# Illumina/manta

Hardware: AMD Instinct MI355X
Metric: candidate SV loci assembled+aligned per second (whole node) (higher is better)
Workload: dtype int32; 1 GPU; BASELINE config[1]: synthetic small-indel loci, 80 reads/locus x150bp, k=31..76 step 5, assemble + 10-mer trim + GlobalLargeIndelAligner(2,-8,-24,-1,-1;-100) on 1800 bp windows; loci_per_gpu=10000, reads_per_locus=80, block_loci=10000, workers_per_gpu=1, parallelism=loci sharded over 1 rank(s); per rank a cost-ordered block queue, queue=rank, dist_world=1, mix=False

## Files before the change

### include/manta_amd.h

```cpp
#ifndef MANTA_AMD_H
#define MANTA_AMD_H

#include <stdint.h>

#ifdef __cplusplus
extern "C" {
#endif

#define MANTA_OK 0
#define MANTA_E_INVALID_ARG (-1)
#define MANTA_E_NO_DEVICE (-2)
#define MANTA_E_HIP (-3)
#define MANTA_E_EMPTY_SEQ (-4)
#define MANTA_E_UNSUPPORTED (-5)
#define MANTA_E_CAPACITY (-6)
#define MANTA_E_DEVICE_FAULT (-7)
#define MANTA_E_SPLIT_QUERY_NOT_SHORTER (-8)
#define MANTA_E_SPLIT_EMPTY_SCAN (-9)
#define MANTA_E_NOT_TAKEN (-10)

typedef struct manta_ctx manta_ctx_t;

int         manta_ctx_create(int device_id, manta_ctx_t** ctx);
void        manta_ctx_destroy(manta_ctx_t* ctx);
const char* manta_last_error(const manta_ctx_t* ctx);
const char* manta_ctx_device_name(const manta_ctx_t* ctx);

enum { MANTA_ALIGNER_GLOBAL = 0, MANTA_ALIGNER_LARGE_INDEL = 1, MANTA_ALIGNER_JUMP = 2, MANTA_ALIGNER_JUMP_INTRON = 3 };

typedef struct {
  int32_t match, mismatch, open, extend, off_edge;
  int32_t is_allow_edge_insertion;
} manta_align_scores_t;

typedef struct {
  uint64_t query_off;
  uint64_t ref1_off;
  uint64_t ref2_off;
  uint32_t query_len;
  uint32_t ref1_len;
  uint32_t ref2_len;
  uint32_t reserved;
} manta_align_task_t;

enum { MANTA_INTRON_REF1_FW = 1, MANTA_INTRON_REF2_FW = 2, MANTA_INTRON_STRANDED = 4 };

typedef struct {
  int32_t  status;
  int32_t  score;
  int32_t  is_jumped;
  int32_t  begin_pos1;
  int32_t  begin_pos2;
  uint32_t jump_insert_size;
  uint32_t jump_range;
  uint32_t cigar1_len, cigar2_len;
  uint64_t cigar1_off, cigar2_off;
} manta_align_result_t;

int manta_align_batch(
    manta_ctx_t* ctx, int kind, const manta_align_scores_t* scores, int32_t extra_score, uint32_t n_tasks,
    const manta_align_task_t* tasks, const uint8_t* seq_arena, uint64_t seq_arena_bytes,
    manta_align_result_t* results, uint32_t* cigar_arena, uint64_t cigar_arena_cap, uint64_t* cigar_arena_used);

int manta_align_intron_batch(
    manta_ctx_t* ctx, const manta_align_scores_t* scores, int32_t jump_score, int32_t intron_open_score,
    int32_t intron_off_edge_score, uint32_t n_tasks, const manta_align_task_t* tasks, const uint8_t* seq_arena,
    uint64_t seq_arena_bytes, manta_align_result_t* results, uint32_t* cigar_arena, uint64_t cigar_arena_cap,
    uint64_t* cigar_arena_used);


typedef struct {
  uint32_t min_word_length, max_word_length, word_step_size, min_contig_length;
  uint32_t min_coverage, min_conservative_coverage, min_unused_reads, min_support_reads, max_assembly_count;
} manta_asm_options_t;

typedef struct {
  uint64_t seq_off;
  uint64_t support_off;
  uint64_t reject_off;
  uint32_t seq_len;
  uint32_t seed_read_count;
  int32_t  conservative_begin, conservative_end;
} manta_asm_contig_t;

typedef struct {
  int32_t  status;
  uint32_t n_contigs;
  uint32_t first_contig;
  uint32_t n_words;
  uint32_t n_pseudo;
  uint32_t final_word_length;
  uint32_t n_iterations;
  uint32_t cyclic_iterations;
  uint64_t pseudo_seq_off;
  uint64_t pseudo_len_off;
} manta_asm_locus_result_t;

int manta_assemble_batch(
    manta_ctx_t* ctx, const manta_asm_options_t* opt, uint32_t n_loci, const uint8_t* bases, const uint64_t* read_off,
    const uint32_t* locus_read_begin, manta_asm_locus_result_t* loci, manta_asm_contig_t* contigs, uint64_t contigs_cap,
    uint8_t* seq_arena, uint64_t seq_arena_cap, uint64_t* seq_arena_used, uint64_t* bits_arena, uint64_t bits_arena_cap,
    uint64_t* bits_arena_used);

int manta_debug_repeat_words(
    manta_ctx_t* ctx, const manta_asm_options_t* opt, uint32_t n_reads, const uint8_t* bases, const uint64_t* read_off, char* out,
    uint64_t out_cap, uint32_t* n_words);


typedef struct {
  uint32_t min_word_length, max_word_length, word_step_size, min_contig_length;
  uint32_t min_coverage, min_conservative_coverage, min_seed_reads, max_assembly_iterations;
} manta_small_asm_options_t;

int manta_small_assemble_batch(
    manta_ctx_t* ctx, const manta_small_asm_options_t* opt, uint32_t n_loci, const uint8_t* bases, const uint64_t* read_off,
    const uint32_t* locus_read_begin, manta_asm_locus_result_t* loci, manta_asm_contig_t* contigs, uint64_t contigs_cap,
    uint8_t* seq_arena, uint64_t seq_arena_cap, uint64_t* seq_arena_used, uint64_t* bits_arena, uint64_t bits_arena_cap,
    uint64_t* bits_arena_used);

typedef struct manta_smallsv manta_smallsv_t;

typedef struct {
  int32_t leading_cut, trailing_cut, max_leading_cut, max_trailing_cut;
} manta_ref_cuts_t;

typedef struct {
  int32_t              adjusted_leading_cut, adjusted_trailing_cut;
  manta_align_result_t align;
} manta_smallsv_alignment_t;

typedef struct {
  float    assemble_ms, schedule_ms, align_ms, total_ms;
  uint32_t n_align_launches;
  uint32_t n_alignments;
  uint64_t ptr_matrix_bytes;
  uint64_t dp_cells;
} manta_smallsv_stats_t;

int  manta_smallsv_create(manta_ctx_t* ctx, const manta_asm_options_t* opt, const manta_align_scores_t* scores,
                          int32_t large_indel_score, manta_smallsv_t** out);
void manta_smallsv_destroy(manta_smallsv_t* b);
int manta_smallsv_upload(manta_smallsv_t* b, uint32_t n_loci, const uint8_t* bases, const uint64_t* read_off,
                         const uint32_t* locus_read_begin, const uint8_t* refs, const uint64_t* ref_off,
                         const manta_ref_cuts_t* cuts);
int manta_smallsv_run(manta_smallsv_t* b);
int manta_smallsv_stats(const manta_smallsv_t* b, manta_smallsv_stats_t* stats);
int manta_smallsv_output_sizes(const manta_smallsv_t* b, uint64_t* contigs, uint64_t* seq_bytes, uint64_t* bits_words,
                               uint64_t* cigar_words);
int manta_smallsv_download(manta_smallsv_t* b, manta_asm_locus_result_t* loci, manta_asm_contig_t* contigs,
                           manta_smallsv_alignment_t* alignments, uint64_t contigs_cap, uint8_t* seq_arena,
                           uint64_t seq_arena_cap, uint64_t* seq_arena_used, uint64_t* bits_arena, uint64_t bits_arena_cap,
                           uint64_t* bits_arena_used, uint32_t* cigar_arena, uint64_t cigar_arena_cap,
                           uint64_t* cigar_arena_used);

typedef struct manta_spanning manta_spanning_t;

typedef struct {
  int32_t align1_leading_cut, align1_trailing_cut, align2_leading_cut, align2_trailing_cut;
} manta_jump_cuts_t;

typedef struct {
  int32_t              is_uncut;
  int32_t              reserved;
  manta_align_result_t align;
} manta_spanning_alignment_t;

int  manta_spanning_create(manta_ctx_t* ctx, const manta_asm_options_t* opt, const manta_align_scores_t* scores,
                           int32_t jump_score, manta_spanning_t** out);
void manta_spanning_destroy(manta_spanning_t* b);
int  manta_spanning_upload(manta_spanning_t* b, uint32_t n_loci, const uint8_t* bases, const uint64_t* read_off,
                           const uint32_t* locus_read_begin, const uint8_t* refs1, const uint64_t* ref1_off,
                           const uint8_t* refs2, const uint64_t* ref2_off, const manta_jump_cuts_t* cuts);
int  manta_spanning_run(manta_spanning_t* b);
int  manta_spanning_stats(const manta_spanning_t* b, manta_smallsv_stats_t* stats);
int  manta_spanning_output_sizes(const manta_spanning_t* b, uint64_t* contigs, uint64_t* seq_bytes, uint64_t* bits_words,
                                 uint64_t* cigar_words);
int  manta_spanning_download(manta_spanning_t* b, manta_asm_locus_result_t* loci, manta_asm_contig_t* contigs,
                             manta_spanning_alignment_t* alignments, uint64_t contigs_cap, uint8_t* seq_arena,
                             uint64_t seq_arena_cap, uint64_t* seq_arena_used, uint64_t* bits_arena, uint64_t bits_arena_cap,
                             uint64_t* bits_arena_used, uint32_t* cigar_arena, uint64_t cigar_arena_cap,
                             uint64_t* cigar_arena_used);

typedef struct {
  uint64_t query_off, qual_off, target_off;
  uint32_t query_len, target_len;
  int32_t  bp_begin, bp_end;
  uint32_t flank_score_size;
  uint32_t reserved;
} manta_split_task_t;

typedef struct {
  int32_t  status;
  uint32_t best_pos;
  float    best_ln_lhood;
  uint32_t left_size, hom_size, right_size;
  uint32_t left_mismatches, hom_mismatches, right_mismatches;
} manta_split_result_t;

int manta_split_read_batch(
    manta_ctx_t* ctx, const double* ln_comp_error_prob, const double* ln_error_prob, uint32_t n_qscores, float ln_one_third,
    float ln_random_base, uint32_t n_tasks, const manta_split_task_t* tasks, const uint8_t* arena, uint64_t arena_bytes,
    manta_split_result_t* results);

int manta_smallsv_set_word_lengths(manta_smallsv_t* b, uint32_t n_loci, const uint32_t* min_word_length,
                                   const uint32_t* max_word_length);
int manta_spanning_set_word_lengths(manta_spanning_t* b, uint32_t n_loci, const uint32_t* min_word_length,
                                    const uint32_t* max_word_length);

typedef struct {
  const uint32_t* codes;
  const uint32_t* nmask;
  const uint32_t* read_len;
  const uint64_t* read_code_off;
  const uint64_t* read_mask_off;
  const uint32_t* locus_read_begin;
} manta_packed_piles_t;

int manta_smallsv_upload_piles(manta_smallsv_t* b, uint32_t n_loci, const manta_packed_piles_t* piles, const uint8_t* refs,
                               const uint64_t* ref_off, const manta_ref_cuts_t* cuts);
int manta_spanning_upload_piles(manta_spanning_t* b, uint32_t n_loci, const manta_packed_piles_t* piles, const uint8_t* refs1,
                                const uint64_t* ref1_off, const uint8_t* refs2, const uint64_t* ref2_off,
                                const manta_jump_cuts_t* cuts);

int  manta_host_alloc(uint64_t bytes, void** out);
void manta_host_free(void* p);

#define MANTA_BATCH_SERIAL_KERNELS 1u
#define MANTA_BATCH_NO_STREAMED_UPLOAD 2u
typedef struct {
  uint32_t block_loci;
  uint32_t n_workers;
  uint32_t flags;
  uint32_t reserved;
  uint32_t* shared_queue;
} manta_batch_plan_t;

#define MANTA_ABI_VERSION 6
uint32_t manta_abi_version(void);
uint64_t manta_batch_stats_size(void);

typedef struct {
  double   wall_ms;
  double   h2d_ms, kernel_ms, d2h_ms;
  float    assemble_ms, schedule_ms, align_ms;
  uint32_t n_blocks, n_workers;
  uint64_t n_alignments, n_align_launches, dp_cells, ptr_matrix_bytes;
  uint64_t h2d_bytes, d2h_bytes;
  uint64_t n_loci_lds_small, n_loci_lds_big, n_loci_handed_back, n_loci_general;
} manta_batch_stats_t;

int manta_smallsv_batch(
    manta_ctx_t* ctx, const manta_asm_options_t* opt, const manta_align_scores_t* scores, int32_t large_indel_score,
    uint32_t n_loci, const uint8_t* bases, const uint64_t* read_off, const uint32_t* locus_read_begin, const uint8_t* refs,
    const uint64_t* ref_off, const manta_ref_cuts_t* cuts, const uint32_t* locus_min_word_length ,
    const uint32_t* locus_max_word_length , manta_asm_locus_result_t* loci, manta_asm_contig_t* contigs,
    manta_smallsv_alignment_t* alignments, uint64_t contigs_cap, uint8_t* seq_arena, uint64_t seq_arena_cap,
    uint64_t* seq_arena_used, uint64_t* bits_arena, uint64_t bits_arena_cap, uint64_t* bits_arena_used, uint32_t* cigar_arena,
    uint64_t cigar_arena_cap, uint64_t* cigar_arena_used, const manta_batch_plan_t* plan ,
    manta_batch_stats_t* stats );

int manta_smallsv_batch_piles(
    manta_ctx_t* ctx, const manta_asm_options_t* opt, const manta_align_scores_t* scores, int32_t large_indel_score,
    uint32_t n_loci, const manta_packed_piles_t* piles, const uint8_t* refs, const uint64_t* ref_off, const manta_ref_cuts_t* cuts,
    const uint32_t* locus_min_word_length , const uint32_t* locus_max_word_length ,
    manta_asm_locus_result_t* loci, manta_asm_contig_t* contigs, manta_smallsv_alignment_t* alignments, uint64_t contigs_cap,
    uint8_t* seq_arena, uint64_t seq_arena_cap, uint64_t* seq_arena_used, uint64_t* bits_arena, uint64_t bits_arena_cap,
    uint64_t* bits_arena_used, uint32_t* cigar_arena, uint64_t cigar_arena_cap, uint64_t* cigar_arena_used,
    const manta_batch_plan_t* plan , manta_batch_stats_t* stats );

int manta_spanning_batch(
    manta_ctx_t* ctx, const manta_asm_options_t* opt, const manta_align_scores_t* scores, int32_t jump_score, uint32_t n_loci,
    const uint8_t* bases, const uint64_t* read_off, const uint32_t* locus_read_begin, const uint8_t* refs1,
    const uint64_t* ref1_off, const uint8_t* refs2, const uint64_t* ref2_off, const manta_jump_cuts_t* cuts,
    const uint32_t* locus_min_word_length , const uint32_t* locus_max_word_length ,
    manta_asm_locus_result_t* loci, manta_asm_contig_t* contigs, manta_spanning_alignment_t* alignments, uint64_t contigs_cap,
    uint8_t* seq_arena, uint64_t seq_arena_cap, uint64_t* seq_arena_used, uint64_t* bits_arena, uint64_t bits_arena_cap,
    uint64_t* bits_arena_used, uint32_t* cigar_arena, uint64_t cigar_arena_cap, uint64_t* cigar_arena_used,
    const manta_batch_plan_t* plan , manta_batch_stats_t* stats );

int manta_spanning_batch_piles(
    manta_ctx_t* ctx, const manta_asm_options_t* opt, const manta_align_scores_t* scores, int32_t jump_score, uint32_t n_loci,
    const manta_packed_piles_t* piles, const uint8_t* refs1, const uint64_t* ref1_off, const uint8_t* refs2, const uint64_t* ref2_off,
    const manta_jump_cuts_t* cuts, const uint32_t* locus_min_word_length , const uint32_t* locus_max_word_length ,
    manta_asm_locus_result_t* loci, manta_asm_contig_t* contigs, manta_spanning_alignment_t* alignments, uint64_t contigs_cap,
    uint8_t* seq_arena, uint64_t seq_arena_cap, uint64_t* seq_arena_used, uint64_t* bits_arena, uint64_t bits_arena_cap,
    uint64_t* bits_arena_used, uint32_t* cigar_arena, uint64_t cigar_arena_cap, uint64_t* cigar_arena_used,
    const manta_batch_plan_t* plan , manta_batch_stats_t* stats );

typedef struct manta_node manta_node_t;
int         manta_node_create(const int32_t* device_ids, uint32_t n_devices, manta_node_t** out);
void        manta_node_destroy(manta_node_t* node);
uint32_t    manta_node_device_count(const manta_node_t* node);
const char* manta_node_last_error(const manta_node_t* node);

int manta_node_smallsv_batch(
    manta_node_t* node, const manta_asm_options_t* opt, const manta_align_scores_t* scores, int32_t large_indel_score,
    uint32_t n_loci, const uint8_t* bases, const uint64_t* read_off, const uint32_t* locus_read_begin, const uint8_t* refs,
    const uint64_t* ref_off, const manta_ref_cuts_t* cuts, const uint32_t* locus_min_word_length ,
    const uint32_t* locus_max_word_length , manta_asm_locus_result_t* loci, manta_asm_contig_t* contigs,
// ... 97 lines not shown
```

### manta_amd/csrc/api.cpp

```cpp
#include "api_internal.hpp"

extern "C" {

uint32_t manta_abi_version(void) { return MANTA_ABI_VERSION; }
uint64_t manta_batch_stats_size(void) { return sizeof(manta_batch_stats_t); }

int manta_ctx_create(int device_id, manta_ctx_t** out)
{
  if (!out) {
    g_createError = "manta_ctx_create: null output pointer";
    return MANTA_E_INVALID_ARG;
  }
  *out = nullptr;
  try {
    rt::init(device_id);
    if (!stringHashMatchesLibstdcxx()) {
      g_createError = "this libstdc++'s std::hash<std::string> is not the Murmur variant the exact repeat search restates";
      return MANTA_E_UNSUPPORTED;
    }
    manta_ctx_t* ctx = new manta_ctx();
    ctx->deviceName  = rt::deviceName();
    ctx->cuCount     = rt::cuCount();
    ctx->deviceId    = rt::currentDevice();
    *out             = ctx;
// ... 267 lines not shown
    AsmLocusOut lo;
    rt::d2h(&lo, st.dLoci, sizeof(lo));
    if (lo.status != ASM_OK) return fail(ctx, asmStatusToAbi(lo.status), "manta_debug_repeat_words: the locus did not assemble");
    const uint32_t nNodes = lo.reserved & 0x3ffffffu, slab = lo.reserved >> 26, k = lo.final_word_length;
    const AsmWsLayout L = asmWorkspaceLayout(st.capSlots, st.capNodes, st.capWords, st.capReads, st.maxContigLen, st.wMax, o.max_assembly_count);
    const uint8_t*    ws = st.dWs + st.stride * uint64_t(slab);
    std::vector<uint32_t> flag(nNodes), key(nNodes), codes(st.capWords + 2);
    rt::d2h(flag.data(), ws + L.node_flag, sizeof(uint32_t) * nNodes);
    rt::d2h(key.data(), ws + L.node_key, sizeof(uint32_t) * nNodes);
    rt::d2h(codes.data(), ws + L.codes, sizeof(uint32_t) * codes.size());
    std::vector<std::string> words;
    for (uint32_t nd = 0; nd < nNodes; ++nd) {
      if (!(flag[nd] & NF_REPEAT)) continue;
      std::string w(k, '?');
      for (uint32_t i = 0; i < k; ++i) {
        const uint32_t pb = key[nd] + i;
        w[i]              = "ACGT"[(codes[pb >> 4] >> (30 - 2 * (pb & 15))) & 3];
      }
      words.push_back(w);
    }
    std::sort(words.begin(), words.end());
    uint64_t used = 0;
    for (const std::string& w : words) {
      if (used + w.size() + 1 > out_cap) return fail(ctx, MANTA_E_CAPACITY, "manta_debug_repeat_words: output buffer too small");
      std::memcpy(out + used, w.data(), w.size());
      used += w.size();
      out[used++] = '\n';
    }
    if (used < out_cap) out[used] = 0;
    *n_words = uint32_t(words.size());
    return MANTA_OK;
  } catch (const std::exception& e) {
    return fail(ctx, MANTA_E_HIP, e.what());
  }
}

int manta_small_assemble_batch(
    manta_ctx_t* ctx, const manta_small_asm_options_t* opt, uint32_t n_loci, const uint8_t* bases, const uint64_t* read_off,
    const uint32_t* locus_read_begin, manta_asm_locus_result_t* loci, manta_asm_contig_t* contigs, uint64_t contigs_cap,
    uint8_t* seq_arena, uint64_t seq_arena_cap, uint64_t* seq_arena_used, uint64_t* bits_arena, uint64_t bits_arena_cap,
    uint64_t* bits_arena_used)
{
  if (!ctx) return MANTA_E_INVALID_ARG;
  if (!opt || (n_loci && (!bases || !read_off || !locus_read_begin || !loci || !contigs || !seq_arena || !bits_arena)))
    return fail(ctx, MANTA_E_INVALID_ARG, "manta_small_assemble_batch: null argument");
  if (opt->word_step_size == 0 || opt->min_word_length < 2 || opt->max_assembly_iterations > 31)
    return fail(ctx, MANTA_E_INVALID_ARG, "manta_small_assemble_batch: wordStepSize 0, minWordLength < 2 or more than 31 iterations");
  if (seq_arena_used) *seq_arena_used = 0;
  if (bits_arena_used) *bits_arena_used = 0;
  if (n_loci == 0) return MANTA_OK;
  try {
    rt::setDevice(ctx->deviceId);
    rt::ScopedStream onStream(ctx->stream);
    AsmStage st(ctx);
    manta_asm_options_t o{};
    o.min_word_length           = opt->min_word_length;
    o.max_word_length           = opt->max_word_length;
    o.word_step_size            = opt->word_step_size;
    o.min_contig_length         = opt->min_contig_length;
    o.min_coverage              = opt->min_coverage;
    o.min_conservative_coverage = opt->min_conservative_coverage;
    o.min_unused_reads          = 0;
    o.min_support_reads         = 0;
    o.max_assembly_count        = opt->max_assembly_iterations + 1;
    st.smallMode                = true;
    st.smallMinSeedReads        = opt->min_seed_reads;
    st.smallMaxIterations       = opt->max_assembly_iterations;
    int rc = st.plan(o, n_loci, read_off, locus_read_begin);
    if (rc != MANTA_OK) {
      for (uint32_t l = 0; l < n_loci; ++l) {
        std::memset(&loci[l], 0, sizeof(loci[l]));
        loci[l].status = rc;
      }
      return rc;
    }
    st.upload(bases, read_off, locus_read_begin);
    st.launch();
    rt::sync();
    return st.fetch(loci, contigs, contigs_cap, seq_arena, seq_arena_cap, seq_arena_used, bits_arena, bits_arena_cap, bits_arena_used);
  } catch (const std::exception& e) {
    return fail(ctx, MANTA_E_HIP, e.what());
  }
}

int manta_smallsv_create(
    manta_ctx_t* ctx, const manta_asm_options_t* opt, const manta_align_scores_t* scores, int32_t large_indel_score,
    manta_smallsv_t** out)
{
  if (!ctx) return MANTA_E_INVALID_ARG;
  if (!opt || !scores || !out) return fail(ctx, MANTA_E_INVALID_ARG, "manta_smallsv_create: null argument");
  try {
    rt::setDevice(ctx->deviceId);
    manta_smallsv* b = new manta_smallsv(ctx);
    b->opt           = *opt;
    b->scores        = *scores;
    b->largeIndel    = large_indel_score;
    *out             = b;
  } catch (const std::exception& e) {
    return fail(ctx, MANTA_E_HIP, e.what());
  }
  return MANTA_OK;
}

void manta_smallsv_destroy(manta_smallsv_t* b)
{
  delete b;
}

int manta_smallsv_upload(
    manta_smallsv_t* b, uint32_t n_loci, const uint8_t* bases, const uint64_t* read_off, const uint32_t* locus_read_begin,
    const uint8_t* refs, const uint64_t* ref_off, const manta_ref_cuts_t* cuts)
{
  if (!b) return MANTA_E_INVALID_ARG;
  manta_ctx_t* ctx = b->ctx;
  if (n_loci == 0 || !bases || !read_off || !locus_read_begin || !refs || !ref_off || !cuts)
    return fail(ctx, MANTA_E_INVALID_ARG, "manta_smallsv_upload: null argument or empty batch");
  try {
    rt::setDevice(ctx->deviceId);
    rt::ScopedStream onStream(b->main);
    b->uploaded = false;
    const double tP0 = nowMs();
    const bool streamed = b->streamUploads && !std::getenv("MANTA_AMD_NO_STREAM_UPLOAD");
    const bool noEarlyStream = std::getenv("MANTA_AMD_NO_EARLY_STREAM") != nullptr;
    const bool        chunksInFlight = streamed && !noEarlyStream && b->asmStage.startStream(n_loci, bases, read_off, locus_read_begin, b->copy);
    struct DrainOnFailure {
      manta_smallsv_t* b;
      bool             armed;
      ~DrainOnFailure() { if (armed) drainCopyStream(b); }
    } drain{b, chunksInFlight};
    int rc      = b->asmStage.plan(b->opt, n_loci, read_off, locus_read_begin);
    if (rc != MANTA_OK) return rc;
    const double tP1 = nowMs();
    b->nLoci    = n_loci;
    b->refBytes = ref_off[n_loci];
    b->maxRef   = 0;
    for (uint32_t l = 0; l < n_loci; ++l) {
      if (ref_off[l + 1] < ref_off[l]) return fail(ctx, MANTA_E_INVALID_ARG, "manta_smallsv_upload: ref_off not monotone");
      b->maxRef = std::max<uint64_t>(b->maxRef, ref_off[l + 1] - ref_off[l]);
      if (cuts[l].leading_cut < 0 || cuts[l].trailing_cut < 0 || cuts[l].max_leading_cut < 0 || cuts[l].max_trailing_cut < 0)
        return fail(ctx, MANTA_E_INVALID_ARG, "manta_smallsv_upload: negative reference cut");
    }
    uint8_t*  dRefs   = b->dRefs.as<uint8_t>(b->refBytes + 16);
    uint64_t* dRefOff = b->dRefOff.as<uint64_t>(n_loci + 1);
    auto*     dCuts   = b->dCuts.as<SmallSvCuts>(n_loci);
    static_assert(sizeof(SmallSvCuts) == sizeof(manta_ref_cuts_t), "cuts layout");
    b->refsOnCopy       = streamed;
    if (streamed) {
      b->asmStage.uploadStreamed(bases, read_off, locus_read_begin, b->copy);
      rt::ScopedStream onCopy(b->copy);
      rt::h2d(dRefs, refs, b->refBytes);
      rt::h2d(dRefOff, ref_off, sizeof(uint64_t) * (n_loci + 1));
      rt::h2d(dCuts, cuts, sizeof(SmallSvCuts) * n_loci);
      b->refsReady.record();
    } else {
      rt::h2d(dRefs, refs, b->refBytes);
      rt::h2d(dRefOff, ref_off, sizeof(uint64_t) * (n_loci + 1));
      rt::h2d(dCuts, cuts, sizeof(SmallSvCuts) * n_loci);
      b->asmStage.upload(bases, read_off, locus_read_begin);
      rt::sync();
    }
    if (std::getenv("MANTA_AMD_DEBUG_TIMING"))
      std::fprintf(stderr, "manta_amd: smallsv_upload plan %.2f ms, upload (%s) %.2f ms\n", tP1 - tP0, b->asmStage.streaming ? "streamed" : "blocking", nowMs() - tP1);
    drain.armed = false;
    b->uploaded = true;
    return MANTA_OK;
  } catch (const std::exception& e) {
    return fail(ctx, MANTA_E_HIP, e.what());
  }
}


int manta_smallsv_upload_piles(
    manta_smallsv_t* b, uint32_t n_loci, const manta_packed_piles_t* piles, const uint8_t* refs, const uint64_t* ref_off,
    const manta_ref_cuts_t* cuts)
{
  if (!b) return MANTA_E_INVALID_ARG;
  manta_ctx_t* ctx = b->ctx;
  if (n_loci == 0 || !refs || !ref_off || !cuts) return fail(ctx, MANTA_E_INVALID_ARG, "manta_smallsv_upload_piles: null argument or empty batch");
  int rc = checkPiles(ctx, piles, "manta_smallsv_upload_piles");
  if (rc != MANTA_OK) return rc;
  try {
    rt::setDevice(ctx->deviceId);
    rt::ScopedStream onStream(b->main);
    b->uploaded = false;
    b->refsOnCopy = false;
    rc          = b->asmStage.plan(b->opt, n_loci, nullptr, piles->locus_read_begin, piles->read_len);
    if (rc != MANTA_OK) return rc;
    b->nLoci    = n_loci;
    b->refBytes = ref_off[n_loci];
    b->maxRef   = 0;
    for (uint32_t l = 0; l < n_loci; ++l) {
      if (ref_off[l + 1] < ref_off[l]) return fail(ctx, MANTA_E_INVALID_ARG, "manta_smallsv_upload_piles: ref_off not monotone");
      b->maxRef = std::max<uint64_t>(b->maxRef, ref_off[l + 1] - ref_off[l]);
      if (cuts[l].leading_cut < 0 || cuts[l].trailing_cut < 0 || cuts[l].max_leading_cut < 0 || cuts[l].max_trailing_cut < 0)
        return fail(ctx, MANTA_E_INVALID_ARG, "manta_smallsv_upload_piles: negative reference cut");
    }
    uint8_t*  dRefs   = b->dRefs.as<uint8_t>(b->refBytes + 16);
    uint64_t* dRefOff = b->dRefOff.as<uint64_t>(n_loci + 1);
    auto*     dCuts   = b->dCuts.as<SmallSvCuts>(n_loci);
    b->refsOnCopy     = b->streamUploads && !std::getenv("MANTA_AMD_NO_STREAM_UPLOAD");
    if (b->refsOnCopy) {
      b->asmStage.uploadPilesStreamed(*piles, b->copy);
      rt::ScopedStream onCopy(b->copy);
      rt::h2d(dRefs, refs, b->refBytes);
      rt::h2d(dRefOff, ref_off, sizeof(uint64_t) * (n_loci + 1));
      rt::h2d(dCuts, cuts, sizeof(SmallSvCuts) * n_loci);
      b->refsReady.record();
    } else {
      b->asmStage.uploadPiles(*piles);
      rt::h2d(dRefs, refs, b->refBytes);
      rt::h2d(dRefOff, ref_off, sizeof(uint64_t) * (n_loci + 1));
      rt::h2d(dCuts, cuts, sizeof(SmallSvCuts) * n_loci);
      rt::sync();
    }
    b->uploaded = true;
    return MANTA_OK;
  } catch (const std::exception& e) {
    return fail(ctx, MANTA_E_HIP, e.what());
  }
}

}

int smallsvRunImpl(manta_smallsv_t* b, StageGates* gates)
{
  if (!b) return MANTA_E_INVALID_ARG;
  manta_ctx_t* ctx = b->ctx;
  if (!b->uploaded) return fail(ctx, MANTA_E_INVALID_ARG, "manta_smallsv_run: nothing uploaded");
  try {
    rt::setDevice(ctx->deviceId);
    rt::ScopedStream onStream(b->main);
    const uint32_t nLoci   = b->nLoci;
    const uint32_t maxAsm  = b->opt.max_assembly_count;
    const uint64_t nSlots  = uint64_t(nLoci) * maxAsm;
    AsmStage&      as(b->asmStage);
    AlignTaskDev*    dTasks   = b->dTasks.as<AlignTaskDev>(nSlots);
    SmallSvTaskInfo* dInfo    = b->dInfo.as<SmallSvTaskInfo>(nSlots);
    AlignResultDev*  dResults = b->dResults.as<AlignResultDev>(nSlots);
    uint32_t*        dBuckets = b->dBucketIds.as<uint32_t>(nSlots * kNumESet);
    uint32_t*        dSmall   = b->dSmall.as<uint32_t>(64);
    const uint32_t   tableCap = nextPow2(2ull * as.maxContigLen);
    const int        schedWaves = std::getenv("MANTA_AMD_SCHED_WAVES_PER_CU") ? std::max(1, std::atoi(std::getenv("MANTA_AMD_SCHED_WAVES_PER_CU"))) : 12;
    const uint32_t   schedChunk = std::getenv("MANTA_AMD_SCHED_CHUNK") ? uint32_t(std::max(1, std::atoi(std::getenv("MANTA_AMD_SCHED_CHUNK")))) : 2u;
    const int        schedGrid = rt::roundGrid(int(std::min<uint64_t>((nLoci + schedChunk - 1) / schedChunk, uint64_t(std::max(1, ctx->cuCount * schedWaves)))));
    uint32_t*        dTable   = b->dTable.as<uint32_t>(uint64_t(tableCap) * schedGrid);
    rt::dzero(dSmall, sizeof(uint32_t) * 64);
    rt::dzero(dResults, sizeof(AlignResultDev) * nSlots);

    const bool dbg = std::getenv("MANTA_AMD_DEBUG") != nullptr;
    auto       stage = [&](const char* what) {
      if (!dbg) return;
      rt::sync();
      std::fprintf(stderr, "manta_amd: smallsv_run %s\n", what);
      std::fflush(stderr);
    };
    stage("start");
    uint64_t asmCnt[4];
    {
      GateLock only(gates, &StageGates::asmMu);
      std::unique_lock<std::mutex> streamedOnly(streamedAsmMu(ctx), std::defer_lock);
      if (as.streaming) streamedOnly.lock();
      as.stageQueued = false;
      as.earlyStaged = false;
      b->evStart.record();
      as.launch();
      b->evAsm.record();
      rt::d2h(asmCnt, as.dCnt, sizeof(asmCnt));
      if (asmCnt[3]) {
        as.rerunCapacityFailures(asmCnt[3]);
        rt::d2h(asmCnt, as.dCnt, sizeof(asmCnt));
      }
    }
    stage("assembled");
    const bool noEarlyStage = std::getenv("MANTA_AMD_NO_EARLY_STAGE") != nullptr;
    const bool        earlyStage   = b->stageBehindRun && b->whileAligning && !noEarlyStage;
    if (earlyStage) as.stageEarly(b->copy, asmCnt, b->evEarlyStaged);
    const uint64_t cigarCap = 8ull * std::min<uint64_t>(asmCnt[1], as.devSeqCap) + 64;
    if (cigarCap + 16 > 0xffffffffull)
      return fail(ctx, MANTA_E_UNSUPPORTED, "manta_smallsv_run: alignment scratch of this block exceeds 2^32 words; use smaller blocks "
                                         "(manta_smallsv_batch splits a batch into blocks, manta_batch_plan_t::block_loci)");
    uint32_t* dCigar = b->dCigar.as<uint32_t>(cigarCap + 16);
    GateLock alignOnly(gates, &StageGates::alignMu);
    if (b->refsOnCopy) rt::curStreamWaits(b->refsReady);

    ScheduleParams S;
    S.loci               = as.dLoci;
    S.contigs            = as.dCont;
    S.seq_arena          = as.dSeq;
    S.n_loci             = nLoci;
    S.max_assembly_count = maxAsm;
    S.refs               = static_cast<const uint8_t*>(b->dRefs.p);
    S.ref_off            = static_cast<const uint64_t*>(b->dRefOff.p);
    S.cuts               = static_cast<const SmallSvCuts*>(b->dCuts.p);
    S.tasks              = dTasks;
    S.info               = dInfo;
    S.bucket_ids         = dBuckets;
    S.bucket_count       = dSmall;
    S.bucket_maxref      = dSmall + 16;
    S.cigar_used         = reinterpret_cast<unsigned long long*>(dSmall + 34);
    S.cigar_cap          = cigarCap;
    S.counter            = dSmall + 32;
    S.table_ws           = dTable;
    S.table_cap          = tableCap;
    S.n_e                = kNumESet;
    S.chunk              = schedChunk;
    for (int i = 0; i < kNumESet; ++i) S.e_set[i] = uint32_t(kESet[i]);
    rt::launch(smallsv_schedule_kernel, schedGrid, SCHED_LDS_BYTES, S);
    uint32_t  pairMask       = 0;
    uint32_t* dBucketsSorted = nullptr;
    for (int k = 0; k < kNumESet; ++k)
      if (alignUsesPairs(MANTA_ALIGNER_LARGE_INDEL, k, b->scores.match, b->scores.mismatch, b->scores.open, b->scores.extend, b->scores.off_edge,
                         b->largeIndel, b->scores.is_allow_edge_insertion ? 1 : 0, b->maxRef))
        pairMask |= 1u << k;
    if (pairMask) {
      dBucketsSorted = b->dBucketIds2.as<uint32_t>(nSlots * kNumESet);
      BucketSortParams BS;
      BS.tasks        = dTasks;
      BS.loci         = as.dLoci;
      BS.info         = dInfo;
      BS.ids_out      = dBucketsSorted;
      BS.n_loci       = nLoci;
      BS.max_assembly_count = maxAsm;
      BS.total        = uint32_t(nSlots);
      BS.mask         = pairMask;
      rt::launchWG(bucket_sort_kernel, kNumESet, int(BS_WAVES), BS_LDS_BYTES, BS);
    }
    b->evSched.record();
    stage("scheduled");

    uint32_t hSmall[40];
    const int    maxWaves = std::max(1, ctx->cuCount * alignWavesPerCu());
    const size_t wsBudget = workspaceBudget(size_t(48) << 30);
    bool         fromHistory = b->bucketHistory && b->stageBehindRun && !std::getenv("MANTA_AMD_SYNC_BUCKETS");
    struct Launch {
      int      k, grid;
      uint64_t stride, slabOff;
      bool     pair;
    };
    std::vector<Launch> launches;
    uint64_t            slabBytes = 0;
    auto pairOf = [&](int k) {
      return alignUsesPairs(MANTA_ALIGNER_LARGE_INDEL, k, b->scores.match, b->scores.mismatch, b->scores.open, b->scores.extend, b->scores.off_edge,
                            b->largeIndel, b->scores.is_allow_edge_insertion ? 1 : 0, b->maxRef);
    };
    const bool batchCall = b->stageBehindRun && !std::getenv("MANTA_AMD_SYNC_BUCKETS");
    bool       haveCounts = false;
    if (batchCall && !fromHistory) {
      rt::d2h(hSmall, dSmall, sizeof(hSmall));
      std::memcpy(b->lastSmall, hSmall, sizeof(b->lastSmall));
      haveCounts  = true;
      fromHistory = true;
    }
    if (fromHistory) {
      for (int k = kNumESet - 1; k >= 0; --k) {
        const bool     pair   = pairOf(k);
        const uint64_t tasks  = b->lastSmall[k] ? uint64_t(b->lastSmall[k]) + b->lastSmall[k] / 4 + 64 : 4;
        const uint64_t hint   = pair ? (tasks + 1) / 2 : tasks;
        const uint64_t qBound = (kESet[k] == 32) ? std::max<uint64_t>(as.maxContigLen, 64ull * 32) : 64ull * uint64_t(kESet[k]);
        const uint64_t refLen = alignSlabRefLen(MANTA_ALIGNER_LARGE_INDEL, kESet[k], qBound, b->maxRef);
        const uint64_t stride = ((pair ? 2 : 1) * alignPtrSlabBytes(MANTA_ALIGNER_LARGE_INDEL, kESet[k], refLen) + 255) & ~uint64_t(255);
        const int      grid   = rt::roundGrid(int(std::min<uint64_t>(hint, uint64_t(maxWaves))));
        launches.push_back(Launch{k, grid, stride, slabBytes, pair});
        slabBytes += stride * uint64_t(grid);
      }
      if (slabBytes > wsBudget / 3) {
        fromHistory = false;
        launches.clear();
        slabBytes = 0;
      }
    }
    if (!fromHistory) {
      if (!haveCounts) rt::d2h(hSmall, dSmall, sizeof(hSmall));
      for (int k = kNumESet - 1; k >= 0; --k) {
        const uint32_t cnt = hSmall[k];
        if (cnt == 0) continue;
        const bool     pair   = pairOf(k);
        const uint64_t stride = ((pair ? 2 : 1) * alignPtrSlabBytes(MANTA_ALIGNER_LARGE_INDEL, kESet[k], hSmall[16 + k]) + 255) & ~uint64_t(255);
        int            grid   = int(std::min<size_t>(pair ? (cnt + 1) / 2 : cnt, size_t(maxWaves)));
        grid                  = int(std::max<size_t>(1, std::min<size_t>(size_t(grid), (wsBudget / 3) / stride)));
        grid                  = rt::roundGrid(grid);
        launches.push_back(Launch{k, grid, stride, slabBytes, pair});
        slabBytes += stride * uint64_t(grid);
      }
    }
    b->stats.n_align_launches = 0;
    b->stats.n_alignments     = 0;
    b->stats.ptr_matrix_bytes = 0;
    {
      static const bool   noMerge = std::getenv("MANTA_AMD_NO_ALIGN_MERGE") != nullptr;
      std::vector<Launch> merged;
      if (!noMerge) {
        std::vector<Launch> rest;
        for (const Launch& l : launches) (l.pair ? merged : rest).push_back(l);
        if (merged.size() < 2 || merged.size() > 6) {
          merged.clear();
        } else {
          launches.swap(rest);
          slabBytes = 0;
          for (Launch& l : launches) {
            l.slabOff = slabBytes;
            slabBytes += l.stride * uint64_t(l.grid);
          }
        }
      }
      uint64_t mergedStride = 0, mergedWaves = 0, mergedOff = slabBytes;
      const uint32_t* counts = fromHistory ? b->lastSmall : hSmall;
      if (!merged.empty()) {
        std::stable_sort(merged.begin(), merged.end(), [&](const Launch& x, const Launch& y) { return counts[x.k] < counts[y.k]; });
        for (const Launch& l : merged) {
          mergedStride = std::max(mergedStride, l.stride);
          mergedWaves += uint64_t(l.grid);
        }
        mergedWaves = std::min<uint64_t>(std::min<uint64_t>(mergedWaves, uint64_t(maxWaves)), (wsBudget / 3) / mergedStride);
        mergedWaves = std::max<uint64_t>(WV_WAVES_PER_WG, (mergedWaves / WV_WAVES_PER_WG) * WV_WAVES_PER_WG);
        slabBytes += mergedStride * mergedWaves;
      }
      uint8_t* dWsAll = b->dPtrWs.as<uint8_t>(slabBytes + 256);
      for (int i = 0; i < 3; ++i) rt::streamWaits(b->side[i], b->evSched);
      auto baseParams = [&]() {
        AlignParams P;
        P.tasks          = dTasks;
        P.results        = dResults;
        P.cigar          = dCigar;
        P.task_ids       = nullptr;
        P.n_tasks        = 0;
        P.n_tasks_dev    = nullptr;
        P.counter        = nullptr;
        P.ptr_ws         = nullptr;
        P.ptr_ws_stride  = 0;
        P.match          = b->scores.match;
        P.mismatch       = b->scores.mismatch;
        P.open           = b->scores.open;
        P.extend         = b->scores.extend;
        P.off_edge       = b->scores.off_edge;
        P.allow_edge_ins = b->scores.is_allow_edge_insertion ? 1 : 0;
        P.extra          = b->largeIndel;
        return P;
      };
      for (size_t i = 0; i < launches.size(); ++i) {
        const Launch& l(launches[i]);
        AlignParams   P  = baseParams();
        P.task_ids       = (l.pair ? dBucketsSorted : dBuckets) + uint64_t(l.k) * nSlots;
        P.n_tasks        = fromHistory ? uint32_t(nSlots) : hSmall[l.k];
        P.n_tasks_dev    = fromHistory ? dSmall + l.k : nullptr;
        P.counter        = dSmall + 40 + l.k;
        P.ptr_ws         = dWsAll + l.slabOff;
        P.ptr_ws_stride  = l.stride;
        {
          rt::ScopedStream onSide(b->side[i % 3]);
          launchAlignKind(MANTA_ALIGNER_LARGE_INDEL, l.k, l.grid, P, l.pair);
        }
        if (!fromHistory) {
          b->stats.n_align_launches++;
          b->stats.n_alignments += hSmall[l.k];
        }
      }
      if (!merged.empty()) {
        PairMultiParams M;
        M.A               = baseParams();
        M.A.counter       = dSmall + 40 + merged[0].k;
        M.A.ptr_ws        = dWsAll + mergedOff;
        M.A.ptr_ws_stride = mergedStride;
        M.bucket_ids      = dBucketsSorted;
        M.counts          = dSmall;
        M.n_slots         = uint32_t(nSlots);
        M.n_order         = uint32_t(merged.size());
        M.prio_work[0] = 2560u;
        M.prio_work[1] = 0u;
        M.prio_work[2] = 4096u;
        if (const char* e = std::getenv("MANTA_AMD_ALIGN_PRIO")) {
          unsigned v[3] = {0, 0, 0};
          std::sscanf(e, "%u,%u,%u", &v[0], &v[1], &v[2]);
          for (int i = 0; i < 3; ++i) M.prio_work[i] = v[i];
        }
        for (size_t i = 0; i < 8; ++i) {
          M.order[i] = uint8_t(i < merged.size() ? merged[i].k : 0);
          M.e_of[i]  = uint8_t(i < merged.size() ? kESet[merged[i].k] : 0);
        }
        if (std::getenv("MANTA_AMD_DEBUG"))
          std::fprintf(stderr, "manta_amd: align_pair_multi_kernel: %llu waves over %zu packed buckets, slab stride %llu\n",
                       (unsigned long long)mergedWaves, merged.size(), (unsigned long long)mergedStride);
        rt::launch(align_pair_multi_kernel, int(mergedWaves), 0, M);
        if (!fromHistory) {
          b->stats.n_align_launches++;
          for (const Launch& l : merged) b->stats.n_alignments += hSmall[l.k];
        }
      }
      for (size_t i = 0; i < std::min<size_t>(launches.size(), 3); ++i) {
        b->sideDone[i].recordOn(b->side[i]);
        rt::curStreamWaits(b->sideDone[i]);
      }
    }
    launchPack(b, dTasks, nullptr, dResults, nullptr, dInfo, nullptr, dCigar, cigarCap);
    b->evAlign.record();
    uint32_t* hSmallPin = b->pSmall.as<uint32_t>(40);
    rt::d2hAsync(hSmallPin, dSmall, sizeof(uint32_t) * 40);
    if (b->stageBehindRun) pipeStageEnqueue(b);
    if (earlyStage) {
      b->evEarlyStaged.sync();
      as.finishEarly();
      b->whileAligning();
    }
    rt::sync();
    std::memcpy(b->lastSmall, hSmallPin, sizeof(b->lastSmall));
    b->bucketHistory = true;
    if (fromHistory)
      for (int k = 0; k < kNumESet; ++k)
        if (b->lastSmall[k]) {
          b->stats.n_align_launches++;
          b->stats.n_alignments += b->lastSmall[k];
        }
    alignOnly.release();
    if (as.streaming) {
      rt::ScopedStream onCopy(b->copy);
      rt::sync();
    }
    stage("aligned");
    b->stats.assemble_ms = rt::elapsedMs(b->evStart, b->evAsm);
    b->stats.schedule_ms = rt::elapsedMs(b->evAsm, b->evSched);
    b->stats.align_ms    = rt::elapsedMs(b->evSched, b->evAlign);
    b->stats.total_ms    = rt::elapsedMs(b->evStart, b->evAlign);
    b->ran               = true;
    return MANTA_OK;
  } catch (const std::exception& e) {
    drainCopyStream(b);
    return fail(ctx, MANTA_E_HIP, e.what());
  }
}

extern "C" {

int manta_smallsv_run(manta_smallsv_t* b) { return smallsvRunImpl(b, nullptr); }

int manta_smallsv_stats(const manta_smallsv_t* b, manta_smallsv_stats_t* stats)
{
  if (!b || !stats) return MANTA_E_INVALID_ARG;
  *stats = b->stats;
  return MANTA_OK;
}

int manta_smallsv_output_sizes(const manta_smallsv_t* b, uint64_t* contigs, uint64_t* seq_bytes, uint64_t* bits_words, uint64_t* cigar_words)
{
  if (!b || !contigs || !seq_bytes || !bits_words || !cigar_words) return MANTA_E_INVALID_ARG;
  if (!b->ran) return fail(b->ctx, MANTA_E_INVALID_ARG, "manta_smallsv_output_sizes: run first");
  try {
    rt::setDevice(b->ctx->deviceId);
    rt::ScopedStream onStream(const_cast<manta_smallsv_t*>(b)->main);
    b->asmStage.outputSizes(*contigs, *seq_bytes, *bits_words);
    uint32_t hSmall[40];
    rt::d2h(hSmall, b->dSmall.p, sizeof(hSmall));
    uint64_t cig = 0;
    std::memcpy(&cig, hSmall + 34, sizeof(uint64_t));
    *cigar_words = cig + 64;
    return MANTA_OK;
  } catch (const std::exception& e) {
    return fail(b->ctx, MANTA_E_HIP, e.what());
  }
}

}


extern "C" {

int manta_smallsv_download(
    manta_smallsv_t* b, manta_asm_locus_result_t* loci, manta_asm_contig_t* contigs, manta_smallsv_alignment_t* alignments,
    uint64_t contigs_cap, uint8_t* seq_arena, uint64_t seq_arena_cap, uint64_t* seq_arena_used, uint64_t* bits_arena,
    uint64_t bits_arena_cap, uint64_t* bits_arena_used, uint32_t* cigar_arena, uint64_t cigar_arena_cap,
    uint64_t* cigar_arena_used)
{
  if (!b) return MANTA_E_INVALID_ARG;
  manta_ctx_t* ctx = b->ctx;
  if (!b->ran) return fail(ctx, MANTA_E_INVALID_ARG, "manta_smallsv_download: run first");
  if (!loci || !contigs || !alignments || !seq_arena || !bits_arena || !cigar_arena)
    return fail(ctx, MANTA_E_INVALID_ARG, "manta_smallsv_download: null argument");
  try {
    rt::setDevice(ctx->deviceId);
    rt::ScopedStream onStream(b->main);
    pipeStage(b);
    return smallsvCompact(b, loci, contigs, alignments, 0, contigs_cap, seq_arena, seq_arena_cap, 0, seq_arena_used, bits_arena,
                          bits_arena_cap, 0, bits_arena_used, cigar_arena, cigar_arena_cap, 0, cigar_arena_used);
  } catch (const std::exception& e) {
    return fail(ctx, MANTA_E_HIP, e.what());
  }
}

int manta_spanning_create(
    manta_ctx_t* ctx, const manta_asm_options_t* opt, const manta_align_scores_t* scores, int32_t jump_score, manta_spanning_t** out)
{
  if (!ctx) return MANTA_E_INVALID_ARG;
  if (!opt || !scores || !out) return fail(ctx, MANTA_E_INVALID_ARG, "manta_spanning_create: null argument");
  if (scores->is_allow_edge_insertion)
    return fail(ctx, MANTA_E_INVALID_ARG, "GlobalJumpAligner does not support isAllowEdgeInsertion");
  try {
    rt::setDevice(ctx->deviceId);
    manta_spanning* b = new manta_spanning(ctx);
    b->opt            = *opt;
    b->scores         = *scores;
    b->jumpScore      = jump_score;
    *out              = b;
  } catch (const std::exception& e) {
    return fail(ctx, MANTA_E_HIP, e.what());
  }
  return MANTA_OK;
}

void manta_spanning_destroy(manta_spanning_t* b)
{
  delete b;
}

int manta_spanning_upload(
    manta_spanning_t* b, uint32_t n_loci, const uint8_t* bases, const uint64_t* read_off, const uint32_t* locus_read_begin,
    const uint8_t* refs1, const uint64_t* ref1_off, const uint8_t* refs2, const uint64_t* ref2_off, const manta_jump_cuts_t* cuts)
{
  if (!b) return MANTA_E_INVALID_ARG;
  manta_ctx_t* ctx = b->ctx;
  if (n_loci == 0 || !bases || !read_off || !locus_read_begin || !refs1 || !ref1_off || !refs2 || !ref2_off || !cuts)
    return fail(ctx, MANTA_E_INVALID_ARG, "manta_spanning_upload: null argument or empty batch");
  try {
    rt::setDevice(ctx->deviceId);
    rt::ScopedStream onStream(b->main);
    b->uploaded = false;
    int rc      = b->asmStage.plan(b->opt, n_loci, read_off, locus_read_begin);
    if (rc != MANTA_OK) return rc;
    b->nLoci     = n_loci;
    b->ref1Bytes = ref1_off[n_loci];
    b->ref2Bytes = ref2_off[n_loci];
    for (uint32_t l = 0; l < n_loci; ++l) {
      if (ref1_off[l + 1] < ref1_off[l] || ref2_off[l + 1] < ref2_off[l])
        return fail(ctx, MANTA_E_INVALID_ARG, "manta_spanning_upload: reference offsets not monotone");
      const manta_jump_cuts_t& c(cuts[l]);
      if (c.align1_leading_cut < 0 || c.align1_trailing_cut < 0 || c.align2_leading_cut < 0 || c.align2_trailing_cut < 0)
        return fail(ctx, MANTA_E_INVALID_ARG, "manta_spanning_upload: negative reference cut");
    }
    static_assert(sizeof(JumpCuts) == sizeof(manta_jump_cuts_t), "cuts layout");
    uint8_t*  dRefs1   = b->dRefs1.as<uint8_t>(b->ref1Bytes + 16);
    uint64_t* dRef1Off = b->dRef1Off.as<uint64_t>(n_loci + 1);
    uint8_t*  dRefs2   = b->dRefs2.as<uint8_t>(b->ref2Bytes + 16);
    uint64_t* dRef2Off = b->dRef2Off.as<uint64_t>(n_loci + 1);
    JumpCuts* dCuts    = b->dCuts.as<JumpCuts>(n_loci);
    auto      copyRefs = [&] {
      rt::h2d(dRefs1, refs1, b->ref1Bytes);
      rt::h2d(dRef1Off, ref1_off, sizeof(uint64_t) * (n_loci + 1));
      rt::h2d(dRefs2, refs2, b->ref2Bytes);
      rt::h2d(dRef2Off, ref2_off, sizeof(uint64_t) * (n_loci + 1));
      rt::h2d(dCuts, cuts, sizeof(JumpCuts) * n_loci);
    };
    b->hostCuts.assign(reinterpret_cast<const JumpCuts*>(cuts), reinterpret_cast<const JumpCuts*>(cuts) + n_loci);
    b->refsOnCopy = b->streamUploads && !std::getenv("MANTA_AMD_NO_STREAM_UPLOAD");
    if (b->refsOnCopy) {
      b->asmStage.uploadStreamed(bases, read_off, locus_read_begin, b->copy);
      rt::ScopedStream onCopy(b->copy);
      copyRefs();
      b->refsReady.record();
    } else {
      b->asmStage.upload(bases, read_off, locus_read_begin);
      copyRefs();
      rt::sync();
    }
    b->uploaded = true;
    return MANTA_OK;
  } catch (const std::exception& e) {
    return fail(ctx, MANTA_E_HIP, e.what());
  }
}

int manta_spanning_upload_piles(
    manta_spanning_t* b, uint32_t n_loci, const manta_packed_piles_t* piles, const uint8_t* refs1, const uint64_t* ref1_off,
    const uint8_t* refs2, const uint64_t* ref2_off, const manta_jump_cuts_t* cuts)
{
  if (!b) return MANTA_E_INVALID_ARG;
  manta_ctx_t* ctx = b->ctx;
  if (n_loci == 0 || !refs1 || !ref1_off || !refs2 || !ref2_off || !cuts)
    return fail(ctx, MANTA_E_INVALID_ARG, "manta_spanning_upload_piles: null argument or empty batch");
  int rc = checkPiles(ctx, piles, "manta_spanning_upload_piles");
  if (rc != MANTA_OK) return rc;
  try {
    rt::setDevice(ctx->deviceId);
    rt::ScopedStream onStream(b->main);
    b->uploaded = false;
    b->refsOnCopy = false;
    rc          = b->asmStage.plan(b->opt, n_loci, nullptr, piles->locus_read_begin, piles->read_len);
    if (rc != MANTA_OK) return rc;
    b->asmStage.uploadPiles(*piles);
    b->nLoci     = n_loci;
    b->ref1Bytes = ref1_off[n_loci];
    b->ref2Bytes = ref2_off[n_loci];
    for (uint32_t l = 0; l < n_loci; ++l) {
      if (ref1_off[l + 1] < ref1_off[l] || ref2_off[l + 1] < ref2_off[l])
        return fail(ctx, MANTA_E_INVALID_ARG, "manta_spanning_upload_piles: reference offsets not monotone");
// ... 349 lines not shown
```

### manta_amd/csrc/api_internal.hpp

```cpp
#pragma once
#include "../../include/manta_amd.h"

#include <algorithm>
#include <atomic>
#include <unistd.h>
#include <functional>
#include <condition_variable>
#include <chrono>
#include <cstdio>
#include <cstdlib>
#include <cstring>
#include <memory>
#include <mutex>
#include <string>
#include <thread>
#include <vector>

#include "align_kernels.hpp"
#include "align_jump_pair.hpp"
#include "assemble_kernels.hpp"
#include "asm_lds.hpp"
#include "small_asm.hpp"
#include "pipeline_kernels.hpp"
#include "split_kernels.hpp"
// ... 310 lines not shown
class HostPool {
 public:
  static HostPool& get()
  {
    static HostPool pool;
    return pool;
  }
  template <typename F>
  void run(const uint64_t n, const unsigned parts, F fn)
  {
    auto begin = [&](unsigned t) { return n * t / parts; };
    if (parts <= 1 || getpid() != owner) {
      fn(0u, uint64_t(0), n);
      return;
    }
    std::lock_guard<std::mutex> only(runMu);
    std::function<void(unsigned)> job = [&](unsigned t) { fn(t, begin(t), begin(t + 1)); };
    {
      std::lock_guard<std::mutex> g(mu);
      current = &job;
      wanted  = parts - 1;
      pending = parts - 1;
      ++generation;
    }
    cv.notify_all();
    struct WaitForHelpers {
      HostPool& p;
      ~WaitForHelpers()
      {
        std::unique_lock<std::mutex> g(p.mu);
        p.done.wait(g, [&] { return p.pending == 0; });
        p.current = nullptr;
      }
    } waitForHelpers{*this};
    fn(0u, begin(0), begin(1));
  }

 private:
  HostPool() : owner(getpid())
  {
    for (unsigned i = 0; i + 1 < kHostPartsMax; ++i) threads.emplace_back([this, i] { loop(i + 1); });
  }
  ~HostPool()
  {
    if (getpid() != owner) {
      for (std::thread& t : threads) t.detach();
      return;
    }
    {
      std::lock_guard<std::mutex> g(mu);
      stop = true;
    }
    cv.notify_all();
    for (std::thread& t : threads) t.join();
  }
  void loop(const unsigned id)
  {
    uint64_t seen = 0;
    while (true) {
      std::function<void(unsigned)>* job = nullptr;
      {
        std::unique_lock<std::mutex> g(mu);
        cv.wait(g, [&] { return stop || generation != seen; });
        if (stop) return;
        seen = generation;
        if (id <= wanted) job = current;
      }
      if (job) {
        (*job)(id);
        std::lock_guard<std::mutex> g(mu);
        if (--pending == 0) done.notify_one();
      }
    }
  }
  const pid_t                    owner;
  std::mutex                     mu, runMu;
  std::condition_variable        cv, done;
  std::vector<std::thread>       threads;
  std::function<void(unsigned)>* current = nullptr;
  unsigned                       wanted = 0, pending = 0;
  uint64_t                       generation = 0;
  bool                           stop = false;
};
template <typename F>
void hostParallel(const uint64_t n, const unsigned parts, F fn)
{
  HostPool::get().run(n, parts, fn);
}

inline uint32_t nextPow2(uint64_t v)
{
  uint64_t p = 1;
  while (p < v) p <<= 1;
  return uint32_t(p);
}

inline int asmStatusToAbi(int st)
{
  switch (st) {
  case ASM_OK: return MANTA_OK;
  case ASM_E_ALPHABET:
  case ASM_E_WORD_TOO_LONG:
  case ASM_E_TOO_MANY_READS: return MANTA_E_UNSUPPORTED;
  default: return MANTA_E_DEVICE_FAULT;
  }
}


struct AsmStage {
  manta_ctx_t* ctx;
  explicit AsmStage(manta_ctx_t* c) : ctx(c)
  {
    g_liveWorkspaces++;
    g_livePerDevice[std::min(kMaxDevices - 1, std::max(0, c->deviceId))]++;
  }
  ~AsmStage()
  {
    g_liveWorkspaces--;
    g_livePerDevice[std::min(kMaxDevices - 1, std::max(0, ctx->deviceId))]--;
    if (dChunksDone) rt::dfree(dChunksDone);
  }
  AsmStage(const AsmStage&) = delete;
  AsmStage& operator=(const AsmStage&) = delete;
  PinnedBuf     pLoci, pCont, pSeq, pBits, pCnt;
  AsmLocusOut*  hLoci = nullptr;
  AsmContigOut* hCont = nullptr;
  uint8_t*      hSeq  = nullptr;
  uint64_t*     hBits = nullptr;
  uint64_t*     hCnt  = nullptr;
  uint64_t      seqUsedDev = 0, bitsUsedDev = 0, nContigsOut = 0, pseudoBytesOut = 0, pseudoCountOut = 0;
  bool          staged = false;
  uint32_t      ldsFallbacks = 0;

  manta_asm_options_t opt{};
  uint32_t            nLoci = 0, nReadsTotal = 0, maxContigLen = 0, wMax = 0, capWords = 0, capReads = 0, capNodes = 0, capSlots = 0;
  uint64_t            nBases = 0, stride = 0, devSeqCap = 0, devBitsCap = 0;
  int                 grid = 1;
  DevBuf              bBases, bReadOff, bLocusBegin, bLoci, bContigs, bSeqArena, bBitsArena, bCounters, bWs, bGrowth, bWl, bOrder;
  std::vector<uint32_t> locusMinWl, locusMaxWl;
  std::vector<uint32_t> order;
  uint32_t              maxWordLen = 0;
  uint32_t              capWords2 = 0, capNodes2 = 0, capSlots2 = 0;
  uint64_t              stride2 = 0;
  DevBuf                bWs2, bFailIds;
  uint32_t              nRerun = 0;
  AsmParams             lastParams{};
  bool                  smallMode = false;
  uint32_t              smallMinSeedReads = 0, smallMaxIterations = 0;
  int                   wavesPerCuCap = 0;
  bool                  useFast = false;
  int                   gridFast = 1;
  int                   gridContig[manta_dev::LG_CLASSES] = {0, 0, 0, 0};
  bool                  contigPool = false;
  uint32_t              classBytes[manta_dev::LG_CLASSES] = {0, 0, 0, 0};
  uint64_t              lgArenaCap = 0, cwsStride = 0;
  std::vector<uint32_t> fastIds, genIds;
  std::vector<uint32_t> bigIds;
  int                   gridBig = 1;
  int                   gridContigBig[manta_dev::LGL_CLASSES] = {0, 0};
  uint32_t              classBytesBig[manta_dev::LGL_CLASSES] = {0, 0};
  uint64_t              cwsStrideBig = 0;
  DevBuf                bLgClassIdsBig, bCwsBig;
  uint32_t              bigRounds = 0;
  std::function<void()> afterFirstRound;
  bool                  firstRoundHookRan = false;
  int                   gridRepeat = 0;
  uint64_t              pseudoArenaDw = 0, rwsStride = 0;
  DevBuf                bLgIter, bLgPseudo, bLgNext, bLgCyc, bLgRounds, bRws, bGws;
  DevBuf                bPunt, bLgArena, bLgOff, bLgClassIds, bLgCnt, bCws, bLgBins;
  uint32_t*             dPunt = nullptr;
  DevBuf                bPlCodes, bPlMask, bPlLen, bPlCodeOff, bPlMaskOff;
  uint32_t *            dPlCodes = nullptr, *dPlMask = nullptr, *dPlLen = nullptr;
  uint64_t *            dPlCodeOff = nullptr, *dPlMaskOff = nullptr;
  uint32_t*             dMinWl = nullptr;
  uint32_t*             dMaxWl = nullptr;
  uint32_t*             dOrder = nullptr;
  uint8_t*            dBases = nullptr;
  uint64_t*           dOff   = nullptr;
  uint32_t*           dBegin = nullptr;
  AsmLocusOut*        dLoci  = nullptr;
  AsmContigOut*       dCont  = nullptr;
  uint8_t*            dSeq   = nullptr;
  uint64_t*           dBits  = nullptr;
  uint64_t*           dCnt   = nullptr;
  uint8_t*            dWs    = nullptr;
  uint32_t*           dGrowth = nullptr;

  int plan(const manta_asm_options_t& o, uint32_t n_loci, const uint64_t* read_off, const uint32_t* locus_read_begin,
           const uint32_t* read_len = nullptr)
  {
    if (o.min_word_length == 0 || o.word_step_size == 0 || o.min_coverage == 0 || o.max_assembly_count == 0)
      return fail(ctx, MANTA_E_INVALID_ARG, "assembler options: word length, step, minCoverage and maxAssemblyCount must be >= 1");
    if (o.max_word_length > 16u * ASM_MAX_KW) return fail(ctx, MANTA_E_UNSUPPORTED, "word lengths above 128 are not supported");
    if (2 * o.max_assembly_count > ASM_MAX_CAND) return fail(ctx, MANTA_E_UNSUPPORTED, "maxAssemblyCount above 32 is not supported");
    opt         = o;
    nLoci       = n_loci;
    for (uint32_t l = 0; l < n_loci; ++l)
      if (locus_read_begin[l + 1] < locus_read_begin[l]) return fail(ctx, MANTA_E_INVALID_ARG, "locus_read_begin not monotone");
    nReadsTotal = locus_read_begin[n_loci];
    maxWordLen  = o.max_word_length;
    if (!locusMinWl.empty()) {
      if (locusMinWl.size() != n_loci || locusMaxWl.size() != n_loci)
        return fail(ctx, MANTA_E_INVALID_ARG, "per-locus word lengths were set for a different number of loci");
      for (uint32_t l = 0; l < n_loci; ++l) {
        if (locusMinWl[l] == 0 || locusMaxWl[l] > 16u * ASM_MAX_KW) return fail(ctx, MANTA_E_UNSUPPORTED, "per-locus word length outside 1..128");
        maxWordLen = std::max(maxWordLen, locusMaxWl[l]);
      }
    }
    nBases      = read_off ? read_off[nReadsTotal] : 0;
    const double tPlan0 = nowMs();
    uint64_t maxLocusBases = 0, maxLocusWords = 0, bitsBound = 0;
    uint32_t maxLocusReads = 0, maxReadLen = 0;
    std::vector<uint64_t> cost(n_loci);
    uint32_t              ldsFit = 0, ldsFitBig = 0;
    {
      struct Part {
        uint64_t maxLocusBases = 0, maxLocusWords = 0, bitsBound = 0;
        uint32_t maxLocusReads = 0, maxReadLen = 0, ldsFit = 0, ldsFitBig = 0;
        int      bad = 0;
      };
      const unsigned    parts = hostParts(nReadsTotal);
      std::vector<Part> part(parts);
      const uint32_t    maxAsm = opt.max_assembly_count;
      const bool        avx2   = hostHasAvx2();
      hostParallel(n_loci, parts, [&](unsigned t, uint64_t l0, uint64_t l1) {
        Part p;
        struct StoreAtExit {
          Part& to;
          Part& from;
          ~StoreAtExit() { to = from; }
        } storeAtExit{part[t], p};
        for (uint64_t l = l0; l < l1; ++l) {
          const uint32_t rb = locus_read_begin[l], re = locus_read_begin[l + 1];
          if (re < rb || re > nReadsTotal) {
            p.bad = 1;
            return;
          }
          uint64_t b = 0, w = 0, longest = 0;
          if (read_off) {
            const uint64_t* o = read_off + rb;
            (avx2 ? scanOffsetsAvx2 : scanOffsetsBase)(o, re - rb, w, longest);
            b = o[re - rb] - o[0];
          } else {
            const uint32_t* o = read_len + rb;
            for (uint32_t i = 0; i < re - rb; ++i) {
              const uint64_t len = o[i];
              b += len;
              w += (len + 15) >> 4;
              longest = std::max(longest, len);
            }
          }
          w += re - rb;
          if (longest > 0xffffffffull) {
            p.bad = 2;
            return;
          }
          p.maxReadLen = std::max<uint32_t>(p.maxReadLen, uint32_t(longest));
          cost[l] = b * uint64_t(re - rb);
          if ((re - rb) + 2 * maxAsm <= manta_dev::LG_MAX_READS && w + 2 <= manta_dev::LG_MAX_PILE) {
            p.ldsFit++;
            cost[l] |= uint64_t(1) << 63;
          } else if ((re - rb) + 2 * maxAsm <= manta_dev::LGL_MAX_READS && w + 2 <= manta_dev::LGL_MAX_PILE + 2 &&
                     (!read_off || b + 64 <= manta_dev::LGL_STAGE_BYTES)) {
            p.ldsFitBig++;
            cost[l] |= uint64_t(1) << 62;
          }
          p.maxLocusBases = std::max(p.maxLocusBases, b);
          p.maxLocusWords = std::max(p.maxLocusWords, w);
          p.maxLocusReads = std::max(p.maxLocusReads, re - rb);
          const uint64_t W = ((re - rb) + 2 * maxAsm + 63) / 64;
          p.bitsBound += uint64_t(maxAsm) * 2 * W + 2 * maxAsm;
        }
      });
      for (const Part& p : part) {
        if (p.bad == 1) return fail(ctx, MANTA_E_INVALID_ARG, "locus_read_begin not monotone");
        if (p.bad == 2) return fail(ctx, MANTA_E_INVALID_ARG, "read_off not monotone");
        maxLocusBases = std::max(maxLocusBases, p.maxLocusBases);
        maxLocusWords = std::max(maxLocusWords, p.maxLocusWords);
        maxLocusReads = std::max(maxLocusReads, p.maxLocusReads);
        maxReadLen    = std::max(maxReadLen, p.maxReadLen);
        ldsFit += p.ldsFit;
        ldsFitBig += p.ldsFitBig;
        bitsBound += p.bitsBound;
      }
    }
    const double tPlan1 = nowMs();
    {
      order.resize(n_loci);
      bool uniform = true;
      for (uint32_t l = 1; l < n_loci && uniform; ++l) uniform = cost[l] == cost[0];
      if (uniform) {
        for (uint32_t l = 0; l < n_loci; ++l) order[l] = l;
      } else {
        std::vector<std::pair<uint64_t, uint32_t>> keyed(n_loci);
        for (uint32_t l = 0; l < n_loci; ++l) keyed[l] = std::make_pair(~(cost[l] & ~(uint64_t(3) << 62)), l);
        std::sort(keyed.begin(), keyed.end());
        for (uint32_t l = 0; l < n_loci; ++l) order[l] = keyed[l].second;
      }
    }
    {
      const char*       pathEnv = std::getenv("MANTA_AMD_ASM_PATH");
      const std::string path    = pathEnv ? pathEnv : "";
      const bool        useBig  = !(std::getenv("MANTA_AMD_LG_BIG") && std::atoi(std::getenv("MANTA_AMD_LG_BIG")) == 0);
      useFast                   = !smallMode && (ldsFit > 0 || (useBig && ldsFitBig > 0)) && path != "general";
      fastIds.clear();
      bigIds.clear();
// ... 76 lines not shown
      if (std::getenv("MANTA_AMD_DEBUG"))
        for (unsigned c = 0; c < LG_CLASSES; ++c) {
          if (!classBytes[c]) continue;
          if (c == 0 && contigPool)
            std::fprintf(stderr, "manta_amd: contig_pool_kernel class 0: up to %u bytes per locus from pools of %u bytes, %d waves in workgroups of %u (%d per CU by the runtime's count)\n",
                         classBytes[c], CK_POOL_BYTES, gridContig[c], CK_POOL_WAVES, rt::blocksPerCu(contig_pool_kernel, 64 * int(CK_POOL_WAVES), CK_POOL_BYTES, -1));
          else
            std::fprintf(stderr, "manta_amd: contig_kernel class %u: %u bytes of LDS, %d workgroups (%d per CU by the runtime's count)\n", c, classBytes[c], gridContig[c], rt::blocksPerCu(contig_kernel, 64, classBytes[c], -1));
        }
      cwsStride  = ckWorkspaceLayout().total;
      gridBig = int(std::max<uint64_t>(1, std::min<uint64_t>(bigIds.size(), uint64_t(ctx->cuCount))));
      static const uint32_t kClassBig[LGL_CLASSES] = {81920, 163840};
      for (unsigned c = 0; c < LGL_CLASSES; ++c) {
        classBytesBig[c] = kClassBig[c];
        gridContigBig[c] = int(std::max<uint64_t>(1, std::min<uint64_t>(bigIds.size(), uint64_t(ctx->cuCount) * (163840 / kClassBig[c]))));
      }
      cwsStrideBig = ckWorkspaceLayout(LgL::SETW).total;
      bigRounds    = 0;
      const char*    re       = std::getenv("MANTA_AMD_BIG_ROUNDS");
      const uint64_t roundMax = std::getenv("MANTA_AMD_BIG_ROUNDS_MAX") ? std::strtoull(std::getenv("MANTA_AMD_BIG_ROUNDS_MAX"), nullptr, 10) : uint64_t(65536);
      const bool     roundsOn = re ? (std::atoi(re) != 0) : (bigIds.size() <= roundMax);
      if (roundsOn && !bigIds.empty() && opt.max_assembly_count <= 20) {
        for (const uint32_t l : bigIds) {
          const uint32_t lo = locusMinWl.empty() ? opt.min_word_length : locusMinWl[l], hi = locusMaxWl.empty() ? opt.max_word_length : locusMaxWl[l];
          if (hi >= lo) bigRounds = std::max<uint32_t>(bigRounds, (hi - lo) / opt.word_step_size + 1);
        }
        bigRounds     = std::min<uint32_t>(bigRounds, LGL_MAX_ROUNDS);
        gridRepeat    = rt::roundGrid(int(std::min<uint64_t>(uint64_t(ctx->cuCount) * 4 * MANTA_RPB_OCC, std::max<uint64_t>(64, bigIds.size() / 4))));
        rwsStride     = rpbWorkspaceLayout().total;
        pseudoArenaDw = std::max<uint64_t>(uint64_t(4) << 20, uint64_t(bigIds.size()) * 512);
      }
      lgArenaCap   = std::min<uint64_t>(uint64_t(fastIds.size()) * lgSlabBytes(LG_MAX_NODES, LG_MAX_NODES, LG_MAX_PILE + 2) +
                                          uint64_t(bigIds.size() + (bigRounds ? 3 * std::min<size_t>(bigIds.size(), 512) : 0)) * lgSlabL(LGL_MAX_NODES, LGL_POOL_CAP + LGL_POOL_OVF, LGL_MAX_PILE_ALL + 4).total + 4096,
                                      wsBudget / 2);
      if (std::getenv("MANTA_AMD_DEBUG"))
        std::fprintf(stderr, "manta_amd: slab arena of the LDS pipeline: %.1f MB for %zu + %zu loci (cap %.1f MB)\n", double(lgArenaCap) / 1e6, fastIds.size(), bigIds.size(),
                     double(wsBudget / 2) / 1e6);
      (void)maxGrid;
    }
    const uint64_t worstLocusSeq = uint64_t(opt.max_assembly_count) * maxContigLen + uint64_t(nCandMax) * pseudoLen;
    devSeqCap  = uint64_t(n_loci) * std::min<uint64_t>(worstLocusSeq, 65536) + worstLocusSeq + 4096;
    devBitsCap = bitsBound + 64;
    if (std::getenv("MANTA_AMD_DEBUG_TIMING"))
      std::fprintf(stderr, "manta_amd: plan: scan %.2f ms, order %.2f, sizing %.2f\n", tPlan1 - tPlan0, tPlan2 - tPlan1, nowMs() - tPlan2);
    std::call_once(ctx->growthOnce, [&] { recordGrowthSchedule(ctx->growthSize, ctx->growthBuckets, 4u << 20); });
    return MANTA_OK;
  }

  void uploadPiles(const manta_packed_piles_t& pl)
  {
    const uint64_t c0 = pl.read_code_off[0], c1 = pl.read_code_off[nReadsTotal], m0 = pl.read_mask_off[0], m1 = pl.read_mask_off[nReadsTotal];
    dPlCodes   = bPlCodes.as<uint32_t>(c1 - c0 + 4);
    dPlMask    = bPlMask.as<uint32_t>(m1 - m0 + 4);
    dPlLen     = bPlLen.as<uint32_t>(nReadsTotal + 1);
    dPlCodeOff = bPlCodeOff.as<uint64_t>(nReadsTotal + 1);
    dPlMaskOff = bPlMaskOff.as<uint64_t>(nReadsTotal + 1);
    rt::h2d(dPlCodes, pl.codes + c0, sizeof(uint32_t) * (c1 - c0));
    rt::h2d(dPlMask, pl.nmask + m0, sizeof(uint32_t) * (m1 - m0));
    rt::h2d(dPlLen, pl.read_len, sizeof(uint32_t) * nReadsTotal);
    if (c0 == 0 && m0 == 0) {
      rt::h2d(dPlCodeOff, pl.read_code_off, sizeof(uint64_t) * (nReadsTotal + 1));
      rt::h2d(dPlMaskOff, pl.read_mask_off, sizeof(uint64_t) * (nReadsTotal + 1));
    } else {
      plRebased.resize(2 * (size_t(nReadsTotal) + 1));
      for (uint32_t r = 0; r <= nReadsTotal; ++r) {
        plRebased[r]                   = pl.read_code_off[r] - c0;
        plRebased[nReadsTotal + 1 + r] = pl.read_mask_off[r] - m0;
      }
      rt::h2d(dPlCodeOff, plRebased.data(), sizeof(uint64_t) * (nReadsTotal + 1));
      rt::h2d(dPlMaskOff, plRebased.data() + nReadsTotal + 1, sizeof(uint64_t) * (nReadsTotal + 1));
    }
    plBytes = 4 * (c1 - c0) + 4 * (m1 - m0) + 20ull * nReadsTotal;
    upload(nullptr, nullptr, pl.locus_read_begin);
  }
  std::vector<uint64_t> plRebased;
  uint64_t              plBytes = 0;

  static const uint32_t kStreamChunks = 32;
  static int streamFreeSlots(const int cuCount)
  {
    static const int forced = std::getenv("MANTA_AMD_STREAM_FREE_WGS") ? std::max(1, std::atoi(std::getenv("MANTA_AMD_STREAM_FREE_WGS"))) : 0;
    const int        want   = forced ? forced : 16;
    return std::max(1, std::min(((want + 7) / 8) * 8, cuCount / 4));
  }
  static uint32_t streamChunks()
  {
    static const uint32_t n = std::getenv("MANTA_AMD_STREAM_CHUNKS") ? uint32_t(std::max(1, std::min(int(kStreamChunks), std::atoi(std::getenv("MANTA_AMD_STREAM_CHUNKS"))))) : 16u;
    return n;
  }
  DevBuf                bPlShift;
  uint64_t*             dPlShift = nullptr;
  bool                  streamingPiles = false;
  DevBuf                bStream;
  uint32_t*             dStream = nullptr;
  uint32_t*             dChunksDone = nullptr;
  PinnedBuf             pChunkIds;
  uint32_t              chunkLoci = 0;
  bool                  streaming = false;

  void uploadStreamed(const uint8_t* bases, const uint64_t* read_off, const uint32_t* locus_read_begin, rt::Stream& copyStream)
  {
    const bool chunksQueued = preStreamed && preLoci == nLoci;
    if (preStreamed && !chunksQueued) {
      rt::ScopedStream onCopy(copyStream);
      rt::sync();
    }
    preStreamed = false;
    StreamLayout L;
    if (chunksQueued)
      L = preLayout;
    else
      L = streamLayout(nLoci, read_off, locus_read_begin);
    chunkLoci                 = L.chunkLoci;
    const uint64_t savedBases = nBases;
    nBases                    = L.cursor + 64;
    upload(nullptr, nullptr, chunksQueued ? nullptr : locus_read_begin);
    nBases  = savedBases;
    dPlCodes = nullptr;
    if (!chunksQueued) rt::h2d(dOff, read_off, sizeof(uint64_t) * (nReadsTotal + 1));
    dStream = bStream.as<uint32_t>(1 + kStreamChunks);
    rt::h2d(dStream, L.shift, sizeof(uint32_t) * (1 + kStreamChunks));
    if (!chunksQueued) resetChunkCounter(copyStream);
    if (chunksQueued) rt::curStreamWaits(evPreSmall);
    rt::sync();
    if (!chunksQueued) queueChunks(L, bases, copyStream);
    streaming = true;
  }

  struct StreamLayout {
    uint32_t chunkLoci = 0, nChunks = 0;
    uint64_t cursor = 0;
    uint64_t hostBegin[kStreamChunks + 1] = {0}, devBegin[kStreamChunks + 1] = {0};
    uint32_t shift[1 + kStreamChunks] = {0};
    bool     monotone = true;
  };
  static StreamLayout streamLayout(const uint32_t n, const uint64_t* read_off, const uint32_t* locus_read_begin)
  {
    StreamLayout L;
    L.chunkLoci = std::max<uint32_t>(1, (n + streamChunks() - 1) / streamChunks());
    L.nChunks   = (n + L.chunkLoci - 1) / L.chunkLoci;
    for (uint32_t c = 0; c < L.nChunks; ++c) {
      const uint32_t l0 = c * L.chunkLoci, l1 = std::min(n, l0 + L.chunkLoci);
      L.hostBegin[c]    = read_off[locus_read_begin[l0]];
      const uint64_t end = read_off[locus_read_begin[l1]];
      if (end < L.hostBegin[c]) L.monotone = false;
      const uint64_t len = end - L.hostBegin[c];
      L.devBegin[c]      = L.cursor;
      L.shift[1 + c]     = uint32_t(L.devBegin[c] - L.hostBegin[c]);
      L.cursor           = (L.cursor + len + 64 + 255) & ~uint64_t(255);
    }
    L.hostBegin[L.nChunks] = read_off[locus_read_begin[n]];
    return L;
  }
  void resetChunkCounter(rt::Stream& copyStream)
  {
    if (!dChunksDone) dChunksDone = static_cast<uint32_t*>(rt::dmallocFine(64));
    uint32_t* ids = pChunkIds.as<uint32_t>(kStreamChunks + 1);
    for (uint32_t c = 0; c <= kStreamChunks; ++c) ids[c] = c;
    {
      rt::ScopedStream onCopy(copyStream);
      rt::sync();
    }
    rt::h2d(dChunksDone, ids, sizeof(uint32_t));
  }
  void queueChunks(const StreamLayout& L, const uint8_t* bases, rt::Stream& copyStream)
  {
    const uint32_t*   ids = pChunkIds.as<uint32_t>(kStreamChunks + 1);
    rt::ScopedStream onCopy(copyStream);
    for (uint32_t c = 0; c < L.nChunks; ++c) {
      rt::h2d(dBases + L.devBegin[c], bases + L.hostBegin[c], L.hostBegin[c + 1] - L.hostBegin[c]);
      if (!rt::streamWrite32(dChunksDone, c + 1)) rt::h2d(dChunksDone, ids + c + 1, sizeof(uint32_t));
    }
  }
  bool                  preStreamed = false;
  rt::Event             evPreSmall;
  uint32_t              preLoci     = 0;
  StreamLayout          preLayout;
  bool startStream(const uint32_t n_loci, const uint8_t* bases, const uint64_t* read_off, const uint32_t* locus_read_begin, rt::Stream& copyStream)
  {
    preStreamed = false;
    for (uint32_t l = 0; l < n_loci; ++l)
      if (locus_read_begin[l + 1] < locus_read_begin[l]) return false;
    preLayout = streamLayout(n_loci, read_off, locus_read_begin);
    if (!preLayout.monotone) return false;
    dBases = bBases.as<uint8_t>(preLayout.cursor + 64 + 64);
    const uint32_t nReads = locus_read_begin[n_loci];
    dOff   = bReadOff.as<uint64_t>(size_t(nReads) + 1);
    dBegin = bLocusBegin.as<uint32_t>(size_t(n_loci) + 1);
    resetChunkCounter(copyStream);
    rt::sync();
    {
      rt::ScopedStream onCopy(copyStream);
      rt::h2d(dOff, read_off, sizeof(uint64_t) * (size_t(nReads) + 1));
      rt::h2d(dBegin, locus_read_begin, sizeof(uint32_t) * (size_t(n_loci) + 1));
      evPreSmall.record();
    }
    queueChunks(preLayout, bases, copyStream);
    preStreamed = true;
    preLoci     = n_loci;
    return true;
  }

  void uploadPilesStreamed(const manta_packed_piles_t& pl, rt::Stream& copyStream)
  {
    chunkLoci = std::max<uint32_t>(1, (nLoci + streamChunks() - 1) / streamChunks());
    const uint32_t nChunks = (nLoci + chunkLoci - 1) / chunkLoci;
    struct Piece {
      uint32_t r0, r1;
      uint64_t c0, c1, m0, m1, dr, dc, dm;
    };
    std::vector<Piece>    pc(nChunks);
    std::vector<uint64_t> shifts(3 * kStreamChunks, 0);
    uint64_t              curR = 0, curC = 0, curM = 0;
    auto                  lineUp = [](uint64_t v) { return (v + 63) & ~uint64_t(63); };
    for (uint32_t c = 0; c < nChunks; ++c) {
      const uint32_t l0 = c * chunkLoci, l1 = std::min(nLoci, l0 + chunkLoci);
      Piece&         q(pc[c]);
      q.r0 = pl.locus_read_begin[l0], q.r1 = pl.locus_read_begin[l1];
      q.c0 = pl.read_code_off[q.r0], q.c1 = pl.read_code_off[q.r1];
      q.m0 = pl.read_mask_off[q.r0], q.m1 = pl.read_mask_off[q.r1];
      q.dr = curR, q.dc = curC, q.dm = curM;
      shifts[3 * c + 0] = q.dr - q.r0;
      shifts[3 * c + 1] = q.dc - q.c0;
      shifts[3 * c + 2] = q.dm - q.m0;
      curR = lineUp(curR + (q.r1 - q.r0) + 1);
      curC = lineUp(curC + (q.c1 - q.c0) + 4);
      curM = lineUp(curM + (q.m1 - q.m0) + 4);
    }
    dPlCodes   = bPlCodes.as<uint32_t>(curC + 64);
    dPlMask    = bPlMask.as<uint32_t>(curM + 64);
    dPlLen     = bPlLen.as<uint32_t>(curR + 64);
    dPlCodeOff = bPlCodeOff.as<uint64_t>(curR + 64);
    dPlMaskOff = bPlMaskOff.as<uint64_t>(curR + 64);
    plBytes    = 0;
    upload(nullptr, nullptr, pl.locus_read_begin);
    dPlShift = bPlShift.as<uint64_t>(3 * kStreamChunks);
    rt::h2d(dPlShift, shifts.data(), sizeof(uint64_t) * 3 * kStreamChunks);
    if (!dChunksDone) dChunksDone = static_cast<uint32_t*>(rt::dmallocFine(64));
    uint32_t* ids = pChunkIds.as<uint32_t>(kStreamChunks + 1);
    for (uint32_t c = 0; c <= kStreamChunks; ++c) ids[c] = c;
    {
      rt::ScopedStream onCopy(copyStream);
      rt::sync();
    }
    rt::h2d(dChunksDone, ids, sizeof(uint32_t));
    rt::sync();
    {
      rt::ScopedStream onCopy(copyStream);
      for (uint32_t c = 0; c < nChunks; ++c) {
        const Piece&   q(pc[c]);
        const uint64_t nR = q.r1 - q.r0;
        rt::h2d(dPlLen + q.dr, pl.read_len + q.r0, sizeof(uint32_t) * nR);
        rt::h2d(dPlCodeOff + q.dr, pl.read_code_off + q.r0, sizeof(uint64_t) * (nR + 1));
        rt::h2d(dPlMaskOff + q.dr, pl.read_mask_off + q.r0, sizeof(uint64_t) * (nR + 1));
        rt::h2d(dPlCodes + q.dc, pl.codes + q.c0, sizeof(uint32_t) * (q.c1 - q.c0));
        rt::h2d(dPlMask + q.dm, pl.nmask + q.m0, sizeof(uint32_t) * (q.m1 - q.m0));
        if (!rt::streamWrite32(dChunksDone, c + 1)) rt::h2d(dChunksDone, ids + c + 1, sizeof(uint32_t));
        plBytes += 4 * (q.c1 - q.c0) + 4 * (q.m1 - q.m0) + 20ull * nR;
      }
    }
    streaming       = true;
    streamingPiles  = true;
  }

  void upload(const uint8_t* bases, const uint64_t* read_off, const uint32_t* locus_read_begin)
  {
    if (bases) dPlCodes = nullptr;
    streaming = streamingPiles = false;
    dBases  = bBases.as<uint8_t>(nBases + 64);
    dOff    = bReadOff.as<uint64_t>(nReadsTotal + 1);
    dBegin  = bLocusBegin.as<uint32_t>(nLoci + 1);
    dLoci   = bLoci.as<AsmLocusOut>(nLoci);
    dCont   = bContigs.as<AsmContigOut>(uint64_t(nLoci) * opt.max_assembly_count);
    dSeq    = bSeqArena.as<uint8_t>(devSeqCap);
    dBits   = bBitsArena.as<uint64_t>(devBitsCap);
    dCnt    = bCounters.as<uint64_t>(16);
    dWs     = bWs.as<uint8_t>(stride * grid);
    dGrowth = bGrowth.as<uint32_t>(2 * ctx->growthSize.size() + 2);
    dOrder  = bOrder.as<uint32_t>(nLoci);
    if (useFast) {
      dPunt = bPunt.as<uint32_t>(nLoci);
      if (!fastIds.empty()) rt::h2d(dOrder, fastIds.data(), sizeof(uint32_t) * fastIds.size());
      if (!bigIds.empty()) rt::h2d(dOrder + fastIds.size(), bigIds.data(), sizeof(uint32_t) * bigIds.size());
      if (!genIds.empty()) rt::h2d(dPunt, genIds.data(), sizeof(uint32_t) * genIds.size());
      int maxGrid = 1, maxGridBig = 1;
      for (unsigned c = 0; c < manta_dev::LG_CLASSES; ++c) maxGrid = std::max(maxGrid, gridContig[c]);
      for (unsigned c = 0; c < manta_dev::LGL_CLASSES; ++c) maxGridBig = std::max(maxGridBig, gridContigBig[c]);
      (void)bLgArena.as<uint8_t>(lgArenaCap + 64);
      (void)bLgOff.as<uint64_t>(nLoci);
      (void)bLgClassIds.as<uint32_t>(uint64_t(manta_dev::LG_CLASSES) * std::max<size_t>(1, fastIds.size()));
      if (contigPool) (void)bLgBins.as<uint32_t>(manta_dev::CK_BIN_IDS + uint64_t(manta_dev::CK_BINS) * fastIds.size());
      (void)bLgCnt.as<uint64_t>(16);
      (void)bCws.as<uint8_t>(cwsStride * uint64_t(maxGrid));
      if (!bigIds.empty()) {
        (void)bLgClassIdsBig.as<uint32_t>(uint64_t(manta_dev::LGL_CLASSES) * bigIds.size());
        (void)bCwsBig.as<uint8_t>(cwsStrideBig * uint64_t(maxGridBig));
        if (bigRounds) {
          (void)bLgIter.as<manta_dev::LgIter>(nLoci);
          (void)bLgPseudo.as<uint32_t>(pseudoArenaDw + 64);
          (void)bLgNext.as<uint32_t>(2 * bigIds.size());
          (void)bLgCyc.as<uint32_t>(bigIds.size());
          (void)bLgRounds.as<uint32_t>(8 * (manta_dev::LGL_MAX_ROUNDS + 1) + 32);
          (void)bRws.as<uint8_t>(rwsStride * uint64_t(gridRepeat));
          (void)bGws.as<uint8_t>(uint64_t(manta_dev::LGL_GWS_BYTES) * uint64_t(gridBig));
        }
      }
    } else {
      rt::h2d(dOrder, order.data(), sizeof(uint32_t) * nLoci);
    }
    dMinWl = dMaxWl = nullptr;
    if (!locusMinWl.empty()) {
      dMinWl = bWl.as<uint32_t>(2ull * nLoci);
      dMaxWl = dMinWl + nLoci;
      rt::h2d(dMinWl, locusMinWl.data(), sizeof(uint32_t) * nLoci);
      rt::h2d(dMaxWl, locusMaxWl.data(), sizeof(uint32_t) * nLoci);
    }
    if (bases) {
      rt::h2d(dBases, bases, nBases);
      rt::h2d(dOff, read_off, sizeof(uint64_t) * (nReadsTotal + 1));
    }
    if (locus_read_begin) rt::h2d(dBegin, locus_read_begin, sizeof(uint32_t) * (nLoci + 1));
    rt::h2d(dGrowth, ctx->growthSize.data(), sizeof(uint32_t) * ctx->growthSize.size());
    rt::h2d(dGrowth + ctx->growthSize.size(), ctx->growthBuckets.data(), sizeof(uint32_t) * ctx->growthBuckets.size());
  }

  void launch()
  {
    rt::dzero(dCnt, sizeof(uint64_t) * 16);
    rt::dfill(dLoci, 0xff, sizeof(AsmLocusOut) * nLoci);
    AsmParams P;
    P.bases            = dBases;
    P.read_off         = dOff;
    P.locus_read_begin = dBegin;
    P.n_loci           = nLoci;
    P.opt = AsmOptsDev{opt.min_word_length, opt.max_word_length, opt.word_step_size, opt.min_coverage,
                       opt.min_conservative_coverage, opt.min_unused_reads, opt.min_support_reads, opt.max_assembly_count};
    P.counter        = reinterpret_cast<uint32_t*>(dCnt);
    P.ws             = dWs;
    P.ws_stride      = stride;
    P.cap_slots      = capSlots;
    P.cap_nodes      = capNodes;
    P.cap_words      = capWords;
    P.cap_reads      = capReads;
    P.max_contig_len = maxContigLen;
    P.w_max          = wMax;
    P.loci           = dLoci;
    P.contigs        = dCont;
    P.seq_arena      = dSeq;
    P.seq_cap        = devSeqCap;
    P.seq_used       = reinterpret_cast<unsigned long long*>(dCnt + 1);
    P.bits_arena     = dBits;
    P.bits_cap       = devBitsCap;
    P.bits_used      = reinterpret_cast<unsigned long long*>(dCnt + 2);
    P.phase_cycles   = reinterpret_cast<unsigned long long*>(dCnt + 4);
    P.growth_size    = dGrowth;
    P.growth_buckets = dGrowth + ctx->growthSize.size();
    P.n_growth       = uint32_t(ctx->growthSize.size());
    P.flags          = std::getenv("MANTA_AMD_SERIAL_WALK") ? ASM_FLAG_SERIAL_WALK : 0u;
    P.locus_min_wl   = dMinWl;
    P.locus_max_wl   = dMaxWl;
    P.locus_ids      = dOrder;
    P.pl_codes       = dPlCodes;
    P.pl_nmask       = dPlMask;
    P.pl_read_len    = dPlLen;
    P.pl_code_off    = dPlCodeOff;
    P.pl_mask_off    = dPlMaskOff;
    P.upload_chunks_done = streaming ? dChunksDone : nullptr;
    P.chunk_shift        = (streaming && !streamingPiles) ? dStream + 1 : nullptr;
    P.pl_chunk_shift     = streamingPiles ? dPlShift : nullptr;
    P.chunk_loci         = streaming ? chunkLoci : 0;
    P.reserved2          = 0;
    P.small_min_seed_reads = smallMinSeedReads;
    P.small_max_iterations = smallMaxIterations;
    P.punt_ids             = nullptr;
    P.punt_count           = nullptr;
    P.n_loci_dev           = nullptr;
    P.lds_bytes            = ASM_LDS_BYTES;
    P.stop_before          = 0;
    lastParams             = P;
    nRerun                 = 0;
    if (smallMode) {
      rt::launch(small_assemble_kernel, grid, 0, P);
      return;
    }
    int g = grid;
    if (streaming && g >= ctx->cuCount * 16) g = rt::roundGrid(g - ctx->cuCount);
    P.lds_bytes = ASM_LDS_BYTES;
    if (useFast) {
      using namespace manta_dev;
      const uint32_t nGen = uint32_t(genIds.size());
      rt::h2d(reinterpret_cast<uint32_t*>(dCnt + 14), &nGen, sizeof(uint32_t));
      uint64_t* dLg = bLgCnt.as<uint64_t>(16);
      rt::dzero(dLg, sizeof(uint64_t) * 16);
      LgArgs A;
      A.P            = P;
      A.P.n_loci     = uint32_t(fastIds.size());
      A.P.punt_ids   = dPunt;
      A.P.punt_count = reinterpret_cast<uint32_t*>(dCnt + 14);
      A.G.arena        = bLgArena.as<uint8_t>(lgArenaCap + 64);
      A.G.arena_cap    = lgArenaCap;
      A.G.arena_used   = reinterpret_cast<unsigned long long*>(dLg);
      A.G.slab_off     = bLgOff.as<uint64_t>(nLoci);
      A.G.class_ids    = bLgClassIds.as<uint32_t>(uint64_t(LG_CLASSES) * std::max<size_t>(1, fastIds.size()));
      A.G.class_count  = reinterpret_cast<uint32_t*>(dLg + 1);
      A.G.class_stride = uint32_t(fastIds.size());
      for (unsigned c = 0; c < LG_CLASSES; ++c) A.G.class_bytes[c] = classBytes[c];
      A.G.cls        = 0;
      A.G.flags      = (std::getenv("MANTA_AMD_LG_NO_PROOF") ? LG_FLAG_NO_PROOF : 0u) | (std::getenv("MANTA_AMD_LG_NO_RESCUE") ? LG_FLAG_NO_RESCUE : 0u);
      A.G.stats      = reinterpret_cast<uint32_t*>(dLg + 8);
      int maxGrid = 1;
      for (unsigned c = 0; c < LG_CLASSES; ++c) maxGrid = std::max(maxGrid, gridContig[c]);
      A.G.cws        = bCws.as<uint8_t>(cwsStride * uint64_t(maxGrid));
      A.G.cws_stride = cwsStride;
      A.G.cost_bins = nullptr;
      if (contigPool && !fastIds.empty()) {
        A.G.cost_bins = bLgBins.as<uint32_t>(CK_BIN_IDS + uint64_t(CK_BINS) * fastIds.size());
        rt::dzero(A.G.cost_bins, sizeof(uint32_t) * CK_BIN_IDS);
      }
      A.G.round = A.G.last_round = 0;
      A.G.iter        = nullptr;
      A.G.parena      = nullptr;
      A.G.parena_cap  = 0;
      A.G.parena_used = nullptr;
      A.G.next_ids = A.G.next_count = A.G.cyc_ids = A.G.cyc_count = nullptr;
      A.G.rws        = nullptr;
      A.G.rws_stride = 0;
      A.G.gws        = nullptr;
      A.G.rprof      = nullptr;
      int gf = gridFast;
      if (streaming && gf >= ctx->cuCount * 2) gf -= streamFreeSlots(ctx->cuCount);
      if (!fastIds.empty()) {
        uint32_t firstWl = opt.min_word_length;
        if (!locusMinWl.empty()) {
          firstWl = 0;
          for (const uint32_t l : fastIds) firstWl = std::max(firstWl, locusMinWl[l]);
        }
        if (firstWl <= 32)
          rt::launchWG(graph_kernel<2>, gf, int(LG_WAVES), LG_BUDGET, A);
        else if (firstWl <= 64)
          rt::launchWG(graph_kernel<4>, gf, int(LG_WAVES), LG_BUDGET, A);
        else
          rt::launchWG(graph_kernel<8>, gf, int(LG_WAVES), LG_BUDGET, A);
      }
      bool smallContigsLaunched = false;
      auto launchSmallContigs   = [&] {
        if (smallContigsLaunched) return;
        smallContigsLaunched = true;
        for (unsigned c = 0; c < LG_CLASSES && !fastIds.empty(); ++c) {
          if (!classBytes[c]) continue;
          A.G.cls       = c;
          A.P.counter   = reinterpret_cast<uint32_t*>(dLg + 3) + c;
          A.P.lds_bytes = classBytes[c];
          if (c == 0 && contigPool)
            rt::launchWG(contig_pool_kernel, gridContig[c] / int(CK_POOL_WAVES), int(CK_POOL_WAVES), CK_POOL_BYTES, A);
          else
            rt::launchSingle(contig_kernel, gridContig[c], classBytes[c], A);
        }
      };
      firstRoundHookRan = false;
      if (!bigIds.empty()) {
        LgArgs B         = A;
        B.G.cost_bins    = nullptr;
        B.P.n_loci       = uint32_t(bigIds.size());
        B.P.locus_ids    = dOrder + fastIds.size();
        B.P.counter      = reinterpret_cast<uint32_t*>(dLg + 7);
        B.G.class_ids    = bLgClassIdsBig.as<uint32_t>(uint64_t(LGL_CLASSES) * bigIds.size());
        B.G.class_count  = reinterpret_cast<uint32_t*>(dLg + 5);
        B.G.class_stride = uint32_t(bigIds.size());
        for (unsigned c = 0; c < LG_CLASSES; ++c) B.G.class_bytes[c] = (c < LGL_CLASSES) ? classBytesBig[c] : 0u;
        B.G.stats        = reinterpret_cast<uint32_t*>(dLg + 11);
        int maxGridBig = 1;
        for (unsigned c = 0; c < LGL_CLASSES; ++c) maxGridBig = std::max(maxGridBig, gridContigBig[c]);
        B.G.cws        = bCwsBig.as<uint8_t>(cwsStrideBig * uint64_t(maxGridBig));
        B.G.cws_stride = cwsStrideBig;
        int gb = gridBig;
        if (streaming && gb >= ctx->cuCount) gb -= streamFreeSlots(ctx->cuCount);
        uint32_t firstWl = bigRounds ? opt.max_word_length : opt.min_word_length;
        if (!locusMinWl.empty()) {
          firstWl = 0;
          for (const uint32_t l : bigIds) firstWl = std::max(firstWl, bigRounds ? locusMaxWl[l] : locusMinWl[l]);
        }
        if (!bigRounds) {
          if (firstWl <= 80)
            rt::launchWG(graph_big_kernel<5>, gb, int(LGL_WAVES), LGL_BUDGET, B);
          else
            rt::launchWG(graph_big_kernel<8>, gb, int(LGL_WAVES), LGL_BUDGET, B);
          for (unsigned c = 0; c < LGL_CLASSES; ++c) {
            B.G.cls       = c;
            B.P.counter   = reinterpret_cast<uint32_t*>(dLg + 9) + c;
            B.P.lds_bytes = classBytesBig[c];
            rt::launchSingle(contig_big_kernel, gridContigBig[c], classBytesBig[c], B);
          }
        } else {
          uint32_t* rc = bLgRounds.as<uint32_t>(8 * (LGL_MAX_ROUNDS + 1) + 32);
          rt::dzero(rc, sizeof(uint32_t) * (8 * (LGL_MAX_ROUNDS + 1) + 32));
          uint32_t* nextBuf = bLgNext.as<uint32_t>(2 * bigIds.size());
          B.G.iter        = bLgIter.as<LgIter>(nLoci);
          B.G.parena      = bLgPseudo.as<uint32_t>(pseudoArenaDw + 64);
          B.G.parena_cap  = pseudoArenaDw;
          B.G.parena_used = reinterpret_cast<unsigned long long*>(rc + 8 * LGL_MAX_ROUNDS);
          B.G.cyc_ids     = bLgCyc.as<uint32_t>(bigIds.size());
          B.G.rws         = bRws.as<uint8_t>(rwsStride * uint64_t(gridRepeat));
          B.G.rws_stride  = rwsStride;
          B.G.gws         = bGws.as<uint8_t>(uint64_t(LGL_GWS_BYTES) * uint64_t(gridBig));
          B.G.rprof       = std::getenv("MANTA_AMD_DEBUG") ? reinterpret_cast<unsigned long long*>(rc + 8 * (LGL_MAX_ROUNDS + 1)) : nullptr;
          B.G.last_round  = bigRounds - 1;
          const int later = int(std::max<size_t>(32, bigIds.size() / 4));
          const bool oneClassLater = !(std::getenv("MANTA_AMD_BIG_ONE_CLASS") && std::atoi(std::getenv("MANTA_AMD_BIG_ONE_CLASS")) == 0);
          for (uint32_t r = 0; r < bigRounds; ++r) {
            uint32_t* cr     = rc + 8 * r;
            LgArgs    R      = B;
            R.G.round        = r;
            R.G.class_count  = cr + 1;
            R.G.cyc_count    = cr + 5;
            R.G.next_ids     = nextBuf + size_t(r & 1u) * bigIds.size();
            R.G.next_count   = cr + 7;
            R.P.counter      = cr;
            if (r > 0) {
              R.P.locus_ids  = nextBuf + size_t((r - 1) & 1u) * bigIds.size();
              R.P.n_loci     = 0;
              R.P.n_loci_dev = rc + 8 * (r - 1) + 7;
            }
            if (oneClassLater && r > 0)
              for (unsigned c = 0; c + 1 < LGL_CLASSES; ++c) R.G.class_bytes[c] = 0;
            const int gg = (r == 0) ? gb : std::min(gb, later);
            if (firstWl <= 80)
              rt::launchWG(graph_big_kernel<5>, gg, int(LGL_WAVES), LGL_BUDGET, R);
            else
              rt::launchWG(graph_big_kernel<8>, gg, int(LGL_WAVES), LGL_BUDGET, R);
            R.P.n_loci_dev = nullptr;
            R.P.counter    = cr + 6;
            R.P.lds_bytes  = RPB_LDS_BYTES;
            rt::launch(repeat_big_kernel, (r == 0) ? gridRepeat : std::min(gridRepeat, rt::roundGrid(2 * later)), RPB_LDS_BYTES, R);
            for (unsigned c = 0; c < LGL_CLASSES; ++c) {
              if (oneClassLater && r > 0 && c + 1 < LGL_CLASSES) continue;
              R.G.cls       = c;
              R.P.counter   = cr + 3 + c;
              R.P.lds_bytes = classBytesBig[c];
              rt::launchSingle(contig_big_kernel, (r == 0) ? gridContigBig[c] : std::min(gridContigBig[c], later), classBytesBig[c], R);
            }
            if (r == 0 && bigRounds > 1) {
              launchSmallContigs();
              if (afterFirstRound) {
                afterFirstRound();
                firstRoundHookRan = true;
              }
            }
          }
        }
      }
      launchSmallContigs();
      P.locus_ids  = dPunt;
      P.n_loci     = nLoci;
      P.n_loci_dev = reinterpret_cast<uint32_t*>(dCnt + 14);
      P.counter    = reinterpret_cast<uint32_t*>(dCnt + 15);
      if (nGen == 0) g = std::min(g, rt::roundGrid(std::max<int>(ctx->cuCount * 4, int(std::min<uint64_t>(bigIds.size() / 8 + 1, uint64_t(g))))));
      rt::launch(assemble_kernel, g, ASM_LDS_BYTES, P);
    } else {
      rt::launch(assemble_kernel, g, ASM_LDS_BYTES, P);
    }
    CountStatusParams C;
    C.loci    = dLoci;
    C.n_loci  = nLoci;
    C.code    = ASM_E_TABLE_FULL;
    C.counter = reinterpret_cast<unsigned long long*>(dCnt + 3);
    rt::launch(count_status_kernel, rt::roundGrid(int(std::min<uint64_t>((nLoci + 63) / 64, 64))), 0, C);
// ... 210 lines not shown
      const char* const* names = useFast ? namesLds : namesGeneral;
      uint64_t           tot = 0;
      for (int i = 0; i < 8; ++i) tot += hCnt[4 + i];
      std::fprintf(stderr, "manta_amd %s phase share (shader clocks summed over %u loci; graph_kernel: clocks of one wave of the workgroup):", useFast ? "graph_kernel + contig_kernel" : "assemble_kernel", nLoci);
      for (int i = 0; i < 8; ++i) std::fprintf(stderr, " %s=%.1f%%", names[i], tot ? 100.0 * double(hCnt[4 + i]) / double(tot) : 0.0);
      std::fprintf(stderr, " | avg clocks/locus=%.0f\n", double(tot) / nLoci);
    }
  }
  void stageOut()
  {
    stageEnqueue([] {});
    rt::sync();
    stageFinish([](bool&) {});
  }

  struct SparseContigs {
    const AsmStage* st;
    const AsmContigOut& operator()(uint32_t l, uint32_t c) const { return st->hCont[uint64_t(l) * st->opt.max_assembly_count + c]; }
  };
  void exactSizes(uint64_t& nContigs, uint64_t& seqBytes, uint64_t& bitsWords) const { exactSizes(SparseContigs{this}, nContigs, seqBytes, bitsWords); }
  template <typename ContigAt>
  void exactSizes(ContigAt contigAt, uint64_t& nContigs, uint64_t& seqBytes, uint64_t& bitsWords) const
  {
    nContigs = nContigsOut;
    seqBytes = pseudoBytesOut;
    bitsWords = pseudoCountOut;
    for (uint32_t l = 0; l < nLoci; ++l) {
      const AsmLocusOut& h(hLoci[l]);
      if (h.status != ASM_OK) continue;
      for (uint32_t c = 0; c < h.n_contigs; ++c) seqBytes += contigAt(l, c).seq_len;
      bitsWords += 2ull * h.n_words * h.n_contigs;
    }
  }

  template <typename ContigAt>
  void rangeSizes(ContigAt contigAt, uint32_t lBegin, uint32_t lEnd, uint64_t& nContigs, uint64_t& seqBytes, uint64_t& bitsWords) const
  {
    nContigs = seqBytes = bitsWords = 0;
    for (uint32_t l = lBegin; l < lEnd; ++l) {
      const AsmLocusOut& h(hLoci[l]);
      if (h.status != ASM_OK) continue;
      nContigs += h.n_contigs;
      for (uint32_t c = 0; c < h.n_contigs; ++c) seqBytes += contigAt(l, c).seq_len;
      for (uint32_t q = 0; q < h.n_pseudo; ++q) seqBytes += hBits[h.pseudo_len_off + q];
      bitsWords += 2ull * h.n_words * h.n_contigs + h.n_pseudo;
    }
  }

  void outputSizes(uint64_t& nContigs, uint64_t& seqBytes, uint64_t& bitsWords) const
  {
    uint64_t c[3];
    rt::d2h(c, dCnt, sizeof(c));
    nContigs  = uint64_t(nLoci) * opt.max_assembly_count + 1;
    seqBytes  = std::min<uint64_t>(c[1], devSeqCap) + 64;
    bitsWords = std::min<uint64_t>(c[2], devBitsCap) + 64;
  }

  int compact(
      manta_asm_locus_result_t* loci, manta_asm_contig_t* contigs, uint64_t contigs_cap, uint8_t* seq_arena,
      uint64_t seq_arena_cap, uint64_t* seq_arena_used, uint64_t* bits_arena, uint64_t bits_arena_cap, uint64_t* bits_arena_used,
      uint64_t contigBase = 0, uint64_t seqBase = 0, uint64_t bitsBase = 0)
  {
    return compact(SparseContigs{this}, loci, contigs, contigs_cap, seq_arena, seq_arena_cap, seq_arena_used, bits_arena, bits_arena_cap,
                   bits_arena_used, contigBase, seqBase, bitsBase);
  }
  template <typename ContigAt>
  int compact(
      ContigAt contigAt, manta_asm_locus_result_t* loci, manta_asm_contig_t* contigs, uint64_t contigs_cap, uint8_t* seq_arena,
      uint64_t seq_arena_cap, uint64_t* seq_arena_used, uint64_t* bits_arena, uint64_t bits_arena_cap, uint64_t* bits_arena_used,
      uint64_t contigBase, uint64_t seqBase, uint64_t bitsBase, uint32_t lBegin = 0, uint32_t lEnd = ~0u)
  {
    uint64_t seqUsed = 0, bitsUsed = 0, nContigs = 0;
    int      worst = MANTA_OK;
    lEnd           = std::min(lEnd, nLoci);
    for (uint32_t l = lBegin; l < lEnd; ++l) {
      const AsmLocusOut&        h(hLoci[l]);
      manta_asm_locus_result_t& o(loci[l]);
      std::memset(&o, 0, sizeof(o));
      o.status       = asmStatusToAbi(h.status);
      o.first_contig = uint32_t(contigBase + nContigs);
      if (o.status != MANTA_OK) {
        worst = o.status;
        if (std::getenv("MANTA_AMD_DEBUG") || std::getenv("MANTA_AMD_DEBUG_STATUS"))
          std::fprintf(stderr, "manta_amd: locus %u device status %d (k=%u iter=%u)\n", l, h.status, h.final_word_length, h.n_iterations);
        continue;
      }
      o.n_contigs         = h.n_contigs;
      o.n_words           = h.n_words;
      o.n_pseudo          = h.n_pseudo;
      o.final_word_length = h.final_word_length;
      o.n_iterations      = h.n_iterations;
      o.cyclic_iterations = h.cyclic_iterations;
      if (nContigs + h.n_contigs > contigs_cap) return fail(ctx, MANTA_E_CAPACITY, "contig array too small");
      for (uint32_t c = 0; c < h.n_contigs; ++c) {
        const AsmContigOut& hc(contigAt(l, c));
        manta_asm_contig_t& oc(contigs[nContigs++]);
        if (seqUsed + hc.seq_len > seq_arena_cap || bitsUsed + 2ull * h.n_words > bits_arena_cap)
          return fail(ctx, MANTA_E_CAPACITY, "output arena too small");
        std::memcpy(seq_arena + seqUsed, hSeq + hc.seq_off, hc.seq_len);
        std::memcpy(bits_arena + bitsUsed, hBits + hc.bits_off, sizeof(uint64_t) * 2 * h.n_words);
        oc.seq_off            = seqBase + seqUsed;
        oc.seq_len            = hc.seq_len;
        oc.support_off        = bitsBase + bitsUsed;
        oc.reject_off         = bitsBase + bitsUsed + h.n_words;
        oc.seed_read_count    = smallMode ? hc.reserved : 0u;
        oc.conservative_begin = hc.cons_begin;
        oc.conservative_end   = hc.cons_end;
        seqUsed += hc.seq_len;
        bitsUsed += 2ull * h.n_words;
      }
      uint64_t pBytes = 0;
      for (uint32_t q = 0; q < h.n_pseudo; ++q) pBytes += hBits[h.pseudo_len_off + q];
      if (seqUsed + pBytes > seq_arena_cap || bitsUsed + h.n_pseudo > bits_arena_cap)
        return fail(ctx, MANTA_E_CAPACITY, "output arena too small");
      std::memcpy(seq_arena + seqUsed, hSeq + h.pseudo_off, pBytes);
      std::memcpy(bits_arena + bitsUsed, hBits + h.pseudo_len_off, sizeof(uint64_t) * h.n_pseudo);
      o.pseudo_seq_off = seqBase + seqUsed;
      o.pseudo_len_off = bitsBase + bitsUsed;
      seqUsed += pBytes;
      bitsUsed += h.n_pseudo;
    }
    if (seq_arena_used) *seq_arena_used = seqUsed;
    if (bits_arena_used) *bits_arena_used = bitsUsed;
    if (worst != MANTA_OK) return fail(ctx, worst, "one or more loci failed; see per-locus status");
    return MANTA_OK;
  }

  int fetch(
      manta_asm_locus_result_t* loci, manta_asm_contig_t* contigs, uint64_t contigs_cap, uint8_t* seq_arena,
      uint64_t seq_arena_cap, uint64_t* seq_arena_used, uint64_t* bits_arena, uint64_t bits_arena_cap, uint64_t* bits_arena_used)
  {
    stageOut();
    return compact(loci, contigs, contigs_cap, seq_arena, seq_arena_cap, seq_arena_used, bits_arena, bits_arena_cap, bits_arena_used);
  }
};

}
using namespace manta_host;

struct manta_smallsv {
  manta_ctx_t*          ctx;
  AsmStage              asmStage;
  manta_asm_options_t   opt{};
  manta_align_scores_t  scores{};
  int32_t               largeIndel = 0;
  uint32_t              nLoci      = 0;
  uint64_t              refBytes = 0, maxRef = 0;
  bool                  uploaded = false, ran = false;
  DevBuf                dRefs, dRefOff, dCuts, dTasks, dInfo, dResults, dBucketIds, dBucketIds2, dSmall, dCigar, dTable, dPtrWs;
  rt::Event             evStart, evAsm, evSched, evAlign, refsReady;
  rt::Stream            main;
  rt::Stream            copy;
  bool                  streamUploads = false, refsOnCopy = false;
  rt::Stream            side[3];
  rt::Event             sideDone[3];
  manta_smallsv_stats_t stats{};
  DevBuf                dFirst, dPacked, dCigPacked, dPackCnt;
  PinnedBuf             pFirst, pPacked, pCig, pPackCnt;
  uint32_t*             hFirst  = nullptr;
  PackedContigOut*      hPacked = nullptr;
  uint32_t*             hCig    = nullptr;
  uint32_t*             hPackCnt = nullptr;
  uint64_t              packLast[2] = {0, 0}, packedCopied = 0, cigCopied = 0;
  PinnedBuf             pSmall;
  uint32_t              lastSmall[40] = {0};
  bool                  bucketHistory = false;
  bool                  stageBehindRun = false;
  bool                  staged = false;
  std::function<void()> whileAligning;
  rt::Event             evEarlyStaged;
  PinnedBuf             hostOff[3], hostBegin;
  explicit manta_smallsv(manta_ctx_t* c) : ctx(c), asmStage(c) {}
};


struct manta_spanning {
  manta_ctx_t*          ctx;
  AsmStage              asmStage;
  manta_asm_options_t   opt{};
  manta_align_scores_t  scores{};
  int32_t               jumpScore = 0;
  uint32_t              nLoci     = 0;
  uint64_t              ref1Bytes = 0, ref2Bytes = 0;
  bool                  uploaded = false, ran = false;
  DevBuf                dRefs1, dRef1Off, dRefs2, dRef2Off, dCuts, dTasks, dTasks2, dInfo, dResults, dResults2, dBucketIds, dBucketIds2, dSmall,
      dCigar, dPtrWs;
  rt::Event             evStart, evAsm, evSched, evAlign, refsReady;
  rt::Stream            main;
  rt::Stream            copy;
  bool                  streamUploads = false, refsOnCopy = false;
  rt::Stream            side[3];
  rt::Event             sideDone[3];
  manta_smallsv_stats_t stats{};
  DevBuf                dFirst, dPacked, dCigPacked, dPackCnt;
  PinnedBuf             pFirst, pPacked, pCig, pPackCnt;
  std::unique_ptr<rt::Stream> early;
  std::unique_ptr<rt::Stream> sideEarly[3];
  int                   sideEarlyReserved = -1;
  rt::Event             evRound0;
  DevBuf                dPassMask;
  uint32_t              earlyLoci = 0;
  std::vector<JumpCuts> hostCuts;
  uint32_t*             hFirst  = nullptr;
  PackedContigOut*      hPacked = nullptr;
  uint32_t*             hCig    = nullptr;
  uint32_t*             hPackCnt = nullptr;
  uint64_t              packLast[2] = {0, 0}, packedCopied = 0, cigCopied = 0;
  bool                  stageBehindRun = false;
  bool                  staged = false;
  std::function<void()> whileAligning;
  rt::Event             evEarlyStaged;
  PinnedBuf             hostOff[3], hostBegin;
  explicit manta_spanning(manta_ctx_t* c) : ctx(c), asmStage(c) {}
};

namespace manta_host {

template <typename Pipe>
void launchPack(Pipe* b, const AlignTaskDev* tasks, const AlignTaskDev* tasks2, const AlignResultDev* res, const AlignResultDev* res2,
                const SmallSvTaskInfo* infoSmall, const SpanTaskInfo* infoSpan, const uint32_t* cigar, uint64_t cigarCap)
{
  const uint32_t nLoci  = b->nLoci;
  const uint64_t nSlots = uint64_t(nLoci) * b->opt.max_assembly_count;
  PackParams     K;
  K.loci               = b->asmStage.dLoci;
  K.contigs            = b->asmStage.dCont;
  K.n_loci             = nLoci;
  K.max_assembly_count = b->opt.max_assembly_count;
  K.tasks              = tasks;
  K.tasks2             = tasks2;
  K.results            = res;
  K.results2           = res2;
  K.info_small         = infoSmall;
  K.info_span          = infoSpan;
  K.cigar              = cigar;
  K.first              = b->dFirst.template as<uint32_t>(nLoci);
  K.packed             = b->dPacked.template as<PackedContigOut>(nSlots);
  K.cigar_packed       = b->dCigPacked.template as<uint32_t>(cigarCap + 16);
  K.counters           = b->dPackCnt.template as<uint32_t>(4);
  rt::dzero(K.counters, 16);
  rt::launch(pack_results_kernel, rt::roundGrid(int(std::min<uint64_t>((nLoci + 63) / 64, uint64_t(std::max(1, b->ctx->cuCount * 8))))), 0, K);
}

}
using namespace manta_host;

namespace manta_host {
inline int checkPiles(manta_ctx_t* ctx, const manta_packed_piles_t* pl, const char* who)
{
  if (!pl || !pl->codes || !pl->nmask || !pl->read_len || !pl->read_code_off || !pl->read_mask_off || !pl->locus_read_begin)
    return fail(ctx, MANTA_E_INVALID_ARG, std::string(who) + ": null pointer in the packed piles");
  return MANTA_OK;
}
}
using namespace manta_host;

static const int kPipelinedAsmWavesPerCu = std::getenv("MANTA_AMD_PIPELINED_ASM_WAVES") ? std::atoi(std::getenv("MANTA_AMD_PIPELINED_ASM_WAVES")) : 12;
struct StageGates {
  std::mutex asmMu, alignMu;
};
inline std::mutex g_streamedAsmMuOfDevice[16];
inline std::mutex& streamedAsmMu(const manta_ctx_t* ctx) { return g_streamedAsmMuOfDevice[unsigned(ctx->deviceId) % 16u]; }
struct GateLock {
  std::unique_lock<std::mutex> l;
  GateLock(StageGates* g, std::mutex StageGates::*m) { if (g) l = std::unique_lock<std::mutex>(g->*m); }
  void release() { if (l.owns_lock()) l.unlock(); }
};

template <typename Pipe>
void drainCopyStream(Pipe* b) noexcept
{
  try {
    rt::ScopedStream onCopy(b->copy);
    rt::sync();
  } catch (...) {
  }
}

int smallsvRunImpl(manta_smallsv_t* b, StageGates* gates);
int spanningRunImpl(manta_spanning_t* b, StageGates* gates);

namespace manta_host {

template <typename Pipe>
void pipeStageEnqueue(Pipe* b)
{
  const uint32_t nLoci = b->nLoci;
  b->hPackCnt          = b->pPackCnt.template as<uint32_t>(4);
  b->hFirst            = b->pFirst.template as<uint32_t>(nLoci);
  auto packCopies = [&] {
        rt::d2hAsync(b->hPackCnt, b->dPackCnt.p, 16);
        rt::d2hAsync(b->hFirst, b->dFirst.p, sizeof(uint32_t) * nLoci);
        b->packedCopied = b->packLast[0] + b->packLast[0] / 4 + (b->packLast[0] ? 64 : 0);
        b->cigCopied    = b->packLast[1] + b->packLast[1] / 4 + (b->packLast[1] ? 1024 : 0);
        b->packedCopied = std::min<uint64_t>(b->packedCopied, b->dPacked.cap / sizeof(PackedContigOut));
        b->cigCopied    = std::min<uint64_t>(b->cigCopied, b->dCigPacked.cap / sizeof(uint32_t));
        b->hPacked      = b->pPacked.template as<PackedContigOut>(b->packedCopied + 1);
        b->hCig         = b->pCig.template as<uint32_t>(b->cigCopied + 1);
        rt::d2hAsync(b->hPacked, b->dPacked.p, sizeof(PackedContigOut) * b->packedCopied);
        rt::d2hAsync(b->hCig, b->dCigPacked.p, sizeof(uint32_t) * b->cigCopied);
      };
  if (b->asmStage.earlyStaged)
    b->asmStage.stageEnqueueRest(packCopies);
  else
    b->asmStage.stageEnqueue(packCopies, false);
}
// ... 212 lines not shown
```

### manta_amd/csrc/asm_contig.hpp

```cpp
#pragma once
#ifdef MANTA_WAVE_EMU
#include <map>
#include <set>
#endif
#include "asm_lds.hpp"

namespace manta_dev {

#ifndef MANTA_CK_FAST_CAP
#define MANTA_CK_FAST_CAP 3
#endif
static const unsigned CK_FAST_CAP = MANTA_CK_FAST_CAP;
static const unsigned CK_MAX_EXT = 1020;

struct CkWsLayout {
  uint64_t lane_seq, lane_bits, lane_meta, lane_log, total;
};
static const unsigned CK_SEQ_WORDS = CK_MAX_EXT / 16 + 2;
static const unsigned CK_LOG_QW    = (CK_MAX_EXT + 4) / 4;
WV_HD CkWsLayout ckWorkspaceLayout(const unsigned setw = 2)
{
  CkWsLayout L;
  uint64_t   o = 0;
  L.lane_seq  = asmPut(o, 64ull * 2 * 4 * CK_SEQ_WORDS);
// ... 1077 lines not shown
    auto chosenAt = [&](const unsigned f) { return unsigned(((f < 10) ? (chosen >> (6 * f)) : (chosenHi >> (6 * (f - 10)))) & 63u); };

    AsmLocusOut out;
    out.status            = ASM_OK;
    out.n_contigs         = finalCount;
    out.n_words           = W;
    const unsigned nP     = st ? wv::first(st->nPseudo) : 0u;
    out.n_pseudo          = nP;
    out.final_word_length = k;
    out.n_iterations      = nIter;
    out.cyclic_iterations = cycIters;
    out.reserved          = 0;
    uint64_t seqBytes = 0;
    for (unsigned f = 0; f < finalCount; ++f) seqBytes += wv::readlane(myLen, int(chosenAt(f)));
    const unsigned pLen = (lane < nP) ? unsigned(st->len[lane]) : 0u;
    {
      unsigned t = pLen;
      for (int off = 1; off < 64; off <<= 1) t += wv::shfl(t, wv::lane() ^ off);
      seqBytes += t;
    }
    const uint64_t     bitsWords = uint64_t(finalCount) * 2 * W + nP;
    unsigned long long seqBase = 0, bitsBase = 0;
    if (lane == 0) {
      seqBase  = wv::atomic_add(P.seq_used, (unsigned long long)seqBytes);
      bitsBase = wv::atomic_add(P.bits_used, (unsigned long long)bitsWords);
    }
    seqBase  = wv::readlane(uint64_t(seqBase), 0);
    bitsBase = wv::readlane(uint64_t(bitsBase), 0);
    if (seqBase + seqBytes > P.seq_cap || bitsBase + bitsWords > P.bits_cap) {
      out.status         = ASM_E_OUT_CAPACITY;
      out.n_contigs      = 0;
      out.pseudo_off     = 0;
      out.pseudo_len_off = 0;
      if (lane == 0) P.loci[locus] = out;
      return;
    }
    uint64_t        so = seqBase, bo = bitsBase;
    const uint16_t* gp = gPb();
    for (unsigned f = 0; f < finalCount; ++f) {
      const int      c   = int(chosenAt(f));
      const unsigned sl  = wv::readlane(candSlotV, c);
      const unsigned nL  = wv::readlane(nLeft, c), nR = wv::readlane(nRight, c), len = nL + k + nR;
      const unsigned seedPb = gp[slotNode[sl]];
      for (unsigned i = lane; i < len; i += 64) P.seq_arena[so + i] = uint8_t("ACGT"[contigCode(sl, nL, seedPb, i)]);
      {
        const unsigned half = lane / W, w = lane % W;
        uint64_t       mine = 0;
        for (unsigned q = 0; q < SW; ++q) {
          const uint64_t sq = wv::readlane(sup.w[q], c), rq = wv::readlane(rej.w[q], c);
          if (w == q) mine = half ? rq : sq;
        }
        if (lane < 2 * W) P.bits_arena[bo + lane] = mine;
      }
      const int cb = wv::readlane(consB, c), ce = wv::readlane(consE, c);
      if (lane == 0) {
        AsmContigOut o;
        o.seq_off    = so;
        o.bits_off   = bo;
        o.seq_len    = len;
        o.cons_begin = cb;
        o.cons_end   = int(len) - ce;
        o.reserved   = 0;
        P.contigs[size_t(locus) * P.opt.maxAssemblyCount + f] = o;
      }
      so += len;
      bo += 2 * W;
    }
    out.pseudo_off     = so;
    out.pseudo_len_off = bo;
    if (nP) {
      const uint32_t* pc = G.parena + st->off;
      unsigned        cw = 0;
      for (unsigned p = 0; p < nP; ++p) {
        const unsigned len = wv::readlane(pLen, int(p));
        for (unsigned i = lane; i < len; i += 64) P.seq_arena[so + i] = uint8_t("ACGT"[(pc[cw + (i >> 4)] >> (30 - 2 * (i & 15))) & 3u]);
        if (lane == 0) P.bits_arena[bo + p] = len;
        so += len;
        cw += (len + 15) / 16 + 1;
      }
    }
    if (lane == 0) P.loci[locus] = out;
  }

  WV_DEV int run(const unsigned locus)
  {
    tMark = wv::clock();
#ifdef MANTA_WAVE_EMU
#define CK_TRACE(why) do { if (std::getenv("MANTA_EMU_PUNT_TRACE") && lane == 0) std::fprintf(stderr, "  contig_kernel punts locus %u: %s (%u words, %u with a set, k %u)\n", locus, why, nNodes, nFat, k); } while (0)
#else
#define CK_TRACE(why) do { } while (0)
#endif
    if (!load(locus)) {
      CK_TRACE("does not fit this launch's LDS");
      if (C::BIG && lane == 0 && G.stats) wv::atomic_add(&G.stats[7], 1u);
      return CK_PUNT;
    }
    tick(4);
    if (!acyclic && !cyclic && graphHasCycle()) {
      CK_TRACE("cyclic graph");
      return CK_PUNT;
    }
    tick(3);
    loadPool();
    tick(4);
    anyRep = false;
    if ((C::BIG ? contigRoundsStretch() : contigRounds()) != 0) {
      CK_TRACE("contig too long");
      if (C::BIG && lane == 0 && G.stats) wv::atomic_add(&G.stats[7], 1u);
      return CK_PUNT;
    }
    const bool rounds = C::BIG && G.iter != nullptr;
    if (anyRep && !rounds) {
      CK_TRACE("repeat hit");
      return CK_PUNT;
    }
    const unsigned round    = rounds ? G.round : 0u;
    const unsigned nIter    = round + 1;
    const unsigned cycIters = ((round > 0) ? wv::first(G.iter[locus].cyclicIters) : 0u) + (cyclic ? 1u : 0u);
    const LgIter*  st       = (round > 0) ? &G.iter[locus] : nullptr;
    if (anyRep) {
      if (!writePseudo(locus)) {
        CK_TRACE("pseudo arena full");
        if (lane == 0 && G.stats) wv::atomic_add(&G.stats[8], 1u);
        return CK_PUNT;
      }
      st                   = &G.iter[locus];
      const unsigned maxWL = P.locus_max_wl ? P.locus_max_wl[locus] : P.opt.maxWordLength;
      if (k + P.opt.wordStepSize <= maxWL) {
        if (round >= G.last_round) {
          CK_TRACE("more word lengths than rounds");
          if (lane == 0 && G.stats) wv::atomic_add(&G.stats[9], 1u);
          return CK_PUNT;
        }
        if (lane == 0) {
          LgIter* w      = &G.iter[locus];
          w->k           = k + P.opt.wordStepSize;
          w->nIter       = nIter;
          w->cyclicIters = cycIters;
          G.next_ids[wv::atomic_add(G.next_count, 1u)] = locus;
        }
        LG_STAT(7, 1);
        return CK_NEXT;
      }
    }
    selectAndEmit(locus, st, nIter, cycIters);
    tick(7);
    LG_STAT(0, 1);
    LG_STAT(3, nCand);
    LG_STAT(6, acyclic ? 1u : 0u);
    return CK_DONE;
  }
};

template <class C>
WV_DEV void contigKernelBody(const LgArgs& A)
{
  const AsmParams& P = A.P;
  const LgParams&  G = A.G;
  uint8_t*        ws    = G.cws + uint64_t(wv::block_single()) * G.cws_stride;
  char*           lds   = wv::lds_single();
  const unsigned  nLoci = wv::first(wv::atomic_load(&G.class_count[G.cls]));
  const uint32_t* ids   = G.class_ids + size_t(G.cls) * G.class_stride;
  while (true) {
    unsigned slot = 0;
    if (wv::lane() == 0) slot = wv::atomic_add(P.counter, 1u);
    slot = wv::first(slot);
    if (slot >= nLoci) break;
    const unsigned locus = ids[slot];
    LdsContig<C>   c(P, G, lds, ws);
    const int      rc = c.run(locus);
    wv::sync();
    if (rc == CK_PUNT && wv::lane() == 0) P.punt_ids[wv::atomic_add(P.punt_count, 1u)] = locus;
    wv::sync();
  }
}
#if !MANTA_TU_DEFINES(MANTA_TU_CONTIG)
WV_KERNEL_SINGLE WV_WAVES_PER_SIMD(2) void contig_kernel(const LgArgs A);
#else
WV_KERNEL_SINGLE WV_WAVES_PER_SIMD(2) void contig_kernel(const LgArgs A)
{
  contigKernelBody<LgS>(A);
}
#endif

static const unsigned CK_POOL_WAVES = 12;
static const unsigned CK_POOL_BYTES = 163840;
static const unsigned CK_POOL_HDR   = 64;
static_assert(4 * (1 + CK_POOL_WAVES) <= CK_POOL_HDR && (CK_POOL_BYTES - CK_POOL_HDR) / 16 < 65536, "pool header");

WV_DEV unsigned ckPoolTake(char* pool, const unsigned w, const unsigned units, uint32_t* stat)
{
  uint32_t*      lock  = reinterpret_cast<uint32_t*>(pool);
  uint32_t*      share = lock + 1;
  const unsigned lane  = unsigned(wv::lane());
  const unsigned capU  = (CK_POOL_BYTES - CK_POOL_HDR) / 16;
  unsigned       polls = 0;
  while (true) {
    ++polls;
    unsigned got = 0;
    if (lane == 0) got = (wv::atomic_cas(lock, 0u, 1u) == 0u) ? 1u : 0u;
    if (wv::first(got)) {
      wv::fence_wg();
      unsigned s = 0;
      if (lane >= 1 && lane <= CK_POOL_WAVES) s = wv::atomic_load(&share[lane - 1]) >> 16;
      bool ok = lane <= CK_POOL_WAVES && s + units <= capU;
      for (unsigned v = 0; v < CK_POOL_WAVES; ++v) {
        const unsigned e = wv::atomic_load(&share[v]), a = e & 0xffffu, b = e >> 16;
        if (a < b && s < b && a < s + units) ok = false;
      }
      const uint64_t m  = wv::ballot(ok);
      const unsigned at = m ? wv::readlane(s, wv::ctz(m)) : 0u;
      if (m && lane == 0) wv::atomic_store(&share[w], at | ((at + units) << 16));
      const unsigned e        = (lane < CK_POOL_WAVES) ? wv::atomic_load(&share[lane]) : 0u;
      const bool     held     = (e & 0xffffu) < (e >> 16);
      const unsigned resident = unsigned(wv::popc(wv::ballot(held)));
      wv::fence_wg();
      if (lane == 0) wv::atomic_exch(lock, 0u);
      if (m) {
        if (stat && lane == 0) {
          wv::atomic_add(&stat[0], 1u);
          wv::atomic_add(&stat[1], resident);
          if (polls > 1) wv::atomic_add(&stat[2], 1u);
          wv::atomic_add(&stat[3], polls);
        }
        return CK_POOL_HDR + 16 * at;
      }
    }
    wv::sleep();
  }
}

template <class C>
WV_DEV void contigPoolBody(const LgArgs& A)
{
  const AsmParams& P    = A.P;
  const LgParams&  G    = A.G;
  const unsigned   w    = unsigned(wv::wave_in_wg());
  uint8_t*         ws   = G.cws + (uint64_t(wv::block_single()) * unsigned(wv::wg_waves()) + w) * G.cws_stride;
  char*            pool = wv::lds_single();
  if (w == 0 && wv::lane() <= int(CK_POOL_WAVES)) reinterpret_cast<uint32_t*>(pool)[wv::lane()] = 0u;
  wv::wg_barrier();
  const unsigned  nLoci = wv::first(wv::atomic_load(&G.class_count[G.cls]));
  const uint32_t* ids   = G.class_ids + size_t(G.cls) * G.class_stride;
  const unsigned  capU  = (P.lds_bytes + 15) / 16;
  const unsigned lane   = unsigned(wv::lane());
  unsigned       binLen = 0, binAt = 0;
  if (G.cost_bins) {
    binLen = (lane < CK_BINS) ? wv::atomic_load(&G.cost_bins[lane]) : 0u;
    binAt  = binLen;
    for (int off = 1; off < 64; off <<= 1) {
      const unsigned o = wv::shfl(binAt, int(lane) - off);
      if (int(lane) >= off) binAt += o;
    }
    binAt -= binLen;
  }
  while (true) {
    unsigned slot = 0;
    if (lane == 0) slot = wv::atomic_add(P.counter, 1u);
    slot = wv::first(slot);
    if (slot >= nLoci) break;
    unsigned locus;
    if (G.cost_bins) {
      const uint64_t inBin = wv::ballot(lane < CK_BINS && slot >= binAt && slot < binAt + binLen);
      const unsigned b     = unsigned(wv::ctz(inBin));
      locus                = G.cost_bins[CK_BIN_IDS + size_t(b) * G.class_stride + (slot - wv::readlane(binAt, int(b)))];
    } else {
      locus = ids[slot];
    }
    const LgHdr*   gh    = reinterpret_cast<const LgHdr*>(G.arena + G.slab_off[locus]);
    const unsigned needU = (wv::first(gh->need) + 15) / 16;
    const unsigned units = (needU < capU) ? needU : capU;
    char*          lds   = pool + ckPoolTake(pool, w, units, G.cost_bins ? G.cost_bins + CK_BIN_STAT : nullptr);
    LdsContig<C>   c(P, G, lds, ws);
    const int      rc = c.run(locus);
    wv::sync();
    if (wv::lane() == 0) wv::atomic_store(reinterpret_cast<uint32_t*>(pool) + 1 + w, 0u);
    if (rc == CK_PUNT && wv::lane() == 0) P.punt_ids[wv::atomic_add(P.punt_count, 1u)] = locus;
    wv::sync();
  }
}
#if !MANTA_TU_DEFINES(MANTA_TU_CONTIG)
WV_KERNEL_WG(CK_POOL_WAVES) WV_WAVES_PER_SIMD(3) void contig_pool_kernel(const LgArgs A);
#else
WV_KERNEL_WG(CK_POOL_WAVES) WV_WAVES_PER_SIMD(3) void contig_pool_kernel(const LgArgs A)
{
  contigPoolBody<LgS>(A);
}
#endif
#if !MANTA_TU_DEFINES(MANTA_TU_CONTIG)
WV_KERNEL_SINGLE WV_WAVES_PER_SIMD(1) void contig_big_kernel(const LgArgs A);
#else
WV_KERNEL_SINGLE WV_WAVES_PER_SIMD(1) void contig_big_kernel(const LgArgs A)
{
  contigKernelBody<LgL>(A);
}
#endif

}

#include "asm_lds_big.hpp"
#include "asm_repeat_big.hpp"
```

### manta_amd/csrc/asm_lds.hpp

```cpp
#pragma once
#include "assemble_kernels.hpp"

namespace manta_dev {

static const unsigned LG_SLOTS     = 2048;
static const unsigned LG_BUCKETS   = LG_SLOTS / 4;
static const unsigned LG_MAX_NODES = 1843;
static const unsigned LG_MAX_READS = 128;
static const unsigned LG_MAX_PILE  = 2046;
static const unsigned LG_EMPTY     = 0xffffffffu;
static const unsigned LG_FAT       = 0x800u;
static const unsigned LG_NO_SLOT   = 0xffffu;
static const unsigned LG_WAVES     = 8;
static const unsigned LG_BUDGET    = 81920;
static const unsigned LG_SIB_CAP   = 32;
static const unsigned LG_OVF_CAP   = 32;
static const unsigned LG_CLASSES   = 4;
static const unsigned CK_BINS     = 8;
static const unsigned CK_BIN_STAT = CK_BINS;
static const unsigned CK_BIN_IDS  = 16;

static const unsigned LG_OFF_HDR   = 0;
static const unsigned LG_OFF_RD    = 512;
static const unsigned LG_OFF_RDM   = LG_OFF_RD + 512;
static const unsigned LG_OFF_DBASE = LG_OFF_RDM + 256;
static const unsigned LG_OFF_WHIST = LG_OFF_DBASE + 1024;
static const unsigned LG_OFF_SLOTS = LG_OFF_WHIST + 1024 * LG_WAVES;
static const unsigned LG_OFF_SETS  = LG_OFF_SLOTS + 4 * LG_SLOTS;
static const unsigned LG_OFF_SORTA = LG_OFF_SETS + 16 * LG_SLOTS;
static const unsigned LG_OFF_SORTB = LG_OFF_SORTA + 2 * LG_SLOTS;
static const unsigned LG_OFF_KEYS  = LG_OFF_SORTB + 2 * LG_SLOTS;
static const unsigned LG_OFF_CNT   = LG_OFF_KEYS + 4 * LG_SLOTS;
static const unsigned LG_OFF_DYN   = LG_OFF_CNT + LG_SLOTS;
static_assert(LG_OFF_DYN + 12000 <= LG_BUDGET, "graph_kernel LDS map");
static_assert(8 * (LG_SIB_CAP + 2 * LG_OVF_CAP) + 528 <= 1024 * LG_WAVES, "side tables inside the histogram region");
static const unsigned LG_OFF_SIB   = LG_OFF_WHIST;
static const unsigned LG_OFF_SOVF  = LG_OFF_SIB + 8 * LG_SIB_CAP;
static const unsigned LG_OFF_POVF  = LG_OFF_SOVF + 8 * LG_OVF_CAP;
static const unsigned LG_OFF_CHAIN = LG_OFF_POVF + 8 * LG_OVF_CAP;
static const unsigned LG_FILTER_BITS = 16384;
static const unsigned LG_OFF_FILTER = LG_OFF_WHIST + 4096;
static const unsigned LG_OFF_PHI   = LG_OFF_SORTB;
static const unsigned LG_OFF_ANCH  = LG_OFF_DBASE;
static const unsigned LG_NO_ANCHOR = 0xffffffffu;

enum {
  LG_H_SLOT = 0,
  LG_H_FLAG = 1,
  LG_H_N    = 2,
  LG_H_NSIB = 3,
  LG_H_NSOVF = 16, LG_H_NPOVF = 17,
  LG_H_CYC  = 18,
  LG_H_PAR  = 32,
  LG_H_OFF_LO = 4,
  LG_H_OFF_HI = 5,
  LG_H_PUNT = 6,
  LG_H_TOT  = 8
};

typedef uint64_t FRec8;
struct alignas(16) FSet {
  uint64_t w[2];
};
struct alignas(16) FBucket {
  uint32_t s[4];
};

struct alignas(16) LgHdr {
  uint32_t nNodes, nFat, k, nNormal;
  uint32_t nEligible;
  uint32_t nSpec;
  uint32_t nSib, codeWords;
  uint32_t W, need;
  uint32_t nSovf, nPovf;
  uint32_t acyclic;
  uint32_t nPseudo;
  uint32_t cyclic;
  uint32_t nCore;
};
struct LgSlab {
  uint32_t recs, pool, spec, sib, sovf, povf, pb, codes, total, rd1, lex, flags;
};
WV_HD LgSlab lgSlab(const unsigned nNodes, const unsigned nFat, const unsigned codeWords)
{
  LgSlab   L;
  uint32_t o = uint32_t(sizeof(LgHdr));
  L.rd1   = 0;
  L.lex   = 0;
  L.flags = 0;
  L.recs  = o;
  o += (8u * nNodes + 15u) & ~15u;
  L.pool  = o;
  o += 16u * nFat;
  L.spec  = o;
  o += 128u;
  L.sib   = o;
  o += 8u * LG_SIB_CAP;
  L.sovf  = o;
  o += 8u * LG_OVF_CAP;
  L.povf  = o;
  o += 8u * LG_OVF_CAP;
  L.pb    = o;
  o += (2u * nNodes + 15u) & ~15u;
  L.codes = o;
  o += (4u * codeWords + 15u) & ~15u;
  L.total = o;
  return L;
}
WV_HD uint64_t lgSlabBytes(const unsigned nNodes, const unsigned nFat, const unsigned codeWords)
{
  return lgSlab(nNodes, nFat, codeWords).total;
}

static const unsigned CK_OFF_HDR    = 0;
static const unsigned CK_OFF_UNUSED = 64;
static const unsigned CK_OFF_TENT   = 320;
static const unsigned CK_OFF_SLOTND = 576;
static const unsigned CK_OFF_TBL    = 704;
static const unsigned CK_OFF_SIB    = 768;
static const unsigned CK_OFF_SOVF   = CK_OFF_SIB + 8 * LG_SIB_CAP;
static const unsigned CK_OFF_POVF   = CK_OFF_SOVF + 8 * LG_OVF_CAP;
static const unsigned CK_OFF_RECS   = CK_OFF_POVF + 8 * LG_OVF_CAP;
WV_HD unsigned ckNeed(const unsigned nNodes, const unsigned nFat, const bool acyclic)
{
  const unsigned kahn = acyclic ? 0u : ((4 * ((nNodes + 3) / 4) + 2 * nNodes + 32 + 15) & ~15u);
  const unsigned pool = 16 * (nFat ? nFat : 1u);
  return CK_OFF_RECS + ((8 * nNodes + 15) & ~15u) + ((pool > kahn) ? pool : kahn);
}

static const unsigned LGL_SLOTS     = 8192;
static const unsigned LGL_BUCKETS   = LGL_SLOTS / 4;
static const unsigned LGL_MAX_NODES = 7168;
static const unsigned LGL_MAX_READS = 256;
static const unsigned LGL_MAX_PILE  = 3598;
static const unsigned LGL_MAX_PILE_ALL = 4090;
static const unsigned LGL_POOL_CAP  = 1280;
static const unsigned LGL_POOL_OVF  = 704;
static const unsigned LGL_GWS_SETS  = 32 * LGL_POOL_OVF;
static const unsigned LGL_GWS_BYTES = LGL_GWS_SETS + 2 * 8192 + 2 * 8192;
static const unsigned LGL_WAVES     = 16;
static const unsigned LGL_BUDGET    = 163840;
static const unsigned LGL_OVF_CAP   = 128;
static const unsigned LGL_CLASSES   = 2;

struct LgS {
  static const bool     BIG       = false;
  static const unsigned ID_BITS   = 11;
  static const unsigned SETW      = 2;
  static const unsigned MAX_NODES = LG_MAX_NODES;
  static const unsigned OVF_CAP   = LG_OVF_CAP;
  static const unsigned UNUSED_DW = 64;
  static const unsigned CNT_SH = 44, FIRST_SH = 55, LAST_SH = 57, SELF_SH = 59, SOVF_SH = 60, POVF_SH = 61;
};
struct LgL {
// ... 18 lines not shown
  WV_DEV static unsigned cnt(const FRec8 w) { return unsigned(w >> C::CNT_SH) & 15u; }
  WV_DEV static unsigned firstBase(const FRec8 w) { return unsigned(w >> C::FIRST_SH) & 3u; }
  WV_DEV static unsigned lastBase(const FRec8 w) { return unsigned(w >> C::LAST_SH) & 3u; }
  WV_DEV static bool     selfLoop(const FRec8 w) { return (w >> C::SELF_SH) & 1u; }
  WV_DEV static bool     sOvf(const FRec8 w) { return (w >> C::SOVF_SH) & 1u; }
  WV_DEV static bool     pOvf(const FRec8 w) { return (w >> C::POVF_SH) & 1u; }
  WV_DEV static uint64_t links(const FRec8 w, const unsigned nd, const bool succ, const uint16_t* ovf, const unsigned nOvf)
  {
    uint64_t l = (succ ? w : (w >> (2 * C::ID_BITS))) & M2;
    if (succ ? sOvf(w) : pOvf(w)) {
      if (C::BIG) {
        const unsigned e = unsigned(l >> C::ID_BITS) & IDM;
        l = (l & IDM) | (uint64_t(ovf[4 * e]) << C::ID_BITS) | (uint64_t(ovf[4 * e + 1]) << (2 * C::ID_BITS)) | (uint64_t(ovf[4 * e + 2]) << (3 * C::ID_BITS));
      } else {
        for (unsigned e = 0; e < nOvf; ++e)
          if (unsigned(ovf[4 * e]) == nd) l |= (uint64_t(ovf[4 * e + 1]) << 22) | (uint64_t(ovf[4 * e + 2]) << 33);
      }
    }
    return l;
  }
  WV_DEV static unsigned linkField(const uint64_t l, const unsigned c) { return unsigned(l >> (C::ID_BITS * c)) & IDM; }
  WV_DEV static unsigned linkId(const uint64_t l, const unsigned c)
  {
    const unsigned f = linkField(l, c);
    return f ? f - 1 : ASM_NONE;
  }
};

WV_HD LgSlab lgSlabL(const unsigned nNodes, const unsigned nFat, const unsigned codeWords)
{
  LgSlab   L;
  uint32_t o = uint32_t(sizeof(LgHdr));
  L.recs  = o;
  o += (8u * nNodes + 15u) & ~15u;
  L.pool  = o;
  o += 32u * nFat;
  L.spec  = o;
  o += 128u;
  L.sib   = o;
  o += 8u * LG_SIB_CAP;
  L.sovf  = o;
  o += 8u * LGL_OVF_CAP;
  L.povf  = o;
  o += 8u * LGL_OVF_CAP;
  L.rd1   = o;
  o += (nNodes + 15u) & ~15u;
  L.pb    = o;
  o += (2u * nNodes + 15u) & ~15u;
  L.codes = o;
  o += (4u * codeWords + 15u) & ~15u;
  L.lex   = o;
  o += (2u * nNodes + 15u) & ~15u;
  L.flags = o;
  o += 8u * 256u;
  L.total = o;
  return L;
}
template <class C>
WV_HD LgSlab lgSlabOf(const unsigned nNodes, const unsigned nFat, const unsigned codeWords)
{
  return C::BIG ? lgSlabL(nNodes, nFat, codeWords) : lgSlab(nNodes, nFat, codeWords);
}

#ifndef MANTA_STRETCH_WIN
#define MANTA_STRETCH_WIN 4
#endif
static const unsigned LGL_STRETCH_WIN = MANTA_STRETCH_WIN;
template <class C>
struct CkMap {
  static const unsigned UNUSED = 64;
  static const unsigned TENT   = UNUSED + 4 * C::UNUSED_DW;
  static const unsigned SLOTND = TENT + (C::BIG ? 2 * 64 * LGL_STRETCH_WIN : 256);
  static const unsigned TBL    = SLOTND + 128;
  static const unsigned SIB    = TBL + 64;
  static const unsigned SOVF   = SIB + 8 * LG_SIB_CAP;
  static const unsigned POVF   = SOVF + 8 * C::OVF_CAP;
  static const unsigned RECS   = POVF + 8 * C::OVF_CAP;
};
static_assert(CkMap<LgS>::TENT == CK_OFF_TENT && CkMap<LgS>::SLOTND == CK_OFF_SLOTND && CkMap<LgS>::TBL == CK_OFF_TBL && CkMap<LgS>::SIB == CK_OFF_SIB &&
              CkMap<LgS>::RECS == CK_OFF_RECS, "the small class keeps its map");
template <class C>
WV_HD unsigned ckNeedOf(const unsigned nNodes, const unsigned nFat, const bool acyclic)
{
  const unsigned kahn = acyclic ? 0u : ((4 * ((nNodes + 3) / 4) + 2 * nNodes + 32 + 15) & ~15u);
  const unsigned pool = 8 * C::SETW * (nFat ? nFat : 1u);
  return CkMap<C>::RECS + ((8 * nNodes + 15) & ~15u) + (C::BIG ? ((nNodes + 15) & ~15u) : 0u) + ((pool > kahn) ? pool : kahn);
}

static const unsigned LGL_CORE_CAP = 4096;
template <class C>
WV_HD unsigned ckCyclicExtra(const unsigned nCore)
{
  return 4u * C::UNUSED_DW + 2u * C::UNUSED_DW + 4u * C::UNUSED_DW + 64u * 4u * ((nCore + 31u) / 32u);
}
template <class C>
WV_HD unsigned ckNeedCyclic(const unsigned nNodes, const unsigned nFat, const unsigned nCore)
{
  const unsigned pool = 8 * C::SETW * (nFat ? nFat : 1u);
  return CkMap<C>::RECS + ((8 * nNodes + 15) & ~15u) + (C::BIG ? ((nNodes + 15) & ~15u) : 0u) + pool + ckCyclicExtra<C>(nCore);
}

static const unsigned LGL_MAX_PSEUDO = 40;
static const unsigned LGL_MAX_ROUNDS = 24;
struct alignas(16) LgIter {
  uint32_t k;
  uint32_t nIter;
  uint32_t cyclicIters;
  uint32_t nPseudo;
  uint64_t off;
  uint32_t codeWords;
  uint32_t slabCap;
  uint16_t len[LGL_MAX_PSEUDO];
};

struct LgParams;
struct LgArgs;
struct LgParams {
  uint8_t*            arena;
  uint64_t            arena_cap;
  unsigned long long* arena_used;
  uint64_t*           slab_off;
  uint32_t*           class_ids;
  uint32_t*           class_count;
  uint32_t            class_stride;
  uint32_t            class_bytes[LG_CLASSES];
  uint32_t            cls;
  uint32_t            flags;
  uint32_t*           stats;
  uint8_t*            cws;
  uint32_t*           cost_bins;
  uint64_t            cws_stride;
  uint32_t            round;
  uint32_t            last_round;
  LgIter*             iter;
  uint32_t*           parena;
  uint64_t            parena_cap;
  unsigned long long* parena_used;
  uint32_t*           next_ids;
  uint32_t*           next_count;
  uint32_t*           cyc_ids;
  uint32_t*           cyc_count;
  uint8_t*            rws;
  uint64_t            rws_stride;
  uint8_t*            gws;
  unsigned long long* rprof;
};

static const uint32_t LG_FLAG_NO_PROOF = 1u;
static const uint32_t LG_FLAG_NO_RESCUE = 2u;

struct LgArgs {
  AsmParams P;
  LgParams  G;
};

#ifdef MANTA_WAVE_EMU
inline unsigned long long* fastStats()
{
  static unsigned long long v[8] = {0, 0, 0, 0, 0, 0, 0, 0};
  return v;
}
#define LG_STAT(i, n) do { if (wv::lane() == 0) fastStats()[i] += (n); } while (0)
#else
#define LG_STAT(i, n) do { } while (0)
#endif

WV_DEV unsigned lg8Succ(const FRec8 w, const unsigned i) { return unsigned(w >> (11 * i)) & 0x7ffu; }
WV_DEV unsigned lg8Pred(const FRec8 w, const unsigned i) { return unsigned(w >> (22 + 11 * i)) & 0x7ffu; }
WV_DEV unsigned lg8Cnt(const FRec8 w) { return unsigned(w >> 44) & 15u; }
WV_DEV unsigned lg8Read(const FRec8 w) { return unsigned(w >> 48) & 0x7fu; }
WV_DEV unsigned lg8FirstBase(const FRec8 w) { return unsigned(w >> 55) & 3u; }
WV_DEV unsigned lg8LastBase(const FRec8 w) { return unsigned(w >> 57) & 3u; }
WV_DEV bool     lg8SelfLoop(const FRec8 w) { return (w >> 59) & 1u; }
WV_DEV bool     lg8SOvf(const FRec8 w) { return (w >> 60) & 1u; }
WV_DEV bool     lg8POvf(const FRec8 w) { return (w >> 61) & 1u; }
static const uint64_t LG_M22 = (uint64_t(1) << 22) - 1;
static const uint64_t LG_M44 = (uint64_t(1) << 44) - 1;
WV_DEV uint64_t lg8Links(const FRec8 w, const unsigned nd, const bool succ, const uint16_t* ovf, const unsigned nOvf)
{
  uint64_t l = (succ ? w : (w >> 22)) & LG_M22;
  if (succ ? lg8SOvf(w) : lg8POvf(w)) {
    for (unsigned e = 0; e < nOvf; ++e)
      if (unsigned(ovf[4 * e]) == nd) l |= (uint64_t(ovf[4 * e + 1]) << 22) | (uint64_t(ovf[4 * e + 2]) << 33);
  }
  return l;
}
WV_DEV unsigned lgLinkId(const uint64_t w, const unsigned c)
{
  const unsigned f = unsigned(w >> (11 * c)) & 0x7ffu;
  return f ? f - 1 : ASM_NONE;
}

struct LdsGraph {
  const AsmParams& P;
  const LgParams&  G;
  char*            lds;
  unsigned         tw, tn, lane;
  uint32_t *       hdr, *rd, *dbase, *whist, *slots, *keyArr, *codes, *nmask;
  uint16_t *       rdm, *sortA, *sortB, *slotId;
  uint8_t*         cntArr;
  FSet*            sets;
  FRec8*           nodes;
  uint64_t*        pred4;
  int16_t*         phi;
  int16_t*         roff;
  uint32_t*        filter;
  unsigned         nNormal, W, k, nNodes, nFat, nEligible, lowTier, codeWords;
  uint64_t         tMark;

  WV_DEV LdsGraph(const AsmParams& p, const LgParams& g, char* base) : P(p), G(g), lds(base)
  {
    tw     = unsigned(wv::wave_in_wg());
    tn     = unsigned(wv::wg_waves());
    lane   = unsigned(wv::lane());
    hdr    = reinterpret_cast<uint32_t*>(lds + LG_OFF_HDR);
    rd     = reinterpret_cast<uint32_t*>(lds + LG_OFF_RD);
    rdm    = reinterpret_cast<uint16_t*>(lds + LG_OFF_RDM);
    dbase  = reinterpret_cast<uint32_t*>(lds + LG_OFF_DBASE);
    whist  = reinterpret_cast<uint32_t*>(lds + LG_OFF_WHIST);
    slots  = reinterpret_cast<uint32_t*>(lds + LG_OFF_SLOTS);
    sets   = reinterpret_cast<FSet*>(lds + LG_OFF_SETS);
    nodes  = reinterpret_cast<FRec8*>(lds + LG_OFF_SETS);
    pred4  = reinterpret_cast<uint64_t*>(lds + LG_OFF_SETS) + LG_SLOTS;
    phi    = reinterpret_cast<int16_t*>(lds + LG_OFF_PHI);
    roff   = reinterpret_cast<int16_t*>(lds + LG_OFF_RDM);
    filter = reinterpret_cast<uint32_t*>(lds + LG_OFF_FILTER);
    sortA  = reinterpret_cast<uint16_t*>(lds + LG_OFF_SORTA);
    sortB  = reinterpret_cast<uint16_t*>(lds + LG_OFF_SORTB);
    keyArr = reinterpret_cast<uint32_t*>(lds + LG_OFF_KEYS);
    slotId = reinterpret_cast<uint16_t*>(lds + LG_OFF_KEYS);
    cntArr = reinterpret_cast<uint8_t*>(lds + LG_OFF_CNT);
    codes  = reinterpret_cast<uint32_t*>(lds + LG_OFF_DYN);
    nmask  = codes;
  }

  WV_DEV void tick(const int phase, const int fine)
  {
#ifdef MANTA_ASM_PROFILE
    const uint64_t now = wv::clock();
#ifdef MANTA_LG_PROFILE_GRAPH
    const int slot = fine;
#else
    const int slot = phase;
#endif
    if (P.phase_cycles && tw == 0 && lane == 0) wv::atomic_add(&P.phase_cycles[slot], (unsigned long long)(now - tMark));
    tMark = now;
#else
    (void)phase;
    (void)fine;
#endif
  }

  WV_DEV void teamSync() const
  {
    wv::sync();
    wv::wg_barrier();
  }
  WV_DEV unsigned tid() const { return 64 * tw + lane; }
  WV_DEV unsigned nThreads() const { return 64 * tn; }

  template <int KW>
  WV_DEV Key<KW> keyAt(const unsigned pb) const
  {
    Key<KW>        key;
    const unsigned kw = (k + 15) >> 4;
    const unsigned wi = pb >> 4, sh = (pb & 15) * 2;
    uint32_t       raw[KW + 1];
    for (int i = 0; i <= KW; ++i) raw[i] = (unsigned(i) <= kw) ? codes[wi + i] : 0u;
    for (int i = 0; i < KW; ++i) {
      uint32_t v = 0;
      if (unsigned(i) < kw) {
        v                   = uint32_t((((uint64_t(raw[i]) << 32) | raw[i + 1]) << sh) >> 32);
        const unsigned have = k - 16u * unsigned(i);
        if (have < 16) v &= ~((1u << (32 - 2 * have)) - 1u);
      }
      key.w[i] = v;
    }
    return key;
  }
  template <int KW>
  WV_DEV static bool keyEq(const Key<KW>& a, const Key<KW>& b)
  {
    bool eq = true;
    for (int i = 0; i < KW; ++i) eq = eq && (a.w[i] == b.w[i]);
    return eq;
  }
  template <int KW>
  WV_DEV static bool keyLess(const Key<KW>& a, const Key<KW>& b)
  {
    for (int i = 0; i < KW; ++i)
      if (a.w[i] != b.w[i]) return a.w[i] < b.w[i];
    return false;
  }
  template <int KW>
  WV_DEV void keySetBase(Key<KW>& key, const unsigned i, const unsigned c) const
  {
    const unsigned sh = 30 - 2 * (i & 15);
    for (int w = 0; w < KW; ++w)
      if (unsigned(w) == (i >> 4)) key.w[w] = (key.w[w] & ~(3u << sh)) | (c << sh);
  }
  template <int KW>
  WV_DEV Key<KW> keyShiftAppend(const Key<KW>& key, const unsigned c) const
  {
    Key<KW> r;
    for (int w = 0; w < KW; ++w) r.w[w] = (key.w[w] << 2) | ((w + 1 < KW) ? (key.w[w + 1] >> 30) : 0u);
    keySetBase(r, k - 1, c);
// ... 989 lines not shown
```

### manta_amd/csrc/pipeline_kernels.hpp

```cpp
#pragma once
#include "align_kernels.hpp"
#include "assemble_kernels.hpp"

namespace manta_dev {

static const int      SMALLSV_MER       = 10;
static const unsigned SCHED_TABLE_BYTES = 4096;
static const unsigned SCHED_SEQ_BYTES   = 6144;
static const unsigned SCHED_LDS_BYTES   = SCHED_TABLE_BYTES + SCHED_SEQ_BYTES + 1024;

struct SmallSvCuts {
  int32_t leadingCut, trailingCut, maxLeadingCut, maxTrailingCut;
};

struct SmallSvTaskInfo {
  int32_t status;
  int32_t adj_leading_cut, adj_trailing_cut;
  int32_t bucket;
};

struct ScheduleParams {
  const AsmLocusOut*  loci;
  const AsmContigOut* contigs;
  const uint8_t*      seq_arena;
  uint32_t            n_loci;
  uint32_t            max_assembly_count;
  const uint8_t*     refs;
  const uint64_t*    ref_off;
  const SmallSvCuts* cuts;
  AlignTaskDev*    tasks;
  SmallSvTaskInfo* info;
  uint32_t*        bucket_ids;
  uint32_t*        bucket_count;
  uint32_t*        bucket_maxref;
  unsigned long long* cigar_used;
  uint64_t         cigar_cap;
  uint32_t*        counter;
  uint32_t* table_ws;
  uint32_t  table_cap;
  uint32_t e_set[16];
  uint32_t n_e;
  uint32_t chunk;
};

WV_DEV unsigned merCode(const uint8_t* p, bool& valid)
{
  unsigned code = 0;
  valid         = true;
  for (int i = 0; i < SMALLSV_MER; ++i) {
    const unsigned c = baseCode(p[i]);
    if (c > 3) valid = false;
    code = (code << 2) | (c & 3u);
  }
  return code;
}

static const int MER_BATCH = 55;
WV_DEV unsigned merLoadBase(const uint8_t* seq, const int len, const int p0)
{
  const int pos = p0 + wv::lane();
  return (pos >= 0 && pos < len) ? baseCode(seq[pos]) : 4u;
}
WV_DEV unsigned merCodesFromBase(const unsigned c, bool& valid)
{
  const int      l   = wv::lane();
  unsigned bad = (c > 3) ? 1u : 0u;
  unsigned w1  = c & 3u;
  const unsigned w2 = (w1 << 2) | wv::shfl(w1, (l + 1) & 63);
  const unsigned b2 = bad | wv::shfl(bad, (l + 1) & 63);
  const unsigned w4 = (w2 << 4) | wv::shfl(w2, (l + 2) & 63);
  const unsigned b4 = b2 | wv::shfl(b2, (l + 2) & 63);
  const unsigned w8 = (w4 << 8) | wv::shfl(w4, (l + 4) & 63);
  const unsigned b8 = b4 | wv::shfl(b4, (l + 4) & 63);
  const unsigned w10 = (w8 << 4) | wv::shfl(w2, (l + 8) & 63);
  const unsigned b10 = b8 | wv::shfl(b2, (l + 8) & 63);
  valid = (l < MER_BATCH) && (b10 == 0);
  return w10;
}
WV_DEV unsigned merCodes55(const uint8_t* seq, const int len, const int p0, bool& valid)
{
  return merCodesFromBase(merLoadBase(seq, len, p0), valid);
}

WV_DEV bool merLookup(const uint32_t* table, const unsigned mask, const unsigned code)
{
  unsigned s = (code * 2654435761u) & mask;
  while (true) {
    const uint32_t v = table[s];
    if (v == 0) return false;
    if (v == code + 1) return true;
    s = (s + 1) & mask;
  }
}

WV_DEV SmallSvTaskInfo scheduleSlot(const ScheduleParams& P, const unsigned slot, const unsigned total, uint32_t* ltable, uint32_t* gtable)
{
  const unsigned    lane  = unsigned(wv::lane());
  const unsigned    locus = slot / P.max_assembly_count, ci = slot % P.max_assembly_count;
  const AsmLocusOut lo    = P.loci[locus];
  SmallSvTaskInfo   info  = {0, 0, 0, -1};
  if (lo.status != ASM_OK || ci >= lo.n_contigs) {
    info.status = (lo.status != ASM_OK) ? 1 : 0;
    return info;
  }
  const AsmContigOut co      = P.contigs[slot];
  const uint8_t*     contigG = P.seq_arena + co.seq_off;
  const unsigned     clen    = co.seq_len;
  const uint8_t*     refG    = P.refs + P.ref_off[locus];
  const int          refSize = int(P.ref_off[locus + 1] - P.ref_off[locus]);
  const SmallSvCuts  cuts    = P.cuts[locus];
  const uint8_t* contig = contigG;
  const uint8_t* ref    = refG;
  {
    uint8_t* const  lseq = reinterpret_cast<uint8_t*>(ltable) + SCHED_TABLE_BYTES;
    const uintptr_t gc = reinterpret_cast<uintptr_t>(contigG), gr = reinterpret_cast<uintptr_t>(refG);
    const unsigned  leadC = unsigned(gc & 15), leadR = unsigned(gr & 15);
    const unsigned  bytesC = (leadC + clen + 15) & ~15u, bytesR = (leadR + unsigned(refSize > 0 ? refSize : 0) + 15) & ~15u;
    if (bytesC + bytesR <= SCHED_SEQ_BYTES) {
      const u32x4* sc = reinterpret_cast<const u32x4*>(gc - leadC);
      const u32x4* sr = reinterpret_cast<const u32x4*>(gr - leadR);
      u32x4*       dc = reinterpret_cast<u32x4*>(lseq);
      u32x4*       dr = reinterpret_cast<u32x4*>(lseq + bytesC);
      for (unsigned i = lane; i < bytesC / 16; i += 64) dc[i] = sc[i];
      for (unsigned i = lane; i < bytesR / 16; i += 64) dr[i] = sr[i];
      wv::sync();
      contig = lseq + leadC;
      ref    = lseq + bytesC + leadR;
    }
  }

  if (clen < unsigned(SMALLSV_MER) || 2 * clen > P.table_cap) {
    info.status = 2;
    return info;
  }
  unsigned tcap = 64;
  while (tcap < 2 * clen) tcap <<= 1;
  const unsigned mask  = tcap - 1;
  uint32_t*      table = (tcap * 4 <= SCHED_TABLE_BYTES) ? ltable : gtable;
  for (unsigned i = lane; i < tcap; i += 64) table[i] = 0;
  wv::sync();
  for (int p0 = 0; p0 + SMALLSV_MER <= int(clen); p0 += MER_BATCH) {
    bool           valid;
    const unsigned code = merCodes55(contig, int(clen), p0, valid);
    if (!valid) continue;
    unsigned s = (code * 2654435761u) & mask;
    while (true) {
      const uint32_t old = wv::atomic_cas(&table[s], 0u, code + 1);
      if (old == 0 || old == code + 1) break;
      s = (s + 1) & mask;
    }
  }
  wv::sync();
  if (table == gtable) wv::fence_acquire();

  const int minRefIndex    = cuts.leadingCut;
  const int maxRefIndex    = refSize - (cuts.trailingCut + SMALLSV_MER);
  const int maxFwdRefIndex = (cuts.maxLeadingCut < maxRefIndex) ? cuts.maxLeadingCut : maxRefIndex;
  int adjLead = maxFwdRefIndex + 1;
  if (adjLead < minRefIndex) adjLead = minRefIndex;
  const int minRevRefIndex = (minRefIndex > refSize - cuts.maxTrailingCut) ? minRefIndex : (refSize - cuts.maxTrailingCut);
  int       revIndex       = minRevRefIndex - 1;
  if (revIndex > maxRefIndex) revIndex = maxRefIndex;
  {
    int  fBase = minRefIndex, bTop = maxRefIndex;
    bool fDone = fBase > maxFwdRefIndex, bDone = bTop < minRevRefIndex;
    while (!fDone || !bDone) {
      const int      bBase = bTop - (MER_BATCH - 1);
      const unsigned cf = merLoadBase(ref, refSize, fDone ? -1000 : fBase), cb = merLoadBase(ref, refSize, bDone ? -1000 : bBase);
      bool           vf, vb;
      const unsigned codeF = merCodesFromBase(cf, vf), codeB = merCodesFromBase(cb, vb);
      const int      iF = fBase + int(lane), iB = bBase + int(lane);
      const bool     hitF = !fDone && vf && iF <= maxFwdRefIndex && merLookup(table, mask, codeF);
      const bool     hitB = !bDone && vb && iB >= minRevRefIndex && iB <= bTop && merLookup(table, mask, codeB);
      const uint64_t mF = wv::ballot(hitF), mB = wv::ballot(hitB);
      if (!fDone) {
        if (mF) {
          adjLead = fBase + wv::ctz(mF);
          fDone   = true;
        } else {
          fBase += MER_BATCH;
          fDone = fBase > maxFwdRefIndex;
        }
      }
      if (!bDone) {
        if (mB) {
          revIndex = bBase + (63 - wv::clz(mB));
          bDone    = true;
        } else {
          bTop -= MER_BATCH;
          bDone = bTop < minRevRefIndex;
        }
      }
    }
  }
  const int adjTrail = refSize - (revIndex + SMALLSV_MER);
  const int winLen   = refSize - adjLead - adjTrail;
  info.adj_leading_cut  = adjLead;
  info.adj_trailing_cut = adjTrail;
  if (winLen <= 0 || adjLead < 0 || adjTrail < 0) {
    info.status = 3;
    return info;
  }
  int            bucket = -1;
  const unsigned need   = (clen + 63) / 64;
  for (unsigned b = 0; b < P.n_e; ++b)
    if (P.e_set[b] >= need) {
      bucket = int(b);
      break;
    }
  if (bucket < 0) bucket = int(P.n_e) - 1;
  const unsigned long long cig = 8ull * co.seq_off;
  if (cig + 4ull * clen + 16 > P.cigar_cap) {
    info.status = 5;
    return info;
  }
  if (lane == 0) {
    AlignTaskDev t;
    t.query     = contigG;
    t.ref1      = refG + adjLead;
    t.ref2      = nullptr;
    t.query_len = clen;
    t.ref1_len  = unsigned(winLen);
    t.ref2_len  = 0;
    t.cigar_off = uint32_t(cig);
    P.tasks[slot] = t;
  }
  info.bucket = bucket;
  return info;
}

static const unsigned SCHED_PEND = 8;
struct SchedPending {
  uint32_t count[16];
  uint32_t maxref[16];
  uint32_t slot[16][SCHED_PEND];
  uint32_t cigarWords;
};
WV_DEV void schedFlush(const ScheduleParams& P, SchedPending* pend, const unsigned bucket, const unsigned total)
{
  const unsigned n = pend->count[bucket];
  if (n == 0) return;
  unsigned pos = 0;
  if (wv::lane() == 0) {
    pos = wv::atomic_add(&P.bucket_count[bucket], n);
    unsigned cur = wv::atomic_load(&P.bucket_maxref[bucket]);
    const unsigned want = pend->maxref[bucket];
    while (cur < want) {
      const unsigned old = wv::atomic_cas(&P.bucket_maxref[bucket], cur, want);
      if (old == cur) break;
      cur = old;
    }
  }
  pos = wv::first(pos);
  if (unsigned(wv::lane()) < n) P.bucket_ids[size_t(bucket) * total + pos + unsigned(wv::lane())] = pend->slot[bucket][wv::lane()];
  wv::sync();
  if (wv::lane() == 0) {
    pend->count[bucket]  = 0;
    pend->maxref[bucket] = 0;
  }
  wv::sync();
}

#if !MANTA_TU_DEFINES(MANTA_TU_GLUE)
WV_KERNEL void smallsv_schedule_kernel(const ScheduleParams P);
#else
WV_KERNEL void smallsv_schedule_kernel(const ScheduleParams P)
{
  const unsigned lane   = unsigned(wv::lane());
  uint32_t*      gtable = P.table_ws + size_t(wv::block()) * P.table_cap;
  uint32_t*      ltable = reinterpret_cast<uint32_t*>(wv::lds(SCHED_LDS_BYTES));
  SchedPending*  pend   = reinterpret_cast<SchedPending*>(reinterpret_cast<char*>(ltable) + SCHED_TABLE_BYTES + SCHED_SEQ_BYTES);
  const unsigned total  = P.n_loci * P.max_assembly_count;
  if (lane < 16) {
    pend->count[lane]  = 0;
    pend->maxref[lane] = 0;
  }
  if (lane == 0) pend->cigarWords = 0;
  wv::sync();
  while (true) {
    unsigned base = 0;
    if (lane == 0) base = wv::atomic_add(P.counter, P.chunk);
    base = wv::first(base);
    if (base >= P.n_loci) break;
    const unsigned end = (base + P.chunk < P.n_loci) ? base + P.chunk : P.n_loci;
    for (unsigned locus = base; locus < end; ++locus) {
      const AsmLocusOut lo       = P.loci[locus];
      const unsigned    nContigs = (lo.status == ASM_OK) ? lo.n_contigs : 0u;
      if (lane >= nContigs && lane < P.max_assembly_count) {
        SmallSvTaskInfo none = {(lo.status != ASM_OK) ? 1 : 0, 0, 0, -1};
        P.info[locus * P.max_assembly_count + lane] = none;
      }
      for (unsigned ci = 0; ci < nContigs; ++ci) {
        const unsigned        slot = locus * P.max_assembly_count + ci;
        const SmallSvTaskInfo info = scheduleSlot(P, slot, total, ltable, gtable);
        wv::sync();
        if (lane == 0) P.info[slot] = info;
        if (info.bucket >= 0) {
          const unsigned b = unsigned(info.bucket);
          if (lane == 0) {
            const AlignTaskDev& t = P.tasks[slot];
            const unsigned slabLen = unsigned(alignSlabRefLen(1, int(P.e_set[b]), t.query_len, t.ref1_len));
            pend->slot[b][pend->count[b]] = slot;
            pend->count[b] += 1;
            pend->cigarWords += 4 * t.query_len + 16;
            if (slabLen > pend->maxref[b]) pend->maxref[b] = slabLen;
          }
          wv::sync();
          if (pend->count[b] == SCHED_PEND) schedFlush(P, pend, b, total);
        }
        wv::sync();
      }
    }
  }
  for (unsigned b = 0; b < P.n_e; ++b) schedFlush(P, pend, b, total);
  if (lane == 0 && pend->cigarWords) wv::atomic_add(P.cigar_used, (unsigned long long)pend->cigarWords);
}
#endif

static const unsigned BS_CLASSES = 512;
static const unsigned BS_WAVES   = 16;
static const unsigned BS_LDS_BYTES = 4 * (BS_WAVES * BS_CLASSES + BS_CLASSES + 8);
struct BucketSortParams {
  const AlignTaskDev*    tasks;
  const AsmLocusOut*     loci;
  const SmallSvTaskInfo* info;
  uint32_t*              ids_out;
  uint32_t               n_loci, max_assembly_count;
  uint32_t               total;
  uint32_t               mask;
};
#if !MANTA_TU_DEFINES(MANTA_TU_GLUE)
WV_KERNEL_WG(16) void bucket_sort_kernel(const BucketSortParams P);
#else
WV_KERNEL_WG(16) void bucket_sort_kernel(const BucketSortParams P)
{
  const unsigned b = unsigned(wv::block_single());
  if (!((P.mask >> b) & 1u)) return;
  uint32_t*      hist  = reinterpret_cast<uint32_t*>(wv::lds_single());
  uint32_t*      dbase = hist + BS_WAVES * BS_CLASSES;
  const unsigned tw = unsigned(wv::wave_in_wg()), tn = unsigned(wv::wg_waves()), lane = unsigned(wv::lane());
  const unsigned tid = 64 * tw + lane, nt = 64 * tn;
  uint32_t*      out    = P.ids_out + size_t(b) * P.total;
  uint32_t*      myHist = hist + BS_CLASSES * tw;
  const unsigned chunk  = (((P.n_loci + tn - 1) / tn) + 63) & ~63u;
  const unsigned c0 = chunk * tw, c1 = (c0 + chunk < P.n_loci) ? (c0 + chunk) : P.n_loci;
  auto cls = [&](const unsigned id) {
    const unsigned c = P.tasks[id].ref1_len >> 3;
    return (BS_CLASSES - 1) - ((c < BS_CLASSES - 1) ? c : (BS_CLASSES - 1));
  };
  auto contigsOf = [&](const unsigned locus) -> unsigned {
    if (locus >= c1) return 0u;
    const AsmLocusOut lo = P.loci[locus];
    return (lo.status == ASM_OK) ? lo.n_contigs : 0u;
  };
  for (unsigned i = tid; i < BS_WAVES * BS_CLASSES + BS_CLASSES; i += nt) hist[i] = 0;
  wv::sync();
  wv::wg_barrier();
  for (unsigned i0 = c0; i0 < c1; i0 += 64) {
    const unsigned locus = i0 + lane, n = contigsOf(locus);
    for (unsigned ci = 0; ci < n; ++ci) {
      const unsigned slot = locus * P.max_assembly_count + ci;
      if (P.info[slot].bucket == int(b)) wv::atomic_add(&myHist[cls(slot)], 1u);
    }
  }
  wv::sync();
  wv::wg_barrier();
  for (unsigned d = tid; d < BS_CLASSES; d += nt) {
    unsigned run = 0;
    for (unsigned w = 0; w < BS_WAVES; ++w) {
      const unsigned c          = (w < tn) ? hist[BS_CLASSES * w + d] : 0u;
      hist[BS_CLASSES * w + d] = run;
      run += c;
    }
    dbase[d] = run;
  }
  wv::sync();
  wv::wg_barrier();
  if (tw == 0) {
    unsigned v[8], sum = 0;
    for (int j = 0; j < 8; ++j) {
      v[j] = dbase[8 * lane + j];
      sum += v[j];
    }
    unsigned inc = sum;
    for (int off = 1; off < 64; off <<= 1) {
      const unsigned o = wv::shfl(inc, int(lane) - off);
      if (int(lane) >= off) inc += o;
    }
    unsigned run = inc - sum;
    for (int j = 0; j < 8; ++j) {
      dbase[8 * lane + j] = run;
      run += v[j];
    }
  }
  wv::sync();
  wv::wg_barrier();
  for (unsigned i0 = c0; i0 < c1; i0 += 64) {
    const unsigned locus = i0 + lane, n = contigsOf(locus);
    unsigned       nMax  = n;
    for (int off = 32; off > 0; off >>= 1) {
      const unsigned o = wv::shfl(nMax, int(lane) ^ off);
      nMax             = (o > nMax) ? o : nMax;
    }
    for (unsigned ci = 0; ci < nMax; ++ci) {
      const unsigned slot  = locus * P.max_assembly_count + ci;
      const bool     valid = ci < n && P.info[slot].bucket == int(b);
      const unsigned d     = valid ? cls(slot) : 0u;
      uint64_t       peers = wv::ballot(valid);
      for (int bit = 0; bit < 9; ++bit) {
        const bool     on = (d >> bit) & 1u;
        const uint64_t m  = wv::ballot(valid && on);
        peers &= on ? m : ~m;
      }
      unsigned base = 0;
      if (valid) base = dbase[d] + myHist[d];
      wv::sync();
      if (valid) {
        out[base + unsigned(wv::popc(peers & ((uint64_t(1) << lane) - 1)))] = slot;
        if ((peers >> lane) == 1u) myHist[d] += unsigned(wv::popc(peers));
      }
      wv::sync();
    }
  }
}
#endif

struct JumpCuts {
  int32_t a1Lead, a1Trail, a2Lead, a2Trail;
};

struct SpanTaskInfo {
  int32_t status;
  int32_t bucket;
  int32_t bucket2;
  int32_t is_uncut;
};

struct SpanParams {
  const AsmLocusOut*  loci;
  const AsmContigOut* contigs;
  const uint8_t*      seq_arena;
  uint32_t            n_loci, max_assembly_count;
  const uint8_t*      refs1;
  const uint64_t*     ref1_off;
  const uint8_t*      refs2;
  const uint64_t*     ref2_off;
  const JumpCuts*     cuts;
  AlignTaskDev*       tasks;
  AlignTaskDev*       tasks2;
  SpanTaskInfo*       info;
  uint32_t*           bucket_ids;
  uint32_t*           bucket_count;
  uint32_t*           bucket_maxref;
  uint32_t*           bucket_ids2;
  uint32_t*           bucket_count2;
  uint32_t*           bucket_maxref2;
  unsigned long long* cigar_used;
  uint64_t            cigar_cap;
  const AlignResultDev* results;
  const uint32_t*       cigar;
  uint32_t            e_set[16];
  uint32_t            n_e;
  const uint8_t*      pass_mask;
  uint32_t            pass_value;
};

struct SpanMarkParams {
  const AsmLocusOut* loci;
// ... 247 lines not shown
```

Before: 1.212 million loci/s.

## Fuse small-SV alignment scheduling into the contig assembly kernel epilogue

Each contig kernel wave now runs the per-locus 10-mer trim and bucket scheduling right after finishing a locus, while the contig data is still hot and the LDS is free. It uses per-wave pending buffers and an epoch flag to check that the reference upload has landed. The standalone schedule kernel still runs with a larger chunk and skips loci already marked as scheduled. The goal is to overlap scheduling with assembly and shrink the separate scheduling pass, at the cost of extra LDS and register pressure in the contig kernels, plus a cigar-cap check that is deferred (set to unlimited during fusion).

Measured after the change: 1.211 million loci/s. Within noise of the previous version (-0.1%).

```diff
diff --git a/include/manta_amd.h b/include/manta_amd.h
--- a/include/manta_amd.h
+++ b/include/manta_amd.h
@@ -145,6 +145,7 @@
                          const manta_ref_cuts_t* cuts);
 int manta_smallsv_run(manta_smallsv_t* b);
 int manta_smallsv_stats(const manta_smallsv_t* b, manta_smallsv_stats_t* stats);
+int manta_debug_smallsv_schedule(manta_smallsv_t* b, int32_t* info, uint32_t* bucket_count, uint32_t* bucket_ids, uint8_t* scheduled);
 int manta_smallsv_output_sizes(const manta_smallsv_t* b, uint64_t* contigs, uint64_t* seq_bytes, uint64_t* bits_words,
                                uint64_t* cigar_words);
 int manta_smallsv_download(manta_smallsv_t* b, manta_asm_locus_result_t* loci, manta_asm_contig_t* contigs,
diff --git a/manta_amd/csrc/api.cpp b/manta_amd/csrc/api.cpp
--- a/manta_amd/csrc/api.cpp
+++ b/manta_amd/csrc/api.cpp
@@ -443,6 +443,8 @@
       rt::h2d(dRefOff, ref_off, sizeof(uint64_t) * (n_loci + 1));
       rt::h2d(dCuts, cuts, sizeof(SmallSvCuts) * n_loci);
       b->refsReady.record();
+      b->refsEpochHost = ++b->refsEpoch;
+      if (!rt::streamWrite32(b->asmStage.refsLandedFlag(), b->refsEpoch)) rt::h2d(b->asmStage.refsLandedFlag(), &b->refsEpochHost, sizeof(uint32_t));
     } else {
       rt::h2d(dRefs, refs, b->refBytes);
       rt::h2d(dRefOff, ref_off, sizeof(uint64_t) * (n_loci + 1));
@@ -497,6 +499,8 @@
       rt::h2d(dRefOff, ref_off, sizeof(uint64_t) * (n_loci + 1));
       rt::h2d(dCuts, cuts, sizeof(SmallSvCuts) * n_loci);
       b->refsReady.record();
+      b->refsEpochHost = ++b->refsEpoch;
+      if (!rt::streamWrite32(b->asmStage.refsLandedFlag(), b->refsEpoch)) rt::h2d(b->asmStage.refsLandedFlag(), &b->refsEpochHost, sizeof(uint32_t));
     } else {
       b->asmStage.uploadPiles(*piles);
       rt::h2d(dRefs, refs, b->refBytes);
@@ -532,11 +536,41 @@
     uint32_t*        dSmall   = b->dSmall.as<uint32_t>(64);
     const uint32_t   tableCap = nextPow2(2ull * as.maxContigLen);
     const int        schedWaves = std::getenv("MANTA_AMD_SCHED_WAVES_PER_CU") ? std::max(1, std::atoi(std::getenv("MANTA_AMD_SCHED_WAVES_PER_CU"))) : 12;
-    const uint32_t   schedChunk = std::getenv("MANTA_AMD_SCHED_CHUNK") ? uint32_t(std::max(1, std::atoi(std::getenv("MANTA_AMD_SCHED_CHUNK")))) : 2u;
+    const bool       fusedSched = !std::getenv("MANTA_AMD_NO_FUSED_SCHEDULE");
+    const uint32_t   schedChunk = std::getenv("MANTA_AMD_SCHED_CHUNK") ? uint32_t(std::min(64, std::max(1, std::atoi(std::getenv("MANTA_AMD_SCHED_CHUNK"))))) : (fusedSched ? 64u : 2u);
     const int        schedGrid = rt::roundGrid(int(std::min<uint64_t>((nLoci + schedChunk - 1) / schedChunk, uint64_t(std::max(1, ctx->cuCount * schedWaves)))));
     uint32_t*        dTable   = b->dTable.as<uint32_t>(uint64_t(tableCap) * schedGrid);
+    uint8_t*         dScheduled = fusedSched ? b->dScheduled.as<uint8_t>(nLoci) : nullptr;
     rt::dzero(dSmall, sizeof(uint32_t) * 64);
     rt::dzero(dResults, sizeof(AlignResultDev) * nSlots);
+    if (dScheduled) rt::dzero(dScheduled, nLoci);
+    b->lastRunFused = fusedSched;
+    ScheduleParams S;
+    S.loci               = as.dLoci;
+    S.contigs            = as.dCont;
+    S.seq_arena          = as.dSeq;
+    S.n_loci             = nLoci;
+    S.max_assembly_count = maxAsm;
+    S.refs               = static_cast<const uint8_t*>(b->dRefs.p);
+    S.ref_off            = static_cast<const uint64_t*>(b->dRefOff.p);
+    S.cuts               = static_cast<const SmallSvCuts*>(b->dCuts.p);
+    S.tasks              = dTasks;
+    S.info               = dInfo;
+    S.bucket_ids         = dBuckets;
+    S.bucket_count       = dSmall;
+    S.bucket_maxref      = dSmall + 16;
+    S.cigar_used         = reinterpret_cast<unsigned long long*>(dSmall + 34);
+    S.cigar_cap          = ~uint64_t(0);
+    S.counter            = dSmall + 32;
+    S.table_ws           = dTable;
+    S.table_cap          = tableCap;
+    S.n_e                = kNumESet;
+    S.chunk              = schedChunk;
+    for (int i = 0; i < 16; ++i) S.e_set[i] = (i < kNumESet) ? uint32_t(kESet[i]) : 0u;
+    S.scheduled          = dScheduled;
+    S.refs_ready         = (fusedSched && b->refsOnCopy) ? as.refsLandedFlag() : nullptr;
+    S.refs_epoch         = b->refsEpoch;
+    S.reserved           = 0;
 
     const bool dbg = std::getenv("MANTA_AMD_DEBUG") != nullptr;
     auto       stage = [&](const char* what) {
@@ -554,7 +588,9 @@
       as.stageQueued = false;
       as.earlyStaged = false;
       b->evStart.record();
+      as.fuseSched = fusedSched ? &S : nullptr;
       as.launch();
+      as.fuseSched = nullptr;
       b->evAsm.record();
       rt::d2h(asmCnt, as.dCnt, sizeof(asmCnt));
       if (asmCnt[3]) {
@@ -574,28 +610,7 @@
     GateLock alignOnly(gates, &StageGates::alignMu);
     if (b->refsOnCopy) rt::curStreamWaits(b->refsReady);
 
-    ScheduleParams S;
-    S.loci               = as.dLoci;
-    S.contigs            = as.dCont;
-    S.seq_arena          = as.dSeq;
-    S.n_loci             = nLoci;
-    S.max_assembly_count = maxAsm;
-    S.refs               = static_cast<const uint8_t*>(b->dRefs.p);
-    S.ref_off            = static_cast<const uint64_t*>(b->dRefOff.p);
-    S.cuts               = static_cast<const SmallSvCuts*>(b->dCuts.p);
-    S.tasks              = dTasks;
-    S.info               = dInfo;
-    S.bucket_ids         = dBuckets;
-    S.bucket_count       = dSmall;
-    S.bucket_maxref      = dSmall + 16;
-    S.cigar_used         = reinterpret_cast<unsigned long long*>(dSmall + 34);
-    S.cigar_cap          = cigarCap;
-    S.counter            = dSmall + 32;
-    S.table_ws           = dTable;
-    S.table_cap          = tableCap;
-    S.n_e                = kNumESet;
-    S.chunk              = schedChunk;
-    for (int i = 0; i < kNumESet; ++i) S.e_set[i] = uint32_t(kESet[i]);
+    S.cigar_cap = cigarCap;
     rt::launch(smallsv_schedule_kernel, schedGrid, SCHED_LDS_BYTES, S);
     uint32_t  pairMask       = 0;
     uint32_t* dBucketsSorted = nullptr;
@@ -618,6 +633,13 @@
     }
     b->evSched.record();
     stage("scheduled");
+    if (dbg && dScheduled) {
+      std::vector<uint8_t> done(nLoci);
+      rt::d2h(done.data(), dScheduled, nLoci);
+      uint32_t n = 0;
+      for (const uint8_t d : done) n += d ? 1u : 0u;
+      std::fprintf(stderr, "manta_amd: fused schedule: %u of %u loci in the contig stage's epilogue, %u in smallsv_schedule_kernel\n", n, nLoci, nLoci - n);
+    }
 
     uint32_t hSmall[40];
     const int    maxWaves = std::max(1, ctx->cuCount * alignWavesPerCu());
@@ -828,6 +850,30 @@
   if (!b || !stats) return MANTA_E_INVALID_ARG;
   *stats = b->stats;
   return MANTA_OK;
+}
+
+int manta_debug_smallsv_schedule(manta_smallsv_t* b, int32_t* info, uint32_t* bucket_count, uint32_t* bucket_ids, uint8_t* scheduled)
+{
+  if (!b || !info || !bucket_count || !bucket_ids) return MANTA_E_INVALID_ARG;
+  if (!b->ran) return fail(b->ctx, MANTA_E_INVALID_ARG, "manta_debug_smallsv_schedule: run first");
+  try {
+    rt::setDevice(b->ctx->deviceId);
+    rt::ScopedStream onStream(b->main);
+    const uint64_t nSlots = uint64_t(b->nLoci) * b->opt.max_assembly_count;
+    static_assert(sizeof(SmallSvTaskInfo) == 4 * sizeof(int32_t), "task info layout");
+    rt::d2h(info, b->dInfo.p, sizeof(SmallSvTaskInfo) * nSlots);
+    std::memset(bucket_count, 0, sizeof(uint32_t) * 16);
+    rt::d2h(bucket_count, b->dSmall.p, sizeof(uint32_t) * kNumESet);
+    std::memset(bucket_ids, 0, sizeof(uint32_t) * 16 * nSlots);
+    rt::d2h(bucket_ids, b->dBucketIds.p, sizeof(uint32_t) * kNumESet * nSlots);
+    if (scheduled) {
+      std::memset(scheduled, 0, b->nLoci);
+      if (b->lastRunFused) rt::d2h(scheduled, b->dScheduled.p, b->nLoci);
+    }
+    return MANTA_OK;
+  } catch (const std::exception& e) {
+    return fail(b->ctx, MANTA_E_HIP, e.what());
+  }
 }
 
 int manta_smallsv_output_sizes(const manta_smallsv_t* b, uint64_t* contigs, uint64_t* seq_bytes, uint64_t* bits_words, uint64_t* cigar_words)
diff --git a/manta_amd/csrc/api_internal.hpp b/manta_amd/csrc/api_internal.hpp
--- a/manta_amd/csrc/api_internal.hpp
+++ b/manta_amd/csrc/api_internal.hpp
@@ -486,6 +486,8 @@
   int                   gridFast = 1;
   int                   gridContig[manta_dev::LG_CLASSES] = {0, 0, 0, 0};
   bool                  contigPool = false;
+  const manta_dev::ScheduleParams* fuseSched = nullptr;
+  DevBuf                bSched, bSchedPend;
   uint32_t              classBytes[manta_dev::LG_CLASSES] = {0, 0, 0, 0};
   uint64_t              lgArenaCap = 0, cwsStride = 0;
   std::vector<uint32_t> fastIds, genIds;
@@ -868,9 +870,13 @@
     L.hostBegin[L.nChunks] = read_off[locus_read_begin[n]];
     return L;
   }
+  uint32_t* refsLandedFlag() const { return dChunksDone ? dChunksDone + 8 : nullptr; }
   void resetChunkCounter(rt::Stream& copyStream)
   {
-    if (!dChunksDone) dChunksDone = static_cast<uint32_t*>(rt::dmallocFine(64));
+    if (!dChunksDone) {
+      dChunksDone = static_cast<uint32_t*>(rt::dmallocFine(64));
+      rt::dzero(dChunksDone, 64);
+    }
     uint32_t* ids = pChunkIds.as<uint32_t>(kStreamChunks + 1);
     for (uint32_t c = 0; c <= kStreamChunks; ++c) ids[c] = c;
     {
@@ -952,7 +958,10 @@
     upload(nullptr, nullptr, pl.locus_read_begin);
     dPlShift = bPlShift.as<uint64_t>(3 * kStreamChunks);
     rt::h2d(dPlShift, shifts.data(), sizeof(uint64_t) * 3 * kStreamChunks);
-    if (!dChunksDone) dChunksDone = static_cast<uint32_t*>(rt::dmallocFine(64));
+    if (!dChunksDone) {
+      dChunksDone = static_cast<uint32_t*>(rt::dmallocFine(64));
+      rt::dzero(dChunksDone, 64);
+    }
     uint32_t* ids = pChunkIds.as<uint32_t>(kStreamChunks + 1);
     for (uint32_t c = 0; c <= kStreamChunks; ++c) ids[c] = c;
     {
@@ -1128,6 +1137,14 @@
       for (unsigned c = 0; c < LG_CLASSES; ++c) maxGrid = std::max(maxGrid, gridContig[c]);
       A.G.cws        = bCws.as<uint8_t>(cwsStride * uint64_t(maxGrid));
       A.G.cws_stride = cwsStride;
+      A.sched = nullptr;
+      A.sched_pend = nullptr;
+      if (fuseSched) {
+        ScheduleParams* dSched = bSched.as<ScheduleParams>(1);
+        rt::h2d(dSched, fuseSched, sizeof(ScheduleParams));
+        A.sched      = dSched;
+        A.sched_pend = bSchedPend.as<SchedPending>(uint64_t(maxGrid));
+      }
       A.G.cost_bins = nullptr;
       if (contigPool && !fastIds.empty()) {
         A.G.cost_bins = bLgBins.as<uint32_t>(CK_BIN_IDS + uint64_t(CK_BINS) * fastIds.size());
@@ -1644,6 +1661,9 @@
   rt::Stream            main;
   rt::Stream            copy;
   bool                  streamUploads = false, refsOnCopy = false;
+  uint32_t              refsEpoch = 0, refsEpochHost = 0;
+  bool                  lastRunFused = false;
+  DevBuf                dScheduled;
   rt::Stream            side[3];
   rt::Event             sideDone[3];
   manta_smallsv_stats_t stats{};
diff --git a/manta_amd/csrc/asm_contig.hpp b/manta_amd/csrc/asm_contig.hpp
--- a/manta_amd/csrc/asm_contig.hpp
+++ b/manta_amd/csrc/asm_contig.hpp
@@ -1253,6 +1253,11 @@
   }
 };
 
+WV_DEV_CALL void ckScheduleEpilogue(const ScheduleParams& S, const unsigned locus, char* lds, const unsigned ldsBytes, SchedPending* pend)
+{
+  scheduleEpilogue(S, locus, lds, ldsBytes, pend);
+}
+
 template <class C>
 WV_DEV void contigKernelBody(const LgArgs& A)
 {
@@ -1262,18 +1267,26 @@
   char*           lds   = wv::lds_single();
   const unsigned  nLoci = wv::first(wv::atomic_load(&G.class_count[G.cls]));
   const uint32_t* ids   = G.class_ids + size_t(G.cls) * G.class_stride;
+  const bool          fused = !C::BIG && A.sched != nullptr;
+  SchedPending* const pend  = fused ? A.sched_pend + wv::block_single() : nullptr;
+  if (fused) schedPendingInit(pend);
   while (true) {
     unsigned slot = 0;
     if (wv::lane() == 0) slot = wv::atomic_add(P.counter, 1u);
     slot = wv::first(slot);
     if (slot >= nLoci) break;
     const unsigned locus = ids[slot];
-    LdsContig<C>   c(P, G, lds, ws);
-    const int      rc = c.run(locus);
+    int            rc;
+    {
+      LdsContig<C> c(P, G, lds, ws);
+      rc = c.run(locus);
+    }
     wv::sync();
+    if (fused && rc == CK_DONE) ckScheduleEpilogue(*A.sched, locus, lds, P.lds_bytes, pend);
     if (rc == CK_PUNT && wv::lane() == 0) P.punt_ids[wv::atomic_add(P.punt_count, 1u)] = locus;
     wv::sync();
   }
+  if (fused) schedPendingDrain(*A.sched, pend, A.sched->n_loci * A.sched->max_assembly_count);
 }
 #if !MANTA_TU_DEFINES(MANTA_TU_CONTIG)
 WV_KERNEL_SINGLE WV_WAVES_PER_SIMD(2) void contig_kernel(const LgArgs A);
@@ -1355,6 +1368,9 @@
     }
     binAt -= binLen;
   }
+  const bool          fused = A.sched != nullptr;
+  SchedPending* const pend  = fused ? A.sched_pend + (size_t(wv::block_single()) * unsigned(wv::wg_waves()) + w) : nullptr;
+  if (fused) schedPendingInit(pend);
   while (true) {
     unsigned slot = 0;
     if (lane == 0) slot = wv::atomic_add(P.counter, 1u);
@@ -1372,13 +1388,19 @@
     const unsigned needU = (wv::first(gh->need) + 15) / 16;
     const unsigned units = (needU < capU) ? needU : capU;
     char*          lds   = pool + ckPoolTake(pool, w, units, G.cost_bins ? G.cost_bins + CK_BIN_STAT : nullptr);
-    LdsContig<C>   c(P, G, lds, ws);
-    const int      rc = c.run(locus);
+    int            rc;
+    {
+      LdsContig<C> c(P, G, lds, ws);
+      rc = c.run(locus);
+    }
+    wv::sync();
+    if (fused && rc == CK_DONE) ckScheduleEpilogue(*A.sched, locus, lds, 16 * units, pend);
     wv::sync();
     if (wv::lane() == 0) wv::atomic_store(reinterpret_cast<uint32_t*>(pool) + 1 + w, 0u);
     if (rc == CK_PUNT && wv::lane() == 0) P.punt_ids[wv::atomic_add(P.punt_count, 1u)] = locus;
     wv::sync();
   }
+  if (fused) schedPendingDrain(*A.sched, pend, A.sched->n_loci * A.sched->max_assembly_count);
 }
 #if !MANTA_TU_DEFINES(MANTA_TU_CONTIG)
 WV_KERNEL_WG(CK_POOL_WAVES) WV_WAVES_PER_SIMD(3) void contig_pool_kernel(const LgArgs A);
diff --git a/manta_amd/csrc/asm_lds.hpp b/manta_amd/csrc/asm_lds.hpp
--- a/manta_amd/csrc/asm_lds.hpp
+++ b/manta_amd/csrc/asm_lds.hpp
@@ -1,5 +1,6 @@
 #pragma once
 #include "assemble_kernels.hpp"
+#include "schedule_slot.hpp"
 
 namespace manta_dev {
 
@@ -324,6 +325,8 @@
 struct LgArgs {
   AsmParams P;
   LgParams  G;
+  const ScheduleParams* sched;
+  SchedPending*  sched_pend;
 };
 
 #ifdef MANTA_WAVE_EMU
diff --git a/manta_amd/csrc/pipeline_kernels.hpp b/manta_amd/csrc/pipeline_kernels.hpp
--- a/manta_amd/csrc/pipeline_kernels.hpp
+++ b/manta_amd/csrc/pipeline_kernels.hpp
@@ -1,265 +1,7 @@
 #pragma once
-#include "align_kernels.hpp"
-#include "assemble_kernels.hpp"
+#include "schedule_slot.hpp"
 
 namespace manta_dev {
-
-static const int      SMALLSV_MER       = 10;
-static const unsigned SCHED_TABLE_BYTES = 4096;
-static const unsigned SCHED_SEQ_BYTES   = 6144;
-static const unsigned SCHED_LDS_BYTES   = SCHED_TABLE_BYTES + SCHED_SEQ_BYTES + 1024;
-
-struct SmallSvCuts {
-  int32_t leadingCut, trailingCut, maxLeadingCut, maxTrailingCut;
-};
-
-struct SmallSvTaskInfo {
-  int32_t status;
-  int32_t adj_leading_cut, adj_trailing_cut;
-  int32_t bucket;
-};
-
-struct ScheduleParams {
-  const AsmLocusOut*  loci;
-  const AsmContigOut* contigs;
-  const uint8_t*      seq_arena;
-  uint32_t            n_loci;
-  uint32_t            max_assembly_count;
-  const uint8_t*     refs;
-  const uint64_t*    ref_off;
-  const SmallSvCuts* cuts;
-  AlignTaskDev*    tasks;
-  SmallSvTaskInfo* info;
-  uint32_t*        bucket_ids;
-  uint32_t*        bucket_count;
-  uint32_t*        bucket_maxref;
-  unsigned long long* cigar_used;
-  uint64_t         cigar_cap;
-  uint32_t*        counter;
-  uint32_t* table_ws;
-  uint32_t  table_cap;
-  uint32_t e_set[16];
-  uint32_t n_e;
-  uint32_t chunk;
-};
-
-WV_DEV unsigned merCode(const uint8_t* p, bool& valid)
-{
-  unsigned code = 0;
-  valid         = true;
-  for (int i = 0; i < SMALLSV_MER; ++i) {
-    const unsigned c = baseCode(p[i]);
-    if (c > 3) valid = false;
-    code = (code << 2) | (c & 3u);
-  }
-  return code;
-}
-
-static const int MER_BATCH = 55;
-WV_DEV unsigned merLoadBase(const uint8_t* seq, const int len, const int p0)
-{
-  const int pos = p0 + wv::lane();
-  return (pos >= 0 && pos < len) ? baseCode(seq[pos]) : 4u;
-}
-WV_DEV unsigned merCodesFromBase(const unsigned c, bool& valid)
-{
-  const int      l   = wv::lane();
-  unsigned bad = (c > 3) ? 1u : 0u;
-  unsigned w1  = c & 3u;
-  const unsigned w2 = (w1 << 2) | wv::shfl(w1, (l + 1) & 63);
-  const unsigned b2 = bad | wv::shfl(bad, (l + 1) & 63);
-  const unsigned w4 = (w2 << 4) | wv::shfl(w2, (l + 2) & 63);
-  const unsigned b4 = b2 | wv::shfl(b2, (l + 2) & 63);
-  const unsigned w8 = (w4 << 8) | wv::shfl(w4, (l + 4) & 63);
-  const unsigned b8 = b4 | wv::shfl(b4, (l + 4) & 63);
-  const unsigned w10 = (w8 << 4) | wv::shfl(w2, (l + 8) & 63);
-  const unsigned b10 = b8 | wv::shfl(b2, (l + 8) & 63);
-  valid = (l < MER_BATCH) && (b10 == 0);
-  return w10;
-}
-WV_DEV unsigned merCodes55(const uint8_t* seq, const int len, const int p0, bool& valid)
-{
-  return merCodesFromBase(merLoadBase(seq, len, p0), valid);
-}
-
-WV_DEV bool merLookup(const uint32_t* table, const unsigned mask, const unsigned code)
-{
-  unsigned s = (code * 2654435761u) & mask;
-  while (true) {
-    const uint32_t v = table[s];
-    if (v == 0) return false;
-    if (v == code + 1) return true;
-    s = (s + 1) & mask;
-  }
-}
-
-WV_DEV SmallSvTaskInfo scheduleSlot(const ScheduleParams& P, const unsigned slot, const unsigned total, uint32_t* ltable, uint32_t* gtable)
-{
-  const unsigned    lane  = unsigned(wv::lane());
-  const unsigned    locus = slot / P.max_assembly_count, ci = slot % P.max_assembly_count;
-  const AsmLocusOut lo    = P.loci[locus];
-  SmallSvTaskInfo   info  = {0, 0, 0, -1};
-  if (lo.status != ASM_OK || ci >= lo.n_contigs) {
-    info.status = (lo.status != ASM_OK) ? 1 : 0;
-    return info;
-  }
-  const AsmContigOut co      = P.contigs[slot];
-  const uint8_t*     contigG = P.seq_arena + co.seq_off;
-  const unsigned     clen    = co.seq_len;
-  const uint8_t*     refG    = P.refs + P.ref_off[locus];
-  const int          refSize = int(P.ref_off[locus + 1] - P.ref_off[locus]);
-  const SmallSvCuts  cuts    = P.cuts[locus];
-  const uint8_t* contig = contigG;
-  const uint8_t* ref    = refG;
-  {
-    uint8_t* const  lseq = reinterpret_cast<uint8_t*>(ltable) + SCHED_TABLE_BYTES;
-    const uintptr_t gc = reinterpret_cast<uintptr_t>(contigG), gr = reinterpret_cast<uintptr_t>(refG);
-    const unsigned  leadC = unsigned(gc & 15), leadR = unsigned(gr & 15);
-    const unsigned  bytesC = (leadC + clen + 15) & ~15u, bytesR = (leadR + unsigned(refSize > 0 ? refSize : 0) + 15) & ~15u;
-    if (bytesC + bytesR <= SCHED_SEQ_BYTES) {
-      const u32x4* sc = reinterpret_cast<const u32x4*>(gc - leadC);
-      const u32x4* sr = reinterpret_cast<const u32x4*>(gr - leadR);
-      u32x4*       dc = reinterpret_cast<u32x4*>(lseq);
-      u32x4*       dr = reinterpret_cast<u32x4*>(lseq + bytesC);
-      for (unsigned i = lane; i < bytesC / 16; i += 64) dc[i] = sc[i];
-      for (unsigned i = lane; i < bytesR / 16; i += 64) dr[i] = sr[i];
-      wv::sync();
-      contig = lseq + leadC;
-      ref    = lseq + bytesC + leadR;
-    }
-  }
-
-  if (clen < unsigned(SMALLSV_MER) || 2 * clen > P.table_cap) {
-    info.status = 2;
-    return info;
-  }
-  unsigned tcap = 64;
-  while (tcap < 2 * clen) tcap <<= 1;
-  const unsigned mask  = tcap - 1;
-  uint32_t*      table = (tcap * 4 <= SCHED_TABLE_BYTES) ? ltable : gtable;
-  for (unsigned i = lane; i < tcap; i += 64) table[i] = 0;
-  wv::sync();
-  for (int p0 = 0; p0 + SMALLSV_MER <= int(clen); p0 += MER_BATCH) {
-    bool           valid;
-    const unsigned code = merCodes55(contig, int(clen), p0, valid);
-    if (!valid) continue;
-    unsigned s = (code * 2654435761u) & mask;
-    while (true) {
-      const uint32_t old = wv::atomic_cas(&table[s], 0u, code + 1);
-      if (old == 0 || old == code + 1) break;
-      s = (s + 1) & mask;
-    }
-  }
-  wv::sync();
-  if (table == gtable) wv::fence_acquire();
-
-  const int minRefIndex    = cuts.leadingCut;
-  const int maxRefIndex    = refSize - (cuts.trailingCut + SMALLSV_MER);
-  const int maxFwdRefIndex = (cuts.maxLeadingCut < maxRefIndex) ? cuts.maxLeadingCut : maxRefIndex;
-  int adjLead = maxFwdRefIndex + 1;
-  if (adjLead < minRefIndex) adjLead = minRefIndex;
-  const int minRevRefIndex = (minRefIndex > refSize - cuts.maxTrailingCut) ? minRefIndex : (refSize - cuts.maxTrailingCut);
-  int       revIndex       = minRevRefIndex - 1;
-  if (revIndex > maxRefIndex) revIndex = maxRefIndex;
-  {
-    int  fBase = minRefIndex, bTop = maxRefIndex;
-    bool fDone = fBase > maxFwdRefIndex, bDone = bTop < minRevRefIndex;
-    while (!fDone || !bDone) {
-      const int      bBase = bTop - (MER_BATCH - 1);
-      const unsigned cf = merLoadBase(ref, refSize, fDone ? -1000 : fBase), cb = merLoadBase(ref, refSize, bDone ? -1000 : bBase);
-      bool           vf, vb;
-      const unsigned codeF = merCodesFromBase(cf, vf), codeB = merCodesFromBase(cb, vb);
-      const int      iF = fBase + int(lane), iB = bBase + int(lane);
-      const bool     hitF = !fDone && vf && iF <= maxFwdRefIndex && merLookup(table, mask, codeF);
-      const bool     hitB = !bDone && vb && iB >= minRevRefIndex && iB <= bTop && merLookup(table, mask, codeB);
-      const uint64_t mF = wv::ballot(hitF), mB = wv::ballot(hitB);
-      if (!fDone) {
-        if (mF) {
-          adjLead = fBase + wv::ctz(mF);
-          fDone   = true;
-        } else {
-          fBase += MER_BATCH;
-          fDone = fBase > maxFwdRefIndex;
-        }
-      }
-      if (!bDone) {
-        if (mB) {
-          revIndex = bBase + (63 - wv::clz(mB));
-          bDone    = true;
-        } else {
-          bTop -= MER_BATCH;
-          bDone = bTop < minRevRefIndex;
-        }
-      }
-    }
-  }
-  const int adjTrail = refSize - (revIndex + SMALLSV_MER);
-  const int winLen   = refSize - adjLead - adjTrail;
-  info.adj_leading_cut  = adjLead;
-  info.adj_trailing_cut = adjTrail;
-  if (winLen <= 0 || adjLead < 0 || adjTrail < 0) {
-    info.status = 3;
-    return info;
-  }
-  int            bucket = -1;
-  const unsigned need   = (clen + 63) / 64;
-  for (unsigned b = 0; b < P.n_e; ++b)
-    if (P.e_set[b] >= need) {
-      bucket = int(b);
-      break;
-    }
-  if (bucket < 0) bucket = int(P.n_e) - 1;
-  const unsigned long long cig = 8ull * co.seq_off;
-  if (cig + 4ull * clen + 16 > P.cigar_cap) {
-    info.status = 5;
-    return info;
-  }
-  if (lane == 0) {
-    AlignTaskDev t;
-    t.query     = contigG;
-    t.ref1      = refG + adjLead;
-    t.ref2      = nullptr;
-    t.query_len = clen;
-    t.ref1_len  = unsigned(winLen);
-    t.ref2_len  = 0;
-    t.cigar_off = uint32_t(cig);
-    P.tasks[slot] = t;
-  }
-  info.bucket = bucket;
-  return info;
-}
-
-static const unsigned SCHED_PEND = 8;
-struct SchedPending {
-  uint32_t count[16];
-  uint32_t maxref[16];
-  uint32_t slot[16][SCHED_PEND];
-  uint32_t cigarWords;
-};
-WV_DEV void schedFlush(const ScheduleParams& P, SchedPending* pend, const unsigned bucket, const unsigned total)
-{
-  const unsigned n = pend->count[bucket];
-  if (n == 0) return;
-  unsigned pos = 0;
-  if (wv::lane() == 0) {
-    pos = wv::atomic_add(&P.bucket_count[bucket], n);
-    unsigned cur = wv::atomic_load(&P.bucket_maxref[bucket]);
-    const unsigned want = pend->maxref[bucket];
-    while (cur < want) {
-      const unsigned old = wv::atomic_cas(&P.bucket_maxref[bucket], cur, want);
-      if (old == cur) break;
-      cur = old;
-    }
-  }
-  pos = wv::first(pos);
-  if (unsigned(wv::lane()) < n) P.bucket_ids[size_t(bucket) * total + pos + unsigned(wv::lane())] = pend->slot[bucket][wv::lane()];
-  wv::sync();
-  if (wv::lane() == 0) {
-    pend->count[bucket]  = 0;
-    pend->maxref[bucket] = 0;
-  }
-  wv::sync();
-}
 
 #if !MANTA_TU_DEFINES(MANTA_TU_GLUE)
 WV_KERNEL void smallsv_schedule_kernel(const ScheduleParams P);
@@ -271,49 +13,21 @@
   uint32_t*      ltable = reinterpret_cast<uint32_t*>(wv::lds(SCHED_LDS_BYTES));
   SchedPending*  pend   = reinterpret_cast<SchedPending*>(reinterpret_cast<char*>(ltable) + SCHED_TABLE_BYTES + SCHED_SEQ_BYTES);
   const unsigned total  = P.n_loci * P.max_assembly_count;
-  if (lane < 16) {
-    pend->count[lane]  = 0;
-    pend->maxref[lane] = 0;
-  }
-  if (lane == 0) pend->cigarWords = 0;
-  wv::sync();
+  schedPendingInit(pend);
   while (true) {
     unsigned base = 0;
     if (lane == 0) base = wv::atomic_add(P.counter, P.chunk);
     base = wv::first(base);
     if (base >= P.n_loci) break;
-    const unsigned end = (base + P.chunk < P.n_loci) ? base + P.chunk : P.n_loci;
-    for (unsigned locus = base; locus < end; ++locus) {
-      const AsmLocusOut lo       = P.loci[locus];
-      const unsigned    nContigs = (lo.status == ASM_OK) ? lo.n_contigs : 0u;
-      if (lane >= nContigs && lane < P.max_assembly_count) {
-        SmallSvTaskInfo none = {(lo.status != ASM_OK) ? 1 : 0, 0, 0, -1};
-        P.info[locus * P.max_assembly_count + lane] = none;
-      }
-      for (unsigned ci = 0; ci < nContigs; ++ci) {
-        const unsigned        slot = locus * P.max_assembly_count + ci;
-        const SmallSvTaskInfo info = scheduleSlot(P, slot, total, ltable, gtable);
-        wv::sync();
-        if (lane == 0) P.info[slot] = info;
-        if (info.bucket >= 0) {
-          const unsigned b = unsigned(info.bucket);
-          if (lane == 0) {
-            const AlignTaskDev& t = P.tasks[slot];
-            const unsigned slabLen = unsigned(alignSlabRefLen(1, int(P.e_set[b]), t.query_len, t.ref1_len));
-            pend->slot[b][pend->count[b]] = slot;
-            pend->count[b] += 1;
-            pend->cigarWords += 4 * t.query_len + 16;
-            if (slabLen > pend->maxref[b]) pend->maxref[b] = slabLen;
-          }
-          wv::sync();
-          if (pend->count[b] == SCHED_PEND) schedFlush(P, pend, b, total);
-        }
-        wv::sync();
-      }
-    }
-  }
-  for (unsigned b = 0; b < P.n_e; ++b) schedFlush(P, pend, b, total);
-  if (lane == 0 && pend->cigarWords) wv::atomic_add(P.cigar_used, (unsigned long long)pend->cigarWords);
+    const unsigned end  = (base + P.chunk < P.n_loci) ? base + P.chunk : P.n_loci;
+    uint64_t       todo = wv::ballot(base + lane < end && !(P.scheduled && P.scheduled[base + lane]));
+    while (todo) {
+      const unsigned i = unsigned(wv::ctz(todo));
+      todo &= todo - 1;
+      scheduleLocus(P, base + i, total, ltable, SCHED_SEQ_BYTES, gtable, pend);
+    }
+  }
+  schedPendingDrain(P, pend, total);
 }
 #endif
 
diff --git a/manta_amd/csrc/schedule_slot.hpp b/manta_amd/csrc/schedule_slot.hpp
--- /dev/null
+++ b/manta_amd/csrc/schedule_slot.hpp
@@ -0,0 +1,334 @@
+#pragma once
+#include "align_kernels.hpp"
+#include "assemble_kernels.hpp"
+
+namespace manta_dev {
+
+static const int      SMALLSV_MER       = 10;
+static const unsigned SCHED_TABLE_BYTES = 4096;
+static const unsigned SCHED_SEQ_BYTES   = 6144;
+static const unsigned SCHED_LDS_BYTES   = SCHED_TABLE_BYTES + SCHED_SEQ_BYTES + 1024;
+
+struct SmallSvCuts {
+  int32_t leadingCut, trailingCut, maxLeadingCut, maxTrailingCut;
+};
+
+struct SmallSvTaskInfo {
+  int32_t status;
+  int32_t adj_leading_cut, adj_trailing_cut;
+  int32_t bucket;
+};
+
+struct ScheduleParams {
+  const AsmLocusOut*  loci;
+  const AsmContigOut* contigs;
+  const uint8_t*      seq_arena;
+  uint32_t            n_loci;
+  uint32_t            max_assembly_count;
+  const uint8_t*     refs;
+  const uint64_t*    ref_off;
+  const SmallSvCuts* cuts;
+  AlignTaskDev*    tasks;
+  SmallSvTaskInfo* info;
+  uint32_t*        bucket_ids;
+  uint32_t*        bucket_count;
+  uint32_t*        bucket_maxref;
+  unsigned long long* cigar_used;
+  uint64_t         cigar_cap;
+  uint32_t*        counter;
+  uint32_t* table_ws;
+  uint32_t  table_cap;
+  uint32_t e_set[16];
+  uint32_t n_e;
+  uint32_t chunk;
+  uint8_t*        scheduled;
+  const uint32_t* refs_ready;
+  uint32_t        refs_epoch;
+  uint32_t        reserved;
+};
+
+WV_DEV unsigned merCode(const uint8_t* p, bool& valid)
+{
+  unsigned code = 0;
+  valid         = true;
+  for (int i = 0; i < SMALLSV_MER; ++i) {
+    const unsigned c = baseCode(p[i]);
+    if (c > 3) valid = false;
+    code = (code << 2) | (c & 3u);
+  }
+  return code;
+}
+
+static const int MER_BATCH = 55;
+WV_DEV unsigned merLoadBase(const uint8_t* seq, const int len, const int p0)
+{
+  const int pos = p0 + wv::lane();
+  return (pos >= 0 && pos < len) ? baseCode(seq[pos]) : 4u;
+}
+WV_DEV unsigned merCodesFromBase(const unsigned c, bool& valid)
+{
+  const int      l   = wv::lane();
+  unsigned bad = (c > 3) ? 1u : 0u;
+  unsigned w1  = c & 3u;
+  const unsigned w2 = (w1 << 2) | wv::shfl(w1, (l + 1) & 63);
+  const unsigned b2 = bad | wv::shfl(bad, (l + 1) & 63);
+  const unsigned w4 = (w2 << 4) | wv::shfl(w2, (l + 2) & 63);
+  const unsigned b4 = b2 | wv::shfl(b2, (l + 2) & 63);
+  const unsigned w8 = (w4 << 8) | wv::shfl(w4, (l + 4) & 63);
+  const unsigned b8 = b4 | wv::shfl(b4, (l + 4) & 63);
+  const unsigned w10 = (w8 << 4) | wv::shfl(w2, (l + 8) & 63);
+  const unsigned b10 = b8 | wv::shfl(b2, (l + 8) & 63);
+  valid = (l < MER_BATCH) && (b10 == 0);
+  return w10;
+}
+WV_DEV unsigned merCodes55(const uint8_t* seq, const int len, const int p0, bool& valid)
+{
+  return merCodesFromBase(merLoadBase(seq, len, p0), valid);
+}
+
+WV_DEV bool merLookup(const uint32_t* table, const unsigned mask, const unsigned code)
+{
+  unsigned s = (code * 2654435761u) & mask;
+  while (true) {
+    const uint32_t v = table[s];
+    if (v == 0) return false;
+    if (v == code + 1) return true;
+    s = (s + 1) & mask;
+  }
+}
+
+WV_DEV SmallSvTaskInfo scheduleSlot(const ScheduleParams& P, const unsigned slot, const unsigned total, uint32_t* ltable, const unsigned seqBytes,
+                                    uint32_t* gtable)
+{
+  const unsigned    lane  = unsigned(wv::lane());
+  const unsigned    locus = slot / P.max_assembly_count, ci = slot % P.max_assembly_count;
+  const AsmLocusOut lo    = P.loci[locus];
+  SmallSvTaskInfo   info  = {0, 0, 0, -1};
+  if (lo.status != ASM_OK || ci >= lo.n_contigs) {
+    info.status = (lo.status != ASM_OK) ? 1 : 0;
+    return info;
+  }
+  const AsmContigOut co      = P.contigs[slot];
+  const uint8_t*     contigG = P.seq_arena + co.seq_off;
+  const unsigned     clen    = co.seq_len;
+  const uint8_t*     refG    = P.refs + P.ref_off[locus];
+  const int          refSize = int(P.ref_off[locus + 1] - P.ref_off[locus]);
+  const SmallSvCuts  cuts    = P.cuts[locus];
+  const uint8_t* contig = contigG;
+  const uint8_t* ref    = refG;
+  {
+    uint8_t* const  lseq = reinterpret_cast<uint8_t*>(ltable) + SCHED_TABLE_BYTES;
+    const uintptr_t gc = reinterpret_cast<uintptr_t>(contigG), gr = reinterpret_cast<uintptr_t>(refG);
+    const unsigned  leadC = unsigned(gc & 15), leadR = unsigned(gr & 15);
+    const unsigned  bytesC = (leadC + clen + 15) & ~15u, bytesR = (leadR + unsigned(refSize > 0 ? refSize : 0) + 15) & ~15u;
+    if (bytesC + bytesR <= seqBytes) {
+      const u32x4* sc = reinterpret_cast<const u32x4*>(gc - leadC);
+      const u32x4* sr = reinterpret_cast<const u32x4*>(gr - leadR);
+      u32x4*       dc = reinterpret_cast<u32x4*>(lseq);
+      u32x4*       dr = reinterpret_cast<u32x4*>(lseq + bytesC);
+      for (unsigned i = lane; i < bytesC / 16; i += 64) dc[i] = sc[i];
+      for (unsigned i = lane; i < bytesR / 16; i += 64) dr[i] = sr[i];
+      wv::sync();
+      contig = lseq + leadC;
+      ref    = lseq + bytesC + leadR;
+    }
+  }
+
+  if (clen < unsigned(SMALLSV_MER) || 2 * clen > P.table_cap) {
+    info.status = 2;
+    return info;
+  }
+  unsigned tcap = 64;
+  while (tcap < 2 * clen) tcap <<= 1;
+  const unsigned mask  = tcap - 1;
+  uint32_t*      table = (tcap * 4 <= SCHED_TABLE_BYTES) ? ltable : gtable;
+  for (unsigned i = lane; i < tcap; i += 64) table[i] = 0;
+  wv::sync();
+  for (int p0 = 0; p0 + SMALLSV_MER <= int(clen); p0 += MER_BATCH) {
+    bool           valid;
+    const unsigned code = merCodes55(contig, int(clen), p0, valid);
+    if (!valid) continue;
+    unsigned s = (code * 2654435761u) & mask;
+    while (true) {
+      const uint32_t old = wv::atomic_cas(&table[s], 0u, code + 1);
+      if (old == 0 || old == code + 1) break;
+      s = (s + 1) & mask;
+    }
+  }
+  wv::sync();
+  if (table == gtable) wv::fence_acquire();
+
+  const int minRefIndex    = cuts.leadingCut;
+  const int maxRefIndex    = refSize - (cuts.trailingCut + SMALLSV_MER);
+  const int maxFwdRefIndex = (cuts.maxLeadingCut < maxRefIndex) ? cuts.maxLeadingCut : maxRefIndex;
+  int adjLead = maxFwdRefIndex + 1;
+  if (adjLead < minRefIndex) adjLead = minRefIndex;
+  const int minRevRefIndex = (minRefIndex > refSize - cuts.maxTrailingCut) ? minRefIndex : (refSize - cuts.maxTrailingCut);
+  int       revIndex       = minRevRefIndex - 1;
+  if (revIndex > maxRefIndex) revIndex = maxRefIndex;
+  {
+    int  fBase = minRefIndex, bTop = maxRefIndex;
+    bool fDone = fBase > maxFwdRefIndex, bDone = bTop < minRevRefIndex;
+    while (!fDone || !bDone) {
+      const int      bBase = bTop - (MER_BATCH - 1);
+      const unsigned cf = merLoadBase(ref, refSize, fDone ? -1000 : fBase), cb = merLoadBase(ref, refSize, bDone ? -1000 : bBase);
+      bool           vf, vb;
+      const unsigned codeF = merCodesFromBase(cf, vf), codeB = merCodesFromBase(cb, vb);
+      const int      iF = fBase + int(lane), iB = bBase + int(lane);
+      const bool     hitF = !fDone && vf && iF <= maxFwdRefIndex && merLookup(table, mask, codeF);
+      const bool     hitB = !bDone && vb && iB >= minRevRefIndex && iB <= bTop && merLookup(table, mask, codeB);
+      const uint64_t mF = wv::ballot(hitF), mB = wv::ballot(hitB);
+      if (!fDone) {
+        if (mF) {
+          adjLead = fBase + wv::ctz(mF);
+          fDone   = true;
+        } else {
+          fBase += MER_BATCH;
+          fDone = fBase > maxFwdRefIndex;
+        }
+      }
+      if (!bDone) {
+        if (mB) {
+          revIndex = bBase + (63 - wv::clz(mB));
+          bDone    = true;
+        } else {
+          bTop -= MER_BATCH;
+          bDone = bTop < minRevRefIndex;
+        }
+      }
+    }
+  }
+  const int adjTrail = refSize - (revIndex + SMALLSV_MER);
+  const int winLen   = refSize - adjLead - adjTrail;
+  info.adj_leading_cut  = adjLead;
+  info.adj_trailing_cut = adjTrail;
+  if (winLen <= 0 || adjLead < 0 || adjTrail < 0) {
+    info.status = 3;
+    return info;
+  }
+  int            bucket = -1;
+  const unsigned need   = (clen + 63) / 64;
+  for (unsigned b = 0; b < P.n_e; ++b)
+    if (P.e_set[b] >= need) {
+      bucket = int(b);
+      break;
+    }
+  if (bucket < 0) bucket = int(P.n_e) - 1;
+  const unsigned long long cig = 8ull * co.seq_off;
+  if (cig + 4ull * clen + 16 > P.cigar_cap) {
+    info.status = 5;
+    return info;
+  }
+  if (lane == 0) {
+    AlignTaskDev t;
+    t.query     = contigG;
+    t.ref1      = refG + adjLead;
+    t.ref2      = nullptr;
+    t.query_len = clen;
+    t.ref1_len  = unsigned(winLen);
+    t.ref2_len  = 0;
+    t.cigar_off = uint32_t(cig);
+    P.tasks[slot] = t;
+  }
+  info.bucket = bucket;
+  return info;
+}
+
+static const unsigned SCHED_PEND = 8;
+struct SchedPending {
+  uint32_t count[16];
+  uint32_t maxref[16];
+  uint32_t slot[16][SCHED_PEND];
+  uint32_t cigarWords;
+};
+WV_DEV void schedFlush(const ScheduleParams& P, SchedPending* pend, const unsigned bucket, const unsigned total)
+{
+  const unsigned n = pend->count[bucket];
+  if (n == 0) return;
+  unsigned pos = 0;
+  if (wv::lane() == 0) {
+    pos = wv::atomic_add(&P.bucket_count[bucket], n);
+    unsigned cur = wv::atomic_load(&P.bucket_maxref[bucket]);
+    const unsigned want = pend->maxref[bucket];
+    while (cur < want) {
+      const unsigned old = wv::atomic_cas(&P.bucket_maxref[bucket], cur, want);
+      if (old == cur) break;
+      cur = old;
+    }
+  }
+  pos = wv::first(pos);
+  if (unsigned(wv::lane()) < n) P.bucket_ids[size_t(bucket) * total + pos + unsigned(wv::lane())] = pend->slot[bucket][wv::lane()];
+  wv::sync();
+  if (wv::lane() == 0) {
+    pend->count[bucket]  = 0;
+    pend->maxref[bucket] = 0;
+  }
+  wv::sync();
+}
+
+WV_DEV void scheduleLocus(const ScheduleParams& P, const unsigned locus, const unsigned total, uint32_t* ltable, const unsigned seqBytes,
+                          uint32_t* gtable, SchedPending* pend)
+{
+  const unsigned    lane     = unsigned(wv::lane());
+  const AsmLocusOut lo       = P.loci[locus];
+  const unsigned    nContigs = (lo.status == ASM_OK) ? lo.n_contigs : 0u;
+  if (lane >= nContigs && lane < P.max_assembly_count) {
+    SmallSvTaskInfo none = {(lo.status != ASM_OK) ? 1 : 0, 0, 0, -1};
+    P.info[locus * P.max_assembly_count + lane] = none;
+  }
+  for (unsigned ci = 0; ci < nContigs; ++ci) {
+    const unsigned        slot = locus * P.max_assembly_count + ci;
+    const SmallSvTaskInfo info = scheduleSlot(P, slot, total, ltable, seqBytes, gtable);
+    wv::sync();
+    if (lane == 0) P.info[slot] = info;
+    if (info.bucket >= 0) {
+      const unsigned b = unsigned(info.bucket);
+      if (lane == 0) {
+        const AlignTaskDev& t = P.tasks[slot];
+        const unsigned slabLen = unsigned(alignSlabRefLen(1, int(P.e_set[b]), t.query_len, t.ref1_len));
+        pend->slot[b][pend->count[b]] = slot;
+        pend->count[b] += 1;
+        pend->cigarWords += 4 * t.query_len + 16;
+        if (slabLen > pend->maxref[b]) pend->maxref[b] = slabLen;
+      }
+      wv::sync();
+      if (pend->count[b] == SCHED_PEND) schedFlush(P, pend, b, total);
+    }
+    wv::sync();
+  }
+}
+WV_DEV void schedPendingInit(SchedPending* pend)
+{
+  if (wv::lane() < 16) {
+    pend->count[wv::lane()]  = 0;
+    pend->maxref[wv::lane()] = 0;
+  }
+  if (wv::lane() == 0) pend->cigarWords = 0;
+  wv::sync();
+}
+WV_DEV void schedPendingDrain(const ScheduleParams& P, SchedPending* pend, const unsigned total)
+{
+  for (unsigned b = 0; b < P.n_e; ++b) schedFlush(P, pend, b, total);
+  if (wv::lane() == 0 && pend->cigarWords) wv::atomic_add(P.cigar_used, (unsigned long long)pend->cigarWords);
+}
+
+WV_DEV void scheduleEpilogue(const ScheduleParams& P, const unsigned locus, char* lds, const unsigned ldsBytes, SchedPending* pend)
+{
+  const unsigned lane = unsigned(wv::lane());
+  if (ldsBytes < SCHED_TABLE_BYTES + 16) return;
+  if (P.refs_ready) {
+    unsigned seen = 0;
+    if (lane == 0) seen = wv::atomic_load_system(P.refs_ready);
+    if (wv::first(seen) != P.refs_epoch) return;
+  }
+  wv::fence_acquire();
+  const AsmLocusOut lo = P.loci[locus];
+  if (lo.status != ASM_OK) return;
+  const unsigned len = (lane < lo.n_contigs) ? P.contigs[size_t(locus) * P.max_assembly_count + lane].seq_len : 0u;
+  if (wv::any(8 * len > SCHED_TABLE_BYTES)) return;
+  const unsigned seqBytes = (ldsBytes - SCHED_TABLE_BYTES) & ~15u;
+  scheduleLocus(P, locus, P.n_loci * P.max_assembly_count, reinterpret_cast<uint32_t*>(lds), seqBytes, nullptr, pend);
+  if (lane == 0) P.scheduled[locus] = 1;
+}
+
+}
```
